# ryogrid/anime-illust-image-searcher

Hardware: AMD Instinct MI355X
Metric: images/sec tagged (ViT fwd) (higher is better)
Workload: dtype f16; 1 GPU; wd-tagger ViT-B/16 448px 16-bit-operand forward + sigmoid + MCut tag selection, batch 64 per GPU, u8 NHWC images resident in HBM (BASELINE.json configs[1]); batch_per_gpu=64, image=448x448x3 u8, classes=10861, parallelism=single GPU

## Files before the change

anime-illust-image-searcher_amd/csrc/gemm.hip:

```cpp
#include <atomic>
#include <cstdlib>
#include <type_traits>

#include "gemm_plan.h"
#include "vit_internal.h"

namespace hipts {
namespace {

#ifndef HIPTS_DW_SNAKE
#define HIPTS_DW_SNAKE 1
#endif
#if HIPTS_DW_SNAKE
#define HIPTS_SNAKE_J(i, j) (((i) & 1) ? 3 - (j) : (j))
#else
#define HIPTS_SNAKE_J(i, j) (j)
#endif
#ifndef HIPTS_MFMA_ORDER
#define HIPTS_MFMA_ORDER 1
#endif
#include "gemm_epi.h"
#include "gemm_loop.h"


template <int EPI>
__global__ __launch_bounds__(512) void gemm_kernel(const GemmArgs a, int tiles_m, int tiles_n) {
    extern __shared__ __attribute__((aligned(16))) char smem[];
    const int tid = threadIdx.x, lane = tid & 63, wave = tid >> 6;
    const int wave_m = wave >> 2, wave_n = wave & 3;

    const int nwg = tiles_m * tiles_n;
    const int bid = xcd_work_id(blockIdx.x, nwg);
    const int tm = bid / tiles_n, tn = bid % tiles_n;
    const int m0 = tm * BM, n0 = tn * BN;
    const int K = a.K, nt = K / BK;
    const int w_rows = tiles_n * BN;

    f32x4 acc[8][4];
#pragma unroll
    for (int i = 0; i < 8; ++i)
#pragma unroll
        for (int j = 0; j < 4; ++j) acc[i][j] = f32x4{0.f, 0.f, 0.f, 0.f};

    stage_tile(a.A, a.M, K, m0, 0, smem, wave, lane);
    stage_tile(a.W, w_rows, K, n0, 0, smem + TILE_BYTES, wave, lane);
    asm volatile("s_waitcnt vmcnt(0)" ::: "memory");
    __syncthreads();

    for (int t = 0; t < nt; ++t) {
        char* cur = smem + (t & 1) * STAGE_BYTES;
        if (t + 1 < nt) {
            char* nxt = smem + ((t + 1) & 1) * STAGE_BYTES;
            stage_tile(a.A, a.M, K, m0, t + 1, nxt, wave, lane);
            stage_tile(a.W, w_rows, K, n0, t + 1, nxt + TILE_BYTES, wave, lane);
        }
#pragma unroll
        for (int kk = 0; kk < 2; ++kk) {
            bf16x8 af[8], wf[4];
#pragma unroll
            for (int j = 0; j < 4; ++j) wf[j] = read_frag(cur + TILE_BYTES, wave_n * 4 + j, kk, lane);
#pragma unroll
            for (int i = 0; i < 8; ++i) af[i] = read_frag(cur, wave_m * 8 + i, kk, lane);
#pragma unroll
            for (int i = 0; i < 8; ++i)
#pragma unroll
                for (int j = 0; j < 4; ++j) {
                    if constexpr (EPI == EPI_VT)
                        acc[i][j] = __builtin_amdgcn_mfma_f32_16x16x32_bf16(af[i], wf[j], acc[i][j], 0, 0, 0);
                    else
                        acc[i][j] = __builtin_amdgcn_mfma_f32_16x16x32_bf16(wf[j], af[i], acc[i][j], 0, 0, 0);
                }
        }
        asm volatile("s_waitcnt vmcnt(0)" ::: "memory");
        __syncthreads();
    }

    gemm_epilogue<EPI>(a, acc, m0, n0, wave_m, wave_n, lane);
}

__device__ __forceinline__ void wait_vmcnt(int n) {
    switch (n) {
        case 0: asm volatile("s_waitcnt vmcnt(0)" ::: "memory"); break;
        case 1: asm volatile("s_waitcnt vmcnt(1)" ::: "memory"); break;
        case 2: asm volatile("s_waitcnt vmcnt(2)" ::: "memory"); break;
        case 3: asm volatile("s_waitcnt vmcnt(3)" ::: "memory"); break;
        case 4: asm volatile("s_waitcnt vmcnt(4)" ::: "memory"); break;
        case 5: asm volatile("s_waitcnt vmcnt(5)" ::: "memory"); break;
        case 6: asm volatile("s_waitcnt vmcnt(6)" ::: "memory"); break;
        case 7: asm volatile("s_waitcnt vmcnt(7)" ::: "memory"); break;
        default: asm volatile("s_waitcnt vmcnt(8)" ::: "memory"); break;
    }
}

template <int EPI, int MR = 8, bool F16 = false, bool OP8 = false, bool SK = false, bool INT = false>
__global__ __launch_bounds__(512) __attribute__((amdgpu_num_vgpr(240))) void gemm_pp_kernel(const GemmArgs a, int tiles_m, int tiles_n) {
    static_assert(!INT || (EPI == EPI_RESID_XG && MR == 8 && !OP8 && !SK), "INT: the residual epilogue's interior form");
    static_assert(!OP8 || (F16 && MR == 8), "e4m3 operands: half 16-bit outputs, full tiles");
    static_assert(!SK || (!OP8 && MR == 8), "split-K: 16-bit operands, full tiles");
    constexpr int TBM = 2 * MR * 16;
    extern __shared__ __attribute__((aligned(16))) char smem[];
    __shared__ float2 st_table[256];
    __shared__ float2 sw_red[EPI == EPI_SWIGLU ? 1024 : 1];
    __shared__ unsigned sk_ticket[SK ? 4 : 1];
    __shared__ f32x4 colvec[INT ? (EPI == EPI_RESID_XGI ? 768 : 512) : 1];
    const int tid = threadIdx.x, lane = tid & 63;
    const int wave = __builtin_amdgcn_readfirstlane(tid >> 6);
    const int wave_m = wave >> 2, wave_n = wave & 3;

    const int nwg = tiles_m * tiles_n;
    const int K = OP8 ? a.K / 2 : a.K, nt_all = K / BK;
    const int w_rows = tiles_n * BN;
    const int S = SK ? a.sk_slices : 1;
    const int n_items = SK ? a.sk_first + (nwg - a.sk_first) * S : nwg;
    auto decode = [&](int item, WorkItem& w) {
        if (!SK || item < a.sk_first) {
            w.tile = item; w.slice = -1; w.kt0 = 0; w.nt = nt_all;
        } else {
            const int j = item - a.sk_first;
            w.tile = a.sk_first + j / S;
            w.slice = j - (j / S) * S;
            w.kt0 = w.slice * nt_all / S;
            w.nt = (w.slice + 1) * nt_all / S - w.kt0;
        }
    };
    const int scale_w = (127 - a.w_exp) * 0x01010101, scale_1 = 127 * 0x01010101;

    int stamp_tile = 0;
#define PPSTAMP(idx)                                                                                     \
    do {                                                                                                 \
        if (a.stamps && blockIdx.x == 8 && stamp_tile < 8) {                                             \
            __builtin_amdgcn_sched_barrier(0);                                                           \
            const unsigned long long ts_ = __builtin_readcyclecounter();                                 \
            if (lane == 0) a.stamps[wave * 64 + stamp_tile * 8 + (idx)] = ts_;                           \
            __builtin_amdgcn_sched_barrier(0);                                                           \
        }                                                                                                \
    } while (0)
    int item = blockIdx.x, m0, n0;
    WorkItem wi;
    decode(item, wi);
    tile_origin<TBM>(a, wi.tile, tiles_m, tiles_n, m0, n0);
    int par = 0;

    if (wave * 4 < 4 * MR) stage_tile(a.A, a.M, K, m0, wi.kt0, smem, wave, lane);
    stage_tile(a.W, w_rows, K, n0, wi.kt0, smem + TILE_BYTES, wave, lane);
    if constexpr (INT) {
        for (int i = tid; i < (a.N >> 2); i += 512) {
            colvec[i] = reinterpret_cast<const f32x4*>(a.ln_gamma)[i];
            colvec[256 + i] = reinterpret_cast<const f32x4*>(a.bias)[i];
            if constexpr (EPI == EPI_RESID_XGI) colvec[512 + i] = reinterpret_cast<const f32x4*>(a.col_u)[i];
        }
        asm volatile("s_waitcnt lgkmcnt(0)" ::: "memory");
    }

    for (;;) {
        f32x4 acc[MR][4];
        const bf16_t* src[8];
        int dst[8];
        {
            const int row_in = lane >> 3;
            const int chunk = (lane & 7) ^ row_in;
            auto slot = [&](int idx, bool isW, int rb8) {
                int grow = (isW ? n0 : m0) + rb8 * 8 + row_in;
                const int lim = isW ? w_rows : a.M;
                grow = grow < lim ? grow : lim - 1;
                src[idx] = (isW ? a.W : a.A) + (size_t)grow * K + (size_t)(wi.kt0 + 1) * BK + chunk * 8;
                dst[idx] = (isW ? TILE_BYTES : 0) + rb8 * 1024;
            };
            for (int u = 0; u < 2; ++u) {
                const int e = 2 * wave + u;
                slot(0 + u, true, e);
                slot(2 + u, true, 16 + e);
                slot(4 + u, false, e < 8 ? e : 2 * MR + (e - 8));
            }
            if constexpr (MR == 8) {
                for (int u = 0; u < 2; ++u) {
                    const int e = 2 * wave + u;
                    slot(6 + u, false, e < 8 ? 8 + e : 2 * MR + 8 + (e - 8));
                }
            } else if constexpr (MR == 6) {
                slot(6, false, wave < 4 ? 8 + wave : 2 * MR + 8 + (wave - 4));
                src[7] = src[6];
                dst[7] = dst[6];
            } else {
                static_assert(MR == 7, "tile heights: 256, 224 or 192 rows");
                auto hi = [](int f) { return f < 6 ? 8 + f : 2 * MR + 8 + (f - 6); };
                if (wave < 4) {
                    slot(6, false, hi(2 * wave));
                    slot(7, false, hi(2 * wave + 1));
                } else {
                    slot(6, false, hi(8 + (wave - 4)));
                    src[7] = src[6];
                    dst[7] = dst[6];
                }
            }
        }
        const int n_hi = (MR == 8 || (MR == 7 && wave < 4)) ? 2 : 1;
        PPSTAMP(0);
        asm volatile("s_waitcnt vmcnt(0)" ::: "memory");
        PPSTAMP(1);
        __builtin_amdgcn_s_barrier();
        if (wave_m == 1) __builtin_amdgcn_s_barrier();
        PPSTAMP(2);
        if (a.stamps && blockIdx.x == 8 && stamp_tile < 8 && lane == 0) a.stamps[wave * 64 + stamp_tile * 8 + 6] = wall_clock64();
        if (HIPTS_STAGE_AHEAD && !HIPTS_STAGE_ORDER_OLD && wi.nt > 1) {
            char* st1 = smem + ((par + 1) & 1) * STAGE_BYTES;
            for (int k : {4, 5, 0, 1}) {
                glds16(src[k], st1 + dst[k]);
                src[k] += BK;
            }
        }

        bf16x8 wf[2][4];
        i32x8 wf8[4], af8[4];
        unsigned xpf = 0;
        auto ktile = [&](int t, auto first_tag) __attribute__((always_inline)) {
            constexpr bool FIRST = decltype(first_tag)::value;
            const char* cur = smem + ((par + t) & 1) * STAGE_BYTES;
            char* nxt = smem + ((par + t + 1) & 1) * STAGE_BYTES;
            const bool more = t + 1 < wi.nt;
#pragma unroll
            for (int p = 0; p < 4; ++p) {
                const int mh = p >> 1, kk = p & 1;
                bf16x8 af[4];
                if constexpr (OP8) {
                    if (p < 2) {
#pragma unroll
                        for (int jj = 0; jj < 2; ++jj) wf8[2 * kk + jj] = read_frag8(cur + TILE_BYTES, wave_n * 4 + 2 * kk + jj, lane);
                    }
                    if (kk == 0) {
#pragma unroll
                        for (int i = 0; i < 4; ++i) af8[i] = read_frag8(cur, wave_m * MR + mh * 4 + i, lane);
                    }
                } else {
                if (p < 2) {
#pragma unroll
                    for (int j = 0; j < 4; ++j) wf[kk][j] = read_frag(cur + TILE_BYTES, wave_n * 4 + j, kk, lane);
                }
#pragma unroll
                for (int i = 0; i < 4; ++i)
                    if (mh * 4 + i < MR) af[i] = read_frag(cur, wave_m * MR + mh * 4 + i, kk, lane);
                }
                if (more) {
                    auto issue = [&](int k) {
                        glds16(src[k], nxt + dst[k]);
                        src[k] += BK;
                    };
                    if (HIPTS_STAGE_ORDER_OLD) {
                        issue(2 * p);
                        if (p < 3 || n_hi == 2) issue(2 * p + 1);
                        if (p == 3) {
                            if (n_hi == 2) asm volatile("s_waitcnt vmcnt(2)" ::: "memory");
                            else asm volatile("s_waitcnt vmcnt(1)" ::: "memory");
                        } else if (p == 1) {
                            asm volatile("s_waitcnt vmcnt(4)" ::: "memory");
                        }
                    } else if (HIPTS_STAGE_AHEAD) {
                        if (p == 0) {
                            issue(2); issue(3);
                        } else if (p == 1) {
                            issue(6);
                            if (n_hi == 2) issue(7);
                            wait_vmcnt(6 + n_hi);
                        } else if (p == 3) {
                            if (t + 2 < wi.nt) {
                                for (int k : {4, 5, 0, 1}) {
                                    glds16(src[k], const_cast<char*>(cur) + dst[k]);
                                    src[k] += BK;
                                }
                                wait_vmcnt(n_hi + 4);
                            } else {
                                wait_vmcnt(n_hi);
                            }
                        }
                    } else {
                        if (p == 0) {
                            issue(4); issue(5); issue(0); issue(1);
                            if (HIPTS_STAGE_W_EARLY) { issue(2); issue(3); }
                        } else if (p == 1) {
                            if (!HIPTS_STAGE_W_EARLY) { issue(2); issue(3); }
                            asm volatile("s_waitcnt vmcnt(6)" ::: "memory");
                        } else if (p == 2) {
                            issue(6);
                            if (n_hi == 2) issue(7);
                        } else {
                            if (n_hi == 2) asm volatile("s_waitcnt vmcnt(2)" ::: "memory");
                            else asm volatile("s_waitcnt vmcnt(1)" ::: "memory");
                        }
                    }
                } else if (p == 1) {
                    asm volatile("s_waitcnt vmcnt(0)" ::: "memory");
                }
                if constexpr (INT) {
                    if (!more && p == 2 && a.epi_prefetch) {
                        const int ldx = a.ld_out ? a.ld_out : a.N;
                        const char* xb = reinterpret_cast<const char*>(a.out_f32 + (size_t)(m0 + wave_m * 128) * ldx + n0 + wave_n * 64);
                        const unsigned o0 = (unsigned)(((lane >> 1) * ldx + (lane & 1) * 32) * 4), ost = (unsigned)(32 * ldx * 4);
                        asm volatile("global_load_dword %0, %1, %5\n\tglobal_load_dword %0, %2, %5\n\tglobal_load_dword %0, %3, %5\n\tglobal_load_dword %0, %4, %5"
                                     : "=&v"(xpf)
                                     : "v"(o0), "v"(o0 + ost), "v"(o0 + 2 * ost), "v"(o0 + 3 * ost), "s"(xb)
                                     : "memory");
                    }
                }
                __builtin_amdgcn_sched_barrier(0);
                __builtin_amdgcn_s_barrier();
                __builtin_amdgcn_sched_barrier(0);
                asm volatile("s_waitcnt lgkmcnt(0)" ::: "memory");
                __builtin_amdgcn_sched_barrier(0);
                __builtin_amdgcn_s_setprio(1);
                pp_multiply<EPI, MR, F16, OP8, FIRST>(p, acc, wf, af, wf8, af8, scale_w, scale_1);
                __builtin_amdgcn_s_setprio(0);
                __builtin_amdgcn_sched_barrier(0);
                __builtin_amdgcn_s_barrier();
                __builtin_amdgcn_sched_barrier(0);
            }
        };
        ktile(0, std::true_type{});
        for (int t = 1; t < wi.nt; ++t) ktile(t, std::false_type{});
        if (wave_m == 0) __builtin_amdgcn_s_barrier();
        PPSTAMP(3);
        if (a.stamps && blockIdx.x == 8 && stamp_tile < 8 && lane == 0) a.stamps[wave * 64 + stamp_tile * 8 + 7] = wall_clock64();

        int elane = lane;
        asm volatile("" : "+v"(elane));
        f32x4 bias_pre[4];
        if constexpr (INT) {
#pragma unroll
            for (int j = 0; j < 4; ++j) bias_pre[j] = f32x4{0.f, 0.f, 0.f, 0.f};
        } else {
            load_bias<EPI>(a, n0, wave_n, elane, bias_pre);
        }
        constexpr bool FOLDABLE = EPI == EPI_VT || EPI == EPI_GELU || EPI == EPI_STAR || EPI == EPI_QK || EPI == EPI_QK_ROPE || EPI == EPI_SWIGLU ||
                                  EPI == EPI_RESID_ROWSTAT || EPI == EPI_RESID_XGI;
        const bool fold_st = FOLDABLE && a.stat_in != nullptr;
        const bool fold_many = fold_st && a.stat_in_blocks > 4;
        float2 st_pv[4];
        if (fold_st && !fold_many && tid < TBM) row_stat_request(a, m0 + tid, st_pv);
        const int next = item + gridDim.x;
        const bool has_next = next < n_items;
        WorkItem wi_next{0, -1, 0, nt_all};
        int m0n = 0, n0n = 0;
        const int par_next = (par + wi.nt) & 1;
        if (has_next) {
            decode(next, wi_next);
            tile_origin<TBM>(a, wi_next.tile, tiles_m, tiles_n, m0n, n0n);
            char* st = smem + par_next * STAGE_BYTES;
            if (wave * 4 < 4 * MR) stage_tile(a.A, a.M, K, m0n, wi_next.kt0, st, wave, lane);
            stage_tile(a.W, w_rows, K, n0n, wi_next.kt0, st + TILE_BYTES, wave, lane);
        }
        PPSTAMP(4);
        bool run_epilogue = true;
        if constexpr (SK) {
            if (wi.slice >= 0) {
                constexpr size_t SLAB = (size_t)TBM * BN * 4;
                const int tl = wi.tile - a.sk_first;
                unsigned* tickets = reinterpret_cast<unsigned*>(a.sk_ws);
                char* slabs = reinterpret_cast<char*>(a.sk_ws) + 4096 + (size_t)tl * S * SLAB;
                {
                    const auto rs = __builtin_amdgcn_make_buffer_rsrc(slabs + (size_t)wi.slice * SLAB, 0, (int)SLAB, 0x00020000);
                    typedef unsigned int u32x4 __attribute__((ext_vector_type(4)));
#pragma unroll
                    for (int i = 0; i < MR; ++i)
#pragma unroll
                        for (int j = 0; j < 4; ++j)
                            __builtin_amdgcn_raw_buffer_store_b128(__builtin_bit_cast(u32x4, acc[i][j]), rs, (((wave * MR + i) * 4 + j) * 64 + lane) * 16, 0, 16);
                }
                asm volatile("s_waitcnt vmcnt(0)" ::: "memory");
                __builtin_amdgcn_s_barrier();
                if (threadIdx.x == 0)
                    sk_ticket[0] = __hip_atomic_fetch_add(tickets + tl, 1u, __ATOMIC_RELAXED, __HIP_MEMORY_SCOPE_AGENT);
                __builtin_amdgcn_fence(__ATOMIC_RELEASE, "workgroup");
                __builtin_amdgcn_s_barrier();
                __builtin_amdgcn_fence(__ATOMIC_ACQUIRE, "workgroup");
                const unsigned ticket = sk_ticket[0];
                if (ticket != (unsigned)(S - 1)) {
                    run_epilogue = false;
                } else {
                    if (threadIdx.x == 0) {
                        __builtin_amdgcn_fence(__ATOMIC_ACQUIRE, "agent");
                        __hip_atomic_store(tickets + tl, 0u, __ATOMIC_RELAXED, __HIP_MEMORY_SCOPE_AGENT);
                    }
                    asm volatile("s_waitcnt vmcnt(0)" ::: "memory");
                    __builtin_amdgcn_s_barrier();
                    const f32x4* sl = reinterpret_cast<const f32x4*>(slabs) + (size_t)(wave * MR * 4) * 64 + lane;
#pragma unroll
                    for (int i = 0; i < MR; ++i) {
#pragma unroll
                        for (int j = 0; j < 4; ++j) acc[i][j] = sl[(size_t)(i * 4 + j) * 64];
                        for (int sx = 1; sx < S; ++sx) {
                            const f32x4* sp = sl + (size_t)sx * (SLAB / 16);
                            f32x4 v[4];
#pragma unroll
                            for (int j = 0; j < 4; ++j) v[j] = sp[(size_t)(i * 4 + j) * 64];
#pragma unroll
                            for (int j = 0; j < 4; ++j) acc[i][j] = acc[i][j] + v[j];
                        }
                    }
                }
            }
        }
        if (run_epilogue) {
            if (fold_st) fold_publish(a, m0, tid, TBM, fold_many, st_pv, st_table);
            bool staged = false;
            if constexpr (staged_epilogue_built(EPI)) {
                if (staged_epilogue_ok(EPI, a)) {
                    float2* red = (EPI == EPI_SWIGLU && a.stat_part) ? sw_red : nullptr;
                    gemm_epilogue_staged<EPI, MR, F16>(a, acc, m0, n0, wave_m, wave_n, elane, smem + ((par + wi.nt + 1) & 1) * STAGE_BYTES + wave * 8192, bias_pre,
                                                       fold_st ? st_table : nullptr, red);
                    staged = true;
                    if constexpr (EPI == EPI_SWIGLU) {
                        if (red) {
                            lds_table_visible();
                            if (tid < TBM) {
                                const float2 p0 = red[tid * 4], p1 = red[tid * 4 + 1], p2 = red[tid * 4 + 2], p3 = red[tid * 4 + 3];
                                const int m = m0 + tid;
                                if (m < a.M)
                                    *reinterpret_cast<float2*>(a.stat_part + 2 * ((size_t)(n0 >> 8) * a.stat_stride + m)) =
                                        make_float2((p0.x + p1.x) + (p2.x + p3.x), (p0.y + p1.y) + (p2.y + p3.y));
                            }
                        }
                    }
                }
            }
            if (!staged)
                gemm_epilogue<EPI, MR, F16, INT>(a, acc, m0, n0, wave_m, wave_n, elane, bias_pre, smem + ((par + wi.nt + 1) & 1) * STAGE_BYTES,
                                                 fold_st ? st_table : nullptr, INT ? colvec : nullptr);
        }
        if (a.epi_prio) __builtin_amdgcn_s_setprio(0);
        if constexpr (INT) asm volatile("" ::"v"(xpf));
        PPSTAMP(5);
        ++stamp_tile;
        if (!has_next) break;
        item = next;
        wi = wi_next;
        m0 = m0n;
        n0 = n0n;
        par = par_next;
    }
#undef PPSTAMP
}

#define PP2_STAMP(idx)                                                                                   \
    if constexpr (STAMP) {                                                                               \
        if (blockIdx.x == 0 && (t == 10 || t == 11)) {                                                   \
            __builtin_amdgcn_sched_barrier(0);                                                           \
            unsigned long long ts_;                                                                      \
            asm volatile("s_memtime %0\n\ts_waitcnt lgkmcnt(0)" : "=s"(ts_)::"memory");                 \
            if (lane == 0) a.stamps[wave * 64 + (t - 10) * 16 + mh * 8 + (idx)] = ts_;                   \
            __builtin_amdgcn_sched_barrier(0);                                                           \
        }                                                                                                \
    }

template <int EPI, bool STAMP = false>
__global__ __launch_bounds__(512) void gemm_pp2_kernel(const GemmArgs a, int tiles_m, int tiles_n) {
    extern __shared__ __attribute__((aligned(16))) char smem[];
    const int tid = threadIdx.x, lane = tid & 63;
    const int wave = __builtin_amdgcn_readfirstlane(tid >> 6);
    const int wave_m = wave >> 2, wave_n = wave & 3;

    const int nwg = tiles_m * tiles_n;
    const int bid = xcd_work_id(blockIdx.x, nwg);
    const int tm = bid / tiles_n, tn = bid % tiles_n;
    const int m0 = tm * BM, n0 = tn * BN;
    const int K = a.K, nt = K / BK;
    const int w_rows = tiles_n * BN;

    f32x4 acc[8][4];
#pragma unroll
    for (int i = 0; i < 8; ++i)
#pragma unroll
        for (int j = 0; j < 4; ++j) acc[i][j] = f32x4{0.f, 0.f, 0.f, 0.f};

    stage_tile(a.A, a.M, K, m0, 0, smem, wave, lane);
    stage_tile(a.W, w_rows, K, n0, 0, smem + TILE_BYTES, wave, lane);

    const bf16_t* src[8];
    int dst[8];
    {
        const int row_in = lane >> 3;
        const int chunk = (lane & 7) ^ row_in;
        auto slot = [&](int idx, bool isW, int rb8) {
            int grow = (isW ? n0 : m0) + rb8 * 8 + row_in;
            const int lim = isW ? w_rows : a.M;
            grow = grow < lim ? grow : lim - 1;
            src[idx] = (isW ? a.W : a.A) + (size_t)grow * K + BK + chunk * 8;
            dst[idx] = (isW ? TILE_BYTES : 0) + rb8 * 1024;
        };
        for (int u = 0; u < 4; ++u) slot(u, true, 4 * wave + u);
        for (int u = 0; u < 2; ++u) {
            const int e = 2 * wave + u;
            slot(4 + u, false, e < 8 ? e : e + 8);
            slot(6 + u, false, e < 8 ? 8 + e : 16 + e);
        }
    }
    asm volatile("s_waitcnt vmcnt(0)" ::: "memory");
    __builtin_amdgcn_s_barrier();
    if (wave_m == 1) __builtin_amdgcn_s_barrier();

    bf16x8 wf[2][4];
    for (int t = 0; t < nt; ++t) {
        const char* cur = smem + (t & 1) * STAGE_BYTES;
        char* nxt = smem + ((t + 1) & 1) * STAGE_BYTES;
        const bool more = t + 1 < nt;
#pragma unroll
        for (int mh = 0; mh < 2; ++mh) {
            PP2_STAMP(0)
            bf16x8 af[2][4];
            if (mh == 0) {
#pragma unroll
                for (int kk = 0; kk < 2; ++kk)
#pragma unroll
                    for (int j = 0; j < 4; ++j) wf[kk][j] = read_frag(cur + TILE_BYTES, wave_n * 4 + j, kk, lane);
            }
#pragma unroll
            for (int kk = 0; kk < 2; ++kk)
#pragma unroll
                for (int i = 0; i < 4; ++i) af[kk][i] = read_frag(cur, wave_m * 8 + mh * 4 + i, kk, lane);
            if (more) {
                if (mh == 0) {
#pragma unroll
                    for (int u = 0; u < 6; ++u) {
                        glds16(src[u], nxt + dst[u]);
                        src[u] += BK;
                    }
                    PP2_STAMP(1)
                    asm volatile("s_waitcnt vmcnt(6)" ::: "memory");
                } else {
#pragma unroll
                    for (int u = 6; u < 8; ++u) {
                        glds16(src[u], nxt + dst[u]);
                        src[u] += BK;
                    }
                    PP2_STAMP(1)
                    asm volatile("s_waitcnt vmcnt(2)" ::: "memory");
                }
            } else if (mh == 0) {
                asm volatile("s_waitcnt vmcnt(0)" ::: "memory");
            }
            PP2_STAMP(2)
            __builtin_amdgcn_sched_barrier(0);
            __builtin_amdgcn_s_barrier();
            __builtin_amdgcn_sched_barrier(0);
            PP2_STAMP(3)
            asm volatile("s_waitcnt lgkmcnt(0)" ::: "memory");
            __builtin_amdgcn_sched_barrier(0);
            PP2_STAMP(4)
            __builtin_amdgcn_s_setprio(1);
#pragma unroll
            for (int kk = 0; kk < 2; ++kk)
#pragma unroll
                for (int i = 0; i < 4; ++i)
#pragma unroll
                    for (int j = 0; j < 4; ++j) {
                        if constexpr (EPI == EPI_VT)
                            acc[mh * 4 + i][j] = __builtin_amdgcn_mfma_f32_16x16x32_bf16(af[kk][i], wf[kk][j], acc[mh * 4 + i][j], 0, 0, 0);
                        else
                            acc[mh * 4 + i][j] = __builtin_amdgcn_mfma_f32_16x16x32_bf16(wf[kk][j], af[kk][i], acc[mh * 4 + i][j], 0, 0, 0);
                    }
            __builtin_amdgcn_s_setprio(0);
            PP2_STAMP(5)
// ... 126 lines not shown
            dst[4 + i] = DW_A_BYTES + rb * 1024;
        }
    }
    const int frag_off = (lane & 15) * 64 + (((lane >> 4) ^ Image64::swizzle(lane & 15)) * 16);
    auto issue = [&](int i, char* st) {
        glds16(src[i], st + dst[i]);
        src[i] += DW_BK;
    };
    auto frag = [&](const char* base, int rb) { return *reinterpret_cast<const bf16x8*>(base + rb * 1024 + frag_off); };

    f32x4 acc[8][4];

    const bool trace = a.stamps && a.trace && blockIdx.x < 4096;
    if (trace && tid == 0) {
        a.stamps[blockIdx.x * 8 + 0] = __builtin_amdgcn_s_getreg(63492);
        a.stamps[blockIdx.x * 8 + 1] = __builtin_amdgcn_s_getreg(63508);
        a.stamps[blockIdx.x * 8 + 2] = wall_clock64();
    }
    const int npro = nt < 3 ? nt : 3;
    for (int s0 = 0; s0 < npro; ++s0)
#pragma unroll
        for (int i = 0; i < 6; ++i) issue(i, smem + s0 * DW_STAGE);
    if (npro == 3) asm volatile("s_waitcnt vmcnt(12)" ::: "memory");
    else if (npro == 2) asm volatile("s_waitcnt vmcnt(6)" ::: "memory");
    else asm volatile("s_waitcnt vmcnt(0)" ::: "memory");
    __builtin_amdgcn_s_barrier();
    __builtin_amdgcn_sched_barrier(0);

    bf16x8 wfr[2][4], alo[2][4], ahi[4];
#pragma unroll
    for (int j = 0; j < 4; ++j) wfr[0][j] = frag(smem + DW_A_BYTES, wave_n * 4 + j);
#pragma unroll
    for (int i = 0; i < 4; ++i) alo[0][i] = frag(smem, wave_m * 8 + i);

    int slot = 0;
    unsigned long long wait_cyc = 0, bar_cyc = 0;
    const unsigned long long loop_t0 = a.stamps ? __builtin_readcyclecounter() : 0;
    const unsigned long long wall_t0 = a.stamps ? wall_clock64() : 0;
    auto mm = [&](f32x4& c, const bf16x8& av, const bf16x8& wv, bool zero) {
        const f32x4 c0 = zero ? f32x4{0.f, 0.f, 0.f, 0.f} : c;
        if constexpr (EPI == EPI_VT) c = mfma_16x16x32<F16>(av, wv, c0);
        else c = mfma_16x16x32<F16>(wv, av, c0);
    };
    auto step = [&](auto H1, auto H2, auto H3, auto U, auto Z) __attribute__((always_inline)) {
        constexpr bool has1 = decltype(H1)::value, has2 = decltype(H2)::value, has3 = decltype(H3)::value, first = decltype(Z)::value;
        constexpr int u = decltype(U)::value;
        const char* cur = smem + slot * DW_STAGE;
        const int slot1 = slot == 2 ? 0 : slot + 1;
        const char* nx = smem + slot1 * DW_STAGE;
#pragma unroll
        for (int i = 0; i < 4; ++i)
#pragma unroll
            for (int j = 0; j < 4; ++j) {
                mm(acc[i][HIPTS_SNAKE_J(i, j)], alo[u][i], wfr[u][HIPTS_SNAKE_J(i, j)], first);
                if (i == 0) ahi[j] = frag(cur, wave_m * 8 + 4 + j);
                __builtin_amdgcn_sched_barrier(0);
            }
        if constexpr (has1) {
            unsigned long long q0 = 0, q1 = 0;
            if (a.stamps) q0 = __builtin_readcyclecounter();
            if constexpr (has2) asm volatile("s_waitcnt vmcnt(6) lgkmcnt(0)" ::: "memory");
            else asm volatile("s_waitcnt vmcnt(0) lgkmcnt(0)" ::: "memory");
            if (a.stamps) q1 = __builtin_readcyclecounter();
            __builtin_amdgcn_s_barrier();
            if (a.stamps) { const unsigned long long q2 = __builtin_readcyclecounter(); wait_cyc += q1 - q0; bar_cyc += q2 - q1; }
        }
        __builtin_amdgcn_sched_barrier(0);
        char* fill = smem + slot * DW_STAGE;
#pragma unroll
        for (int i = 0; i < 4; ++i)
#pragma unroll
            for (int j = 0; j < 4; ++j) {
                mm(acc[4 + i][HIPTS_SNAKE_J(i, j)], ahi[i], wfr[u][HIPTS_SNAKE_J(i, j)], first);
                const int idx = i * 4 + j;
                if constexpr (has1) {
                    if (idx < 4) wfr[u ^ 1][idx] = frag(nx + DW_A_BYTES, wave_n * 4 + idx);
                    else if (idx < 8) alo[u ^ 1][idx - 4] = frag(nx, wave_m * 8 + (idx - 4));
                }
                if constexpr (has3) {
                    if (idx >= 8 && idx < 14) issue(idx - 8, fill);
                }
                __builtin_amdgcn_sched_barrier(0);
            }
        slot = slot1;
    };
    using T = std::true_type;
    using F = std::false_type;
    using U0 = std::integral_constant<int, 0>;
    using U1 = std::integral_constant<int, 1>;
    if (nt >= 6) {
        step(T{}, T{}, T{}, U0{}, T{});
        step(T{}, T{}, T{}, U1{}, F{});
        for (int s = 2; s + 6 <= nt; s += 2) {
            step(T{}, T{}, T{}, U0{}, F{});
            step(T{}, T{}, T{}, U1{}, F{});
        }
    }
    if (nt >= 4) {
        if (nt == 4) step(T{}, T{}, T{}, U0{}, T{});
        else step(T{}, T{}, T{}, U0{}, F{});
        step(T{}, T{}, F{}, U1{}, F{});
    }
    if (nt == 2) step(T{}, F{}, F{}, U0{}, T{});
    else step(T{}, F{}, F{}, U0{}, F{});
    step(F{}, F{}, F{}, U1{}, F{});
    if (trace && tid == 0) a.stamps[blockIdx.x * 8 + 3] = wall_clock64();
    if (a.stamps && !trace && blockIdx.x == 8 && lane == 0) {
        a.stamps[wave * 64 + 0] = __builtin_readcyclecounter() - loop_t0;
        a.stamps[wave * 64 + 1] = wait_cyc;
        a.stamps[wave * 64 + 2] = bar_cyc;
        a.stamps[wave * 64 + 3] = wall_clock64() - wall_t0;
    }
    __builtin_amdgcn_s_barrier();
    if constexpr (staged_epilogue_built(EPI)) {
        if (staged_epilogue_ok(EPI, a)) {
            const float2* st_tab = nullptr;
            if (a.stat_in) {
                float2* tab = reinterpret_cast<float2*>(smem + 4 * 8192 * 2);
                fold_rows<false>(a, m0 + tid, tab, tid);
                st_tab = tab;
            }
            gemm_epilogue_staged<EPI, 8, F16>(a, acc, m0, n0, wave_m, wave_n, lane, smem + wave * 8192, nullptr, st_tab);
            if (trace && tid == 0) a.stamps[blockIdx.x * 8 + 4] = wall_clock64();
            return;
        }
    }
    gemm_epilogue<EPI, 8, F16>(a, acc, m0, n0, wave_m, wave_n, lane, nullptr, smem);
    if (trace && tid == 0) a.stamps[blockIdx.x * 8 + 4] = wall_clock64();
}

static_assert(GEMM_PLAN_TILE == BM && GEMM_PLAN_TILE == BN && GEMM_PLAN_BK == BK && GEMM_PLAN_HALF_BN == DW_BN && GEMM_PLAN_HALF_BN == S3_BN &&
              GEMM_PLAN_LDS == LDS_BYTES && GEMM_PLAN_LDS3 == DW_LDS && GEMM_PLAN_LDS3 == S3_LDS, "gemm_plan.h plans for other tiles than these kernels'");

std::atomic<long long> g_q4_mask{-1};
unsigned gemm_q4_mask() {
    long long v = g_q4_mask.load(std::memory_order_relaxed);
    if (v < 0) {
        v = getenv("HIPTS_GEMM_Q4") ? (long long)(unsigned)strtoul(getenv("HIPTS_GEMM_Q4"), nullptr, 0) : (long long)GEMM_Q4_DEFAULT_MASK;
        g_q4_mask.store(v, std::memory_order_relaxed);
    }
    return (unsigned)v;
}

int gemm_variant() { return gemm_knobs().variant; }

int gemm_plan_status(const GemmPlan& p, GemmEpilogue epi) {
    if (p.error == 1) return set_error(HIPTS_ERR_INVALID, "half-precision operands are only built for the pp and dw GEMM loops");
    if (p.error == 2) return set_error(HIPTS_ERR_INVALID, "gemm: e4m3 operands are not built for epilogue %d", (int)epi);
    return HIPTS_OK;
}

using GemmKernel = void (*)(const GemmArgs, int, int);
template <int EPI>
GemmKernel pp_kernel(int mr, bool f16, bool op8, bool sk, bool interior) {
    if (op8) {
        if constexpr (EPI == EPI_STAR || EPI == EPI_RESID || EPI == EPI_RESCALE || EPI == EPI_RESID_LN || EPI == EPI_QK || EPI == EPI_VT || EPI == EPI_BIAS)
            if (mr == 8 && f16 && !sk && !interior) return gemm_pp_kernel<EPI, 8, true, true>;
        return nullptr;
    }
    if (sk) {
        if constexpr (EPI == EPI_RESID || EPI == EPI_RESID_XG || EPI == EPI_RESID_XGI || EPI == EPI_RESID_ROWSTAT || EPI == EPI_HEAD)
            if (mr == 8 && !interior) return f16 ? gemm_pp_kernel<EPI, 8, true, false, true> : gemm_pp_kernel<EPI, 8, false, false, true>;
        return nullptr;
    }
    if (interior) {
        if constexpr (EPI == EPI_RESID_XG)
            if (mr == 8) return f16 ? gemm_pp_kernel<EPI, 8, true, false, false, true> : gemm_pp_kernel<EPI, 8, false, false, false, true>;
        return nullptr;
    }
    if (f16) return mr == 6 ? gemm_pp_kernel<EPI, 6, true> : mr == 7 ? gemm_pp_kernel<EPI, 7, true> : mr == 8 ? gemm_pp_kernel<EPI, 8, true> : nullptr;
    return mr == 7 ? gemm_pp_kernel<EPI, 7, false> : mr == 8 ? gemm_pp_kernel<EPI, 8, false> : nullptr;
}

template <int EPI>
int kernel_resources_t(int mr, bool f16, bool op8, bool sk, bool interior, int* num_regs, int* scratch_bytes, int* static_lds) {
    const GemmKernel k = pp_kernel<EPI>(mr, f16, op8, sk, interior);
    HIPTS_REQUIRE(k != nullptr, "hiptsdbg_gemm_kernel_resources: no gemm_pp_kernel is built for epilogue %d, mr %d, f16 %d, op8 %d, sk %d, interior %d", EPI, mr,
                  (int)f16, (int)op8, (int)sk, (int)interior);
    hipFuncAttributes at;
    HIPTS_HIP(hipFuncGetAttributes(&at, reinterpret_cast<const void*>(k)));
    *num_regs = at.numRegs;
    *scratch_bytes = (int)at.localSizeBytes;
    *static_lds = (int)at.sharedSizeBytes;
    return HIPTS_OK;
}

template <int EPI>
int launch_t(const GemmArgs& a, hipStream_t s) {
    int dev = 0;
    const int cus = current_device_cus(&dev);
    const GemmPlan p = gemm_plan((GemmEpilogue)EPI, a, cus, gemm_knobs(), gemm_q4_mask());
    HIPTS_TRY(gemm_plan_status(p, (GemmEpilogue)EPI));
    GemmArgs ar = a;
    ar.raster_gm = p.raster_gm; ar.raster_gn = p.raster_gn; ar.epi_prio = p.epi_prio; ar.epi_prefetch = p.epi_prefetch;
    ar.sk_first = p.sk_first; ar.sk_slices = p.sk_slices;
    const bool f16 = a.f16 != 0;
    auto go = [&](void (*kernel)(const GemmArgs, int, int)) { kernel<<<p.grid, p.block, p.lds_bytes, s>>>(ar, p.tiles_m, p.tiles_n); };
    switch (p.loop) {
        case HIPTSDBG_GEMM_Q4: return launch_gemm_q4((GemmEpilogue)EPI, ar, p, dev, s);
        case HIPTSDBG_GEMM_PP_E4M3:
            if constexpr (EPI == EPI_STAR || EPI == EPI_RESID || EPI == EPI_RESCALE || EPI == EPI_RESID_LN || EPI == EPI_QK || EPI == EPI_VT ||
                          EPI == EPI_BIAS) {
                static PerDevice once;
                HIPTS_TRY(allow_dynamic_lds(once, dev, p.lds_bytes, gemm_pp_kernel<EPI, 8, true, true>));
                go(pp_kernel<EPI>(8, true, true, false, false));
            }
            break;
        case HIPTSDBG_GEMM_DW: {
            if constexpr (EPI == EPI_VT || EPI == EPI_GELU || EPI == EPI_STAR || EPI == EPI_QK || EPI == EPI_QK_ROPE || EPI == EPI_SWIGLU)
                HIPTS_REQUIRE(!(a.stat_in && a.stat_in_blocks > 4), "gemm: the two-workgroups-per-CU loop folds at most 4 stat_in pairs per row (%d given)", a.stat_in_blocks);
            static PerDevice once;
            HIPTS_TRY(allow_dynamic_lds(once, dev, p.lds_bytes, gemm_dw_kernel<EPI, false>, gemm_dw_kernel<EPI, true>));
            if (f16) go(gemm_dw_kernel<EPI, true>);
            else go(gemm_dw_kernel<EPI, false>);
            break;
        }
        case HIPTSDBG_GEMM_S3: {
            static PerDevice once;
            HIPTS_TRY(allow_dynamic_lds(once, dev, p.lds_bytes, gemm_s3_kernel<EPI>));
            go(gemm_s3_kernel<EPI>);
            break;
        }
        case HIPTSDBG_GEMM_V1: {
            static PerDevice once;
            HIPTS_TRY(allow_dynamic_lds(once, dev, p.lds_bytes, gemm_kernel<EPI>));
            go(gemm_kernel<EPI>);
            break;
        }
        case HIPTSDBG_GEMM_PP2: {
            static PerDevice once;
            if constexpr (EPI == EPI_GELU) {
                HIPTS_TRY(allow_dynamic_lds(once, dev, p.lds_bytes, gemm_pp2_kernel<EPI, false>, gemm_pp2_kernel<EPI, true>));
                if (p.stamped) {
                    go(gemm_pp2_kernel<EPI, true>);
                    break;
                }
            } else {
                HIPTS_TRY(allow_dynamic_lds(once, dev, p.lds_bytes, gemm_pp2_kernel<EPI, false>));
            }
            go(gemm_pp2_kernel<EPI, false>);
            break;
        }
        default: {
            if constexpr (EPI == EPI_RESID || EPI == EPI_RESID_XG || EPI == EPI_RESID_XGI || EPI == EPI_RESID_ROWSTAT || EPI == EPI_HEAD) {
                if (p.sk_slices >= 2) {
                    static PerDevice once;
                    HIPTS_TRY(allow_dynamic_lds(once, dev, p.lds_bytes, gemm_pp_kernel<EPI, 8, false, false, true>, gemm_pp_kernel<EPI, 8, true, false, true>));
                    go(pp_kernel<EPI>(8, f16, false, true, false));
                    break;
                }
            }
            if constexpr (EPI == EPI_RESID_XG) {
                if (p.interior) {
                    static PerDevice once;
                    HIPTS_TRY(allow_dynamic_lds(once, dev, p.lds_bytes, gemm_pp_kernel<EPI, 8, false, false, false, true>, gemm_pp_kernel<EPI, 8, true, false, false, true>));
                    go(pp_kernel<EPI>(8, f16, false, false, true));
                    break;
                }
            }
            static PerDevice once;
            HIPTS_TRY(allow_dynamic_lds(once, dev, p.lds_bytes, gemm_pp_kernel<EPI, 8, false>, gemm_pp_kernel<EPI, 7, false>, gemm_pp_kernel<EPI, 8, true>,
                                        gemm_pp_kernel<EPI, 7, true>, gemm_pp_kernel<EPI, 6, true>));
            const GemmKernel k = pp_kernel<EPI>(p.mr, f16, false, false, false);
            HIPTS_REQUIRE(k != nullptr, "gemm: no %d-row tiles are built for these operands", 32 * p.mr);
            go(k);
        }
    }
    HIPTS_LAUNCH_CHECK();
    return HIPTS_OK;
}

}

const GemmKnobs& gemm_knobs() {
    static const GemmKnobs knobs = [] {
        auto num = [](const char* name, int dflt) { const char* e = getenv(name); return e ? atoi(e) : dflt; };
        GemmKnobs k;
        const char* e = getenv("HIPTS_GEMM");
        k.variant_set = e != nullptr;
        k.variant = (e && strcmp(e, "v1") == 0) ? HIPTSDBG_GEMM_V1 : (e && strcmp(e, "pp2") == 0) ? HIPTSDBG_GEMM_PP2 : (e && strcmp(e, "s3") == 0) ? HIPTSDBG_GEMM_S3
                    : (e && strcmp(e, "dw") == 0) ? HIPTSDBG_GEMM_DW : HIPTSDBG_GEMM_PP;
        k.auto_dw = num("HIPTS_GEMM_AUTO_DW", 1) != 0;
        k.dw_limit4 = num("HIPTS_GEMM_DW_LIMIT", 2);
        k.dw_mask = getenv("HIPTS_GEMM_DW_MASK") ? (unsigned)strtoul(getenv("HIPTS_GEMM_DW_MASK"), nullptr, 0) : 0u;
        e = getenv("HIPTS_GEMM_BM");
        k.min_mr = !e ? 6 : strcmp(e, "256") == 0 ? 8 : strcmp(e, "224") == 0 ? 7 : 6;
        k.mr_shared = num("HIPTS_GEMM_MR_SHARED", -1);
        e = getenv("HIPTS_GEMM_PERSIST");
        k.persist = !(e && strcmp(e, "0") == 0);
        k.raster = num("HIPTS_GEMM_RASTER", 8);
        k.raster_gn = num("HIPTS_GEMM_RASTER_GN", 6);
        k.epi_prio = num("HIPTS_EPI_PRIO", 0);
        k.epi_prefetch = num("HIPTS_EPI_PREFETCH", 0);
        k.resid_general = num("HIPTS_RESID_GENERAL", 0) != 0;
        k.splitk = num("HIPTS_GEMM_SPLITK", 0);
        k.splitk_head = num("HIPTS_GEMM_SPLITK_HEAD", 0);
        k.splitk_minkt = num("HIPTS_GEMM_SPLITK_MINKT", 5);
        return k;
    }();
    return knobs;
}

int launch_gemm(GemmEpilogue epi, const GemmArgs& a, hipStream_t s) {
    if (a.op8) HIPTS_REQUIRE(a.K % 128 == 0 && a.K >= 128, "gemm: K=%d must be a positive multiple of 128 with e4m3 operands", a.K);
    if (a.out8)
        HIPTS_REQUIRE((epi == EPI_STAR || epi == EPI_RESID_LN) && (a.ld_out ? a.ld_out : a.N) % 16 == 0,
                      "gemm: e4m3 output needs the STAR / RESID_LN epilogue and a row stride that is a multiple of 16");
    HIPTS_REQUIRE(a.K % BK == 0 && a.K >= BK, "gemm: K=%d must be a positive multiple of %d", a.K, BK);
    HIPTS_REQUIRE(a.M >= 1 && a.N >= 1, "gemm: empty problem");
    if (epi != EPI_HEAD) HIPTS_REQUIRE(a.N % 16 == 0, "gemm: N=%d must be a multiple of 16", a.N);
    if (epi == EPI_VT) HIPTS_REQUIRE(a.M % 4 == 0 && a.tokens % 4 == 0, "gemm: V^T epilogue needs tokens %% 4 == 0");
    if (epi == EPI_VT && staged_epilogue_ok(epi, a))
        HIPTS_REQUIRE(a.M % 8 == 0, "gemm: V^T epilogue with tokens %% 8 == 0 needs M %% 8 == 0 (M = %d)", a.M);
    if (epi == EPI_QK || epi == EPI_VT) HIPTS_REQUIRE(a.hd_log2 == 5 || a.hd_log2 == 6, "gemm: head_dim must be 32 or 64");
    if (epi == EPI_QK || epi == EPI_QK_ROPE)
        HIPTS_REQUIRE(a.out_bf16 && a.out2_bf16 && a.dim > 0 && a.N <= 3 * a.dim && (a.N <= 2 * a.dim || a.out3_bf16), "gemm: q / k / v outputs missing for N = %d, dim = %d", a.N, a.dim);
    if (epi == EPI_QK_ROPE)
        HIPTS_REQUIRE(a.hd_log2 == 6 && a.dim % 64 == 0 && a.rope && a.rope_tokens >= 0 && a.tokens >= 1, "gemm: QK_ROPE needs head_dim 64 and the rotary table");
    if (epi == EPI_RESID_XG) HIPTS_REQUIRE(!a.rowstat && !a.stat_in, "gemm: RESID_XG ignores an input fold; use RESID_XGI");
    if (epi == EPI_RESID_XGI) HIPTS_REQUIRE((a.rowstat || a.stat_in) && a.col_u, "gemm: RESID_XGI needs rowstat / stat_in and col_u");
    if (epi == EPI_RESID_XG || epi == EPI_RESID_XGI)
        HIPTS_REQUIRE(a.out_f32 && (!a.out_bf16 || (a.ln_gamma && a.N % 8 == 0 && (!a.stat_part || a.stat_stride >= a.M))),
                      "gemm: RESID_XG needs the fp32 stream, col_u with rowstat, and gamma (N %% 8 == 0) with the 16-bit copy");
    if (a.stat_in) HIPTS_REQUIRE(a.stat_in_blocks <= 64 && a.stat_in_blocks >= 1 && a.stat_in_stride >= a.M && a.ln_dim >= 1, "gemm: stat_in needs its block count (<= 64), stride and ln_dim");
    if ((a.rowstat || a.stat_in) && epi != EPI_RESID_ROWSTAT && epi != EPI_RESID_XGI)
        HIPTS_REQUIRE(a.col_u && (epi == EPI_QK || epi == EPI_QK_ROPE || epi == EPI_VT || epi == EPI_GELU || epi == EPI_SWIGLU || epi == EPI_STAR),
                      "gemm: a folded LayerNorm (rowstat) is built for the QK, QK_ROPE, VT, GELU, STAR and SWIGLU epilogues");
    if ((a.rowstat || a.stat_in) && epi != EPI_RESID_ROWSTAT && epi != EPI_RESID_XGI) {
        HIPTS_REQUIRE(staged_epilogue_ok(epi, a) && (gemm_variant() == 1 || gemm_variant() == 4), "gemm: a folded LayerNorm needs the staged epilogue (pp / dw loops, aligned outputs)");
    }
    if (epi == EPI_RESID_ROWSTAT) HIPTS_REQUIRE((a.rowstat || a.stat_in) && a.col_u && a.out_f32, "gemm: RESID_ROWSTAT needs rowstat / stat_in, col_u and the fp32 stream");
    if (epi == EPI_SWIGLU) HIPTS_REQUIRE(!a.stat_part || a.stat_stride >= a.M, "gemm: SWIGLU stat_stride must cover M rows");
    if (epi == EPI_SWIGLU)
        HIPTS_REQUIRE(a.N % 64 == 0 && (a.ld_out ? a.ld_out : a.N / 2) % 8 == 0 && a.out_bf16, "gemm: SWIGLU needs N %% 64 == 0 and an output stride that is a multiple of 8");
    if (epi == EPI_RESCALE) HIPTS_REQUIRE(a.res_scale != nullptr, "gemm: RESCALE epilogue needs res_scale");
    if (epi == EPI_RESID_LS) HIPTS_REQUIRE(a.res_scale && a.out_f32 && !a.x_blocked, "gemm: RESID_LS needs the layer scale and the row-major fp32 stream");
    if (epi == EPI_RESID_LN)
        HIPTS_REQUIRE(a.N <= BN && a.ln_gamma && a.out_bf16 && a.out_f32, "gemm: RESID_LN needs the whole row in one tile (N <= %d), gamma and both outputs", BN);
    switch (epi) {
        case EPI_PATCH: return launch_t<EPI_PATCH>(a, s);
        case EPI_QK: return launch_t<EPI_QK>(a, s);
        case EPI_VT: return launch_t<EPI_VT>(a, s);
        case EPI_RESID: return launch_t<EPI_RESID>(a, s);
        case EPI_GELU: return launch_t<EPI_GELU>(a, s);
        case EPI_HEAD: return launch_t<EPI_HEAD>(a, s);
        case EPI_STAR: return launch_t<EPI_STAR>(a, s);
        case EPI_RESCALE: return launch_t<EPI_RESCALE>(a, s);
        case EPI_BIAS: return launch_t<EPI_BIAS>(a, s);
        case EPI_RESID_LN: return launch_t<EPI_RESID_LN>(a, s);
        case EPI_QK_ROPE: return launch_t<EPI_QK_ROPE>(a, s);
        case EPI_SWIGLU: return launch_t<EPI_SWIGLU>(a, s);
        case EPI_RESID_ROWSTAT: return launch_t<EPI_RESID_ROWSTAT>(a, s);
        case EPI_RESID_XG: return launch_t<EPI_RESID_XG>(a, s);
        case EPI_RESID_XGI: return launch_t<EPI_RESID_XGI>(a, s);
        case EPI_RESID_LS: return launch_t<EPI_RESID_LS>(a, s);
    }
    return set_error(HIPTS_ERR_INVALID, "gemm: unknown epilogue");
}

void set_gemm_q4_mask(unsigned mask) { g_q4_mask.store((long long)mask, std::memory_order_relaxed); }

namespace {
__global__ void gelu_probe_kernel(const f32x4* __restrict__ x, f32x4* __restrict__ y, int n4, int tanh_form) {
    const int i = blockIdx.x * blockDim.x + threadIdx.x;
    if (i < n4) y[i] = gelu_f4(x[i], tanh_form);
}
}

}

extern "C" int hiptsdbg_gelu(const float* x_host, int n, int tanh_form, float* y_host) {
    using namespace hipts;
    HIPTS_TRY(use_device(0));
    HIPTS_REQUIRE(x_host && y_host && n > 0 && n % 4 == 0, "hiptsdbg_gelu: n must be a positive multiple of 4");
    DevBuf x, y;
    HIPTS_TRY(x.alloc((size_t)n * 4));
    HIPTS_TRY(y.alloc((size_t)n * 4));
    HIPTS_TRY(upload(x.p, x_host, (size_t)n * 4));
    gelu_probe_kernel<<<(n / 4 + 255) / 256, 256>>>(x.as<f32x4>(), y.as<f32x4>(), n / 4, tanh_form);
    HIPTS_LAUNCH_CHECK();
    HIPTS_HIP(hipMemcpy(y_host, y.p, (size_t)n * 4, hipMemcpyDeviceToHost));
    return HIPTS_OK;
}

extern "C" int hiptsdbg_gemm_kernel_resources(int epi, int mr, int f16, int op8, int sk, int interior, int* num_regs, int* scratch_bytes, int* static_lds) {
    using namespace hipts;
    HIPTS_REQUIRE(num_regs && scratch_bytes && static_lds && epi >= EPI_PATCH && epi <= EPI_RESID_LS, "hiptsdbg_gemm_kernel_resources: bad argument");
    HIPTS_TRY(use_device(0));
#define HIPTS_RES_CASE(E) \
    case E: return kernel_resources_t<E>(mr, f16 != 0, op8 != 0, sk != 0, interior != 0, num_regs, scratch_bytes, static_lds)
    switch (epi) {
        HIPTS_RES_CASE(EPI_PATCH); HIPTS_RES_CASE(EPI_QK); HIPTS_RES_CASE(EPI_VT); HIPTS_RES_CASE(EPI_RESID); HIPTS_RES_CASE(EPI_GELU);
        HIPTS_RES_CASE(EPI_HEAD); HIPTS_RES_CASE(EPI_STAR); HIPTS_RES_CASE(EPI_RESCALE); HIPTS_RES_CASE(EPI_BIAS); HIPTS_RES_CASE(EPI_RESID_LN);
        HIPTS_RES_CASE(EPI_QK_ROPE); HIPTS_RES_CASE(EPI_SWIGLU); HIPTS_RES_CASE(EPI_RESID_ROWSTAT); HIPTS_RES_CASE(EPI_RESID_XG);
        HIPTS_RES_CASE(EPI_RESID_XGI); HIPTS_RES_CASE(EPI_RESID_LS);
    }
#undef HIPTS_RES_CASE
    return set_error(HIPTS_ERR_INVALID, "hiptsdbg_gemm_kernel_resources: unknown epilogue");
}

extern "C" int hiptsdbg_gemm_plan(int epi, int M, int N, int K, int f16, int shared_chip, unsigned features, int ld_out, int dim, int cus,
                                  unsigned q4_mask, hiptsdbg_gemm_plan_t* out) {
    using namespace hipts;
    HIPTS_REQUIRE(out && epi >= EPI_PATCH && epi <= EPI_RESID_LS && M >= 1 && N >= 1 && K >= 64 && K % 64 == 0 && cus >= 1, "hiptsdbg_gemm_plan: bad argument");
    static float dummy[2];
    GemmArgs g{};
    g.M = M; g.N = N; g.K = K; g.f16 = f16; g.shared_chip = shared_chip; g.ld_out = ld_out; g.dim = dim;
    if (features & 1) g.stat_part = dummy;
    if (features & 2) { g.sk_ws = dummy; g.sk_ws_bytes = GEMM_SK_WS_BYTES; }
    if (features & 4) g.pos = dummy;
    if (features & 8) g.res_scale = dummy;
    if (features & 16) { g.out_bf16 = reinterpret_cast<bf16_t*>(dummy); g.ln_gamma = dummy; }
    if (features & 32) g.stat_in = dummy;
    if (features & 64) g.op8 = 1;
    if (features & 128) g.stamps = reinterpret_cast<unsigned long long*>(dummy);
    *out = gemm_plan((GemmEpilogue)epi, g, cus, gemm_knobs(), q4_mask);
    return gemm_plan_status(*out, (GemmEpilogue)epi);
}

extern "C" int hiptsdbg_gemm_tile_walk(int tiles_m, int tiles_n, int tile_rows, int raster_gm, int raster_gn, int32_t* m0, int32_t* n0) {
    using namespace hipts;
    HIPTS_REQUIRE(m0 && n0 && tiles_m >= 1 && tiles_n >= 1 && (tile_rows == 256 || tile_rows == 224 || tile_rows == 192) && raster_gm >= 0 && raster_gn >= 0,
                  "hiptsdbg_gemm_tile_walk: bad argument");
    GemmArgs g{};
    g.raster_gm = raster_gm;
    g.raster_gn = raster_gn;
    for (int id = 0; id < tiles_m * tiles_n; ++id) {
        int m, n;
        if (tile_rows == 256) tile_origin<256>(g, id, tiles_m, tiles_n, m, n);
        else if (tile_rows == 224) tile_origin<224>(g, id, tiles_m, tiles_n, m, n);
        else tile_origin<192>(g, id, tiles_m, tiles_n, m, n);
        m0[id] = m;
        n0[id] = n;
    }
    return HIPTS_OK;
}
```

anime-illust-image-searcher_amd/csrc/gemm_dbg.hip:

```cpp
#include <vector>

#include "../../include/hip_tagsearch_debug.h"
#include "vit_internal.h"

namespace hipts {
namespace {

int put_f32(DevBuf& buf, const float* host, size_t n, const float** dev) {
    *dev = nullptr;
    if (!host) return HIPTS_OK;
    HIPTS_TRY(buf.alloc(n * 4));
    HIPTS_TRY(upload(buf.p, host, n * 4));
    *dev = buf.as<float>();
    return HIPTS_OK;
}

int guarded(DevBuf& buf, uint64_t bytes, uint64_t need, int fill, const char* what, bool required) {
    if (bytes == 0) {
        HIPTS_REQUIRE(!required, "hiptsdbg_gemm_epilogue: the %s buffer is required by this epilogue", what);
        return HIPTS_OK;
    }
    HIPTS_REQUIRE(bytes >= need, "hiptsdbg_gemm_epilogue: the %s buffer has %llu bytes, the launch's extent is %llu", what, (unsigned long long)bytes,
                  (unsigned long long)need);
    HIPTS_TRY(buf.alloc(bytes));
    HIPTS_HIP(hipMemset(buf.p, fill & 0xff, bytes));
    return HIPTS_OK;
}

int fetch(void* host, const DevBuf& buf, uint64_t bytes) {
    if (bytes == 0) return HIPTS_OK;
    HIPTS_REQUIRE(host, "hiptsdbg_gemm_epilogue: an output buffer has a size but no host pointer");
    HIPTS_HIP(hipMemcpy(host, buf.p, bytes, hipMemcpyDeviceToHost));
    return HIPTS_OK;
}

}
}

extern "C" int hiptsdbg_gemm_epilogue(const hiptsdbg_gemm_case_t* in, hiptsdbg_gemm_out_t* out) {
    using namespace hipts;
    HIPTS_REQUIRE(in && out && in->a && in->w, "hiptsdbg_gemm_epilogue: null argument");
    const int epi = in->epi, M = in->M, N = in->N, K = in->K;
    HIPTS_REQUIRE(epi >= EPI_PATCH && epi <= EPI_RESID_LS && M >= 1 && N >= 1 && K >= 64 && K % 64 == 0 && (long long)M * K < (1ll << 31) &&
                      (long long)N * K < (1ll << 31),
                  "hiptsdbg_gemm_epilogue: unsupported shape");
    HIPTS_REQUIRE(epi == EPI_HEAD || N % 16 == 0, "hiptsdbg_gemm_epilogue: N must be a multiple of 16");
    HIPTS_TRY(use_device(0));

    const bool is_qk = epi == EPI_QK || epi == EPI_QK_ROPE;
    const uint64_t ld = in->ld_out ? in->ld_out : (epi == EPI_SWIGLU ? N / 2 : N);
    HIPTS_REQUIRE(ld >= (uint64_t)(epi == EPI_SWIGLU ? N / 2 : N) || is_qk || epi == EPI_VT, "hiptsdbg_gemm_epilogue: ld_out is smaller than a row");
    const bool blocked_ok = epi == EPI_RESID || epi == EPI_RESCALE || epi == EPI_RESID_ROWSTAT || epi == EPI_RESID_XG || epi == EPI_RESID_XGI ||
                            epi == EPI_BIAS || epi == EPI_RESID_LN;
    HIPTS_REQUIRE(!in->x_blocked || (blocked_ok && ld % 16 == 0), "hiptsdbg_gemm_epilogue: x_blocked needs a residual / bias epilogue and ld %% 16 == 0");
    const bool writes_x = blocked_ok || epi == EPI_PATCH || epi == EPI_RESID_LS;
    const uint64_t rows_x = in->x_blocked ? (uint64_t)round_up(M, 16) : (uint64_t)M;
    uint64_t need16[3] = {0, 0, 0};
    bool req16[3] = {false, false, false};
    if (is_qk || epi == EPI_VT) {
        HIPTS_REQUIRE(in->tokens >= 1 && in->tokens_pad >= in->tokens && in->dim >= 16 && (in->hd_log2 == 5 || in->hd_log2 == 6) &&
                          (in->heads << in->hd_log2) == in->dim && N <= (is_qk ? 3 : 1) * in->dim,
                      "hiptsdbg_gemm_epilogue: q / k / v layouts need tokens <= tokens_pad, heads * head_dim == dim and N within the layouts");
        const uint64_t images = (uint64_t)(M + in->tokens - 1) / in->tokens;
        const uint64_t layout = images * in->tokens_pad * in->dim * 2;
        need16[0] = layout; req16[0] = true;
        if (is_qk) { need16[1] = layout; req16[1] = true; }
        if (is_qk && N > 2 * in->dim) { need16[2] = layout; req16[2] = true; }
    } else if (epi == EPI_GELU || epi == EPI_STAR || epi == EPI_SWIGLU || epi == EPI_RESID_LN) {
        need16[0] = (uint64_t)M * ld * 2; req16[0] = true;
    } else if (epi == EPI_RESID_XG || epi == EPI_RESID_XGI || epi == EPI_RESID_LS) {
        need16[0] = (uint64_t)M * ld * 2;
    }
    if (epi == EPI_PATCH || in->pos) HIPTS_REQUIRE(in->pos && in->tokens >= 1, "hiptsdbg_gemm_epilogue: pos needs tokens");
    const bool has_stat = epi == EPI_SWIGLU || epi == EPI_RESID_XG || epi == EPI_RESID_XGI;
    HIPTS_REQUIRE(out->stat_part_bytes == 0 || (has_stat && in->stat_stride >= M), "hiptsdbg_gemm_epilogue: stat_part needs SWIGLU / RESID_XG / RESID_XGI and stat_stride >= M");
    HIPTS_REQUIRE(out->rowmajor_bytes == 0 || (in->x_blocked && (epi == EPI_RESID || epi == EPI_RESCALE || epi == EPI_RESID_ROWSTAT)),
                  "hiptsdbg_gemm_epilogue: resid_rowmajor_out needs x_blocked and a plain residual epilogue");
    HIPTS_REQUIRE(out->probs_bytes == 0 || epi == EPI_HEAD, "hiptsdbg_gemm_epilogue: probs is EPI_HEAD's");
    HIPTS_REQUIRE(in->x_init_bytes <= out->x_bytes && (in->x_init_bytes == 0 || in->x_init), "hiptsdbg_gemm_epilogue: x_init does not fit x");
    if (in->stat_in)
        HIPTS_REQUIRE(in->stat_in_blocks >= 1 && in->stat_in_blocks <= 64 && in->stat_in_stride >= M, "hiptsdbg_gemm_epilogue: stat_in needs its block count and stride");

    DevBuf x, rowmajor, probs, o16[3], stat;
    HIPTS_TRY(guarded(x, out->x_bytes, (writes_x || epi == EPI_HEAD) ? rows_x * ld * 4 : 0, in->fill, "x", writes_x));
    HIPTS_TRY(guarded(rowmajor, out->rowmajor_bytes, (uint64_t)M * ld * 4, in->fill, "rowmajor", false));
    HIPTS_TRY(guarded(probs, out->probs_bytes, (uint64_t)M * ld * 4, in->fill, "probs", false));
    for (int i = 0; i < 3; ++i) {
        HIPTS_REQUIRE(out->out16_bytes[i] == 0 || need16[i] > 0, "hiptsdbg_gemm_epilogue: this epilogue has no 16-bit output %d", i);
        HIPTS_TRY(guarded(o16[i], out->out16_bytes[i], need16[i], in->fill, "out16", req16[i]));
    }
    HIPTS_TRY(guarded(stat, out->stat_part_bytes, (uint64_t)((N + 255) / 256) * (uint64_t)in->stat_stride * 8, in->fill, "stat_part", false));
    if (in->x_init_bytes) HIPTS_TRY(upload(x.p, in->x_init, in->x_init_bytes));

    DevBuf A, W, bias, pos, rs, lg, lb, cu, rst, sti, rope, skws;
    const int Np = round_up(N, 256);
    HIPTS_TRY(A.alloc((size_t)M * K * 2));
    HIPTS_TRY(W.alloc((size_t)Np * K * 2));
    HIPTS_HIP(hipMemset(W.p, 0, W.bytes));
    HIPTS_TRY(upload(A.p, in->a, (size_t)M * K * 2));
    HIPTS_TRY(upload(W.p, in->w, (size_t)N * K * 2));
    GemmArgs g{};
    g.A = A.as<bf16_t>(); g.W = W.as<bf16_t>(); g.M = M; g.N = N; g.K = K; g.f16 = in->f16 ? 1 : 0; g.shared_chip = in->shared_chip ? 1 : 0;
    if (in->bias) {
        HIPTS_TRY(put_f32(bias, in->bias, (size_t)N, &g.bias));
    } else {
        HIPTS_TRY(bias.alloc((size_t)Np * 4));
        HIPTS_HIP(hipMemset(bias.p, 0, bias.bytes));
        g.bias = bias.as<float>();
    }
    HIPTS_TRY(put_f32(pos, in->pos, in->pos ? (size_t)in->tokens * N : 0, &g.pos));
    HIPTS_TRY(put_f32(rs, in->res_scale, (size_t)N, &g.res_scale));
    HIPTS_TRY(put_f32(lg, in->ln_gamma, (size_t)(epi == EPI_SWIGLU ? N / 2 : N), &g.ln_gamma));
    HIPTS_TRY(put_f32(lb, in->ln_beta, (size_t)N, &g.ln_beta));
    HIPTS_TRY(put_f32(cu, in->col_u, (size_t)N, &g.col_u));
    HIPTS_TRY(put_f32(rst, in->rowstat, (size_t)2 * M, &g.rowstat));
    HIPTS_TRY(put_f32(sti, in->stat_in, in->stat_in ? (size_t)2 * in->stat_in_blocks * in->stat_in_stride : 0, &g.stat_in));
    if (epi == EPI_QK_ROPE) {
        HIPTS_REQUIRE(in->rope && in->rope_tokens >= 1, "hiptsdbg_gemm_epilogue: QK_ROPE needs the rotary table");
        HIPTS_TRY(put_f32(rope, in->rope, (size_t)in->rope_tokens * 64, &g.rope));
    }
    if (in->sk_ws) {
        HIPTS_TRY(skws.alloc(GEMM_SK_WS_BYTES));
        HIPTS_HIP(hipMemset(skws.p, 0, skws.bytes));
        g.sk_ws = skws.p; g.sk_ws_bytes = GEMM_SK_WS_BYTES;
    }
    g.out_f32 = out->x_bytes ? x.as<float>() : nullptr;
    g.resid_rowmajor_out = out->rowmajor_bytes ? rowmajor.as<float>() : nullptr;
    g.out2_f32 = out->probs_bytes ? probs.as<float>() : nullptr;
    g.out_bf16 = out->out16_bytes[0] ? o16[0].as<bf16_t>() : nullptr;
    g.out2_bf16 = out->out16_bytes[1] ? o16[1].as<bf16_t>() : nullptr;
    g.out3_bf16 = out->out16_bytes[2] ? o16[2].as<bf16_t>() : nullptr;
    g.stat_part = out->stat_part_bytes ? stat.as<float>() : nullptr;
    g.stat_stride = in->stat_stride;
    g.tokens = in->tokens; g.tokens_pad = in->tokens_pad; g.heads = in->heads; g.dim = in->dim; g.hd_log2 = in->hd_log2;
    g.stat_in_blocks = in->stat_in_blocks; g.stat_in_stride = in->stat_in_stride; g.ln_dim = in->ln_dim; g.rope_tokens = in->rope_tokens;
    g.gelu_tanh = in->gelu_tanh; g.star_kind = in->star_kind; g.ld_out = in->ld_out; g.x_blocked = in->x_blocked ? 1 : 0;
    g.qscale = in->qscale; g.ln_eps = in->ln_eps; g.star_scale = in->star_scale; g.star_bias = in->star_bias;

    HIPTS_TRY(launch_gemm((GemmEpilogue)epi, g, nullptr));
    HIPTS_HIP(hipDeviceSynchronize());

    HIPTS_TRY(fetch(out->x, x, out->x_bytes));
    HIPTS_TRY(fetch(out->rowmajor, rowmajor, out->rowmajor_bytes));
    HIPTS_TRY(fetch(out->probs, probs, out->probs_bytes));
    for (int i = 0; i < 3; ++i) HIPTS_TRY(fetch(out->out16[i], o16[i], out->out16_bytes[i]));
    HIPTS_TRY(fetch(out->stat_part, stat, out->stat_part_bytes));
    return HIPTS_OK;
}
```

anime-illust-image-searcher_amd/csrc/gemm_epi.h:

```cpp

constexpr int BM = 256, BN = 256, BK = 64;
#ifndef HIPTS_STAGE_AHEAD
#define HIPTS_STAGE_AHEAD 1
#endif
#ifndef HIPTS_STAGE_W_EARLY
#define HIPTS_STAGE_W_EARLY 0
#endif
#ifndef HIPTS_STAGE_ORDER_OLD
#define HIPTS_STAGE_ORDER_OLD 0
#endif
constexpr int TILE_BYTES = BM * BK * 2;
constexpr int STAGE_BYTES = 2 * TILE_BYTES;
constexpr int LDS_BYTES = 2 * STAGE_BYTES;

__device__ __forceinline__ void glds16(const void* g, void* lds) {
    __builtin_amdgcn_global_load_lds((const __attribute__((address_space(1))) void*)g,
                                     (__attribute__((address_space(3))) void*)lds, 16, 0, 0);
}

__device__ __forceinline__ void stage_tile(const bf16_t* __restrict__ X, int rows_total, int K, int row0, int kt,
                                           char* lds_tile, int wave, int lane) {
    const int row_in = lane >> 3;
    const int chunk = (lane & 7) ^ row_in;
#pragma unroll
    for (int i = 0; i < 4; ++i) {
        const int rb8 = wave * 4 + i;
        int grow = row0 + rb8 * 8 + row_in;
        grow = grow < rows_total ? grow : rows_total - 1;
        const bf16_t* g = X + (size_t)grow * K + (size_t)kt * BK + chunk * 8;
        glds16(g, lds_tile + rb8 * 1024);
    }
}

__device__ __forceinline__ bf16x8 read_frag(const char* lds_tile, int rowblk, int kk, int lane) {
    const int r = lane & 15;
    const int c = (kk * 4 + (lane >> 4)) ^ (r & 7);
    return *reinterpret_cast<const bf16x8*>(lds_tile + (rowblk * 2 + (r >> 3)) * 1024 + (r & 7) * 128 + c * 16);
}

__device__ __forceinline__ i32x8 read_frag8(const char* lds_tile, int rowblk, int lane) {
    const int r = lane & 15, q = lane >> 4;
    const char* row = lds_tile + (rowblk * 2 + (r >> 3)) * 1024 + (r & 7) * 128;
    const int4 lo = *reinterpret_cast<const int4*>(row + (((2 * q) ^ (r & 7)) * 16));
    const int4 hi = *reinterpret_cast<const int4*>(row + (((2 * q + 1) ^ (r & 7)) * 16));
    return i32x8{lo.x, lo.y, lo.z, lo.w, hi.x, hi.y, hi.z, hi.w};
}

template <bool TANH>
__device__ __forceinline__ f32x4 gelu_f4(f32x4 x) {
    if constexpr (TANH) {
        const float c1 = -2.885390081777927f * 0.7978845608028654f, c2 = c1 * 0.044715f;
        const f32x4 t = x * x;
        const f32x4 g = x * __builtin_elementwise_fma(f32x4{c2, c2, c2, c2}, t, f32x4{c1, c1, c1, c1});
        f32x4 e{__builtin_amdgcn_exp2f(g[0]), __builtin_amdgcn_exp2f(g[1]), __builtin_amdgcn_exp2f(g[2]), __builtin_amdgcn_exp2f(g[3])};
        e = e + f32x4{1.f, 1.f, 1.f, 1.f};
        return x * f32x4{__builtin_amdgcn_rcpf(e[0]), __builtin_amdgcn_rcpf(e[1]), __builtin_amdgcn_rcpf(e[2]), __builtin_amdgcn_rcpf(e[3])};
    }
    const f32x4 xc{__builtin_amdgcn_fmed3f(x[0], -5.5f, 5.5f), __builtin_amdgcn_fmed3f(x[1], -5.5f, 5.5f), __builtin_amdgcn_fmed3f(x[2], -5.5f, 5.5f),
                   __builtin_amdgcn_fmed3f(x[3], -5.5f, 5.5f)};
    const f32x4 t = xc * xc;
    auto k4 = [](float c) { return f32x4{c, c, c, c}; };
    f32x4 p = __builtin_elementwise_fma(k4(2.2240455115528255e-08f), t, k4(6.478198381570408e-06f));
    p = __builtin_elementwise_fma(p, t, k4(0.00017989516452868775f));
    p = __builtin_elementwise_fma(p, t, k4(0.00474442647621276f));
    p = __builtin_elementwise_fma(p, t, k4(0.03488362160853281f));
    p = __builtin_elementwise_fma(p, t, k4(0.39894214428114516f));
    f32x4 q = __builtin_elementwise_fma(k4(1.1920686967418627e-06f), t, k4(7.74708620425572e-05f));
    q = __builtin_elementwise_fma(q, t, k4(0.0019464965294343475f));
    q = __builtin_elementwise_fma(q, t, k4(0.02924650260921815f));
    q = __builtin_elementwise_fma(q, t, k4(0.25410501090673415f));
    q = __builtin_elementwise_fma(q, t, k4(1.0f));
    const f32x4 rq{__builtin_amdgcn_rcpf(q[0]), __builtin_amdgcn_rcpf(q[1]), __builtin_amdgcn_rcpf(q[2]), __builtin_amdgcn_rcpf(q[3])};
    const f32x4 r = (xc * p) * rq;
    return x * (r + k4(0.5f));
}
__device__ __forceinline__ f32x4 gelu_f4(f32x4 x, int tanh_form) { return tanh_form ? gelu_f4<true>(x) : gelu_f4<false>(x); }

__device__ __forceinline__ float2 ln_stat_pair(const GemmArgs& a, float s1, float s2) {
    const float inv = 1.0f / (float)a.ln_dim;
    const float mean = s1 * inv;
    const float var = fmaxf(s2 * inv - mean * mean, 0.f);
    const float rstd = 1.0f / sqrtf(var + a.ln_eps);
    return make_float2(rstd, rstd * mean);
}

__device__ __forceinline__ float2 row_stat(const GemmArgs& a, int m) {
    m = m < a.M ? m : a.M - 1;
    if (a.stat_in) {
        float s1 = 0.f, s2 = 0.f;
        int b = 0;
        for (; b + 8 <= a.stat_in_blocks; b += 8) {
            float2 v[8];
#pragma unroll
            for (int u = 0; u < 8; ++u) v[u] = *reinterpret_cast<const float2*>(a.stat_in + 2 * ((size_t)(b + u) * a.stat_in_stride + m));
#pragma unroll
            for (int u = 0; u < 8; ++u) {
                s1 += v[u].x;
                s2 += v[u].y;
            }
        }
        for (; b < a.stat_in_blocks; ++b) {
            const float2 v = *reinterpret_cast<const float2*>(a.stat_in + 2 * ((size_t)b * a.stat_in_stride + m));
            s1 += v.x;
            s2 += v.y;
        }
        return ln_stat_pair(a, s1, s2);
    }
    return *reinterpret_cast<const float2*>(a.rowstat + 2 * (size_t)m);
}

__device__ __forceinline__ void row_stat_request(const GemmArgs& a, int m, float2 (&pv)[4]) {
    m = m < a.M ? m : a.M - 1;
#pragma unroll
    for (int b = 0; b < 4; ++b)
        pv[b] = b < a.stat_in_blocks ? *reinterpret_cast<const float2*>(a.stat_in + 2 * ((size_t)b * a.stat_in_stride + m)) : make_float2(0.f, 0.f);
}
__device__ __forceinline__ float2 row_stat_finish(const GemmArgs& a, const float2 (&pv)[4]) {
    return ln_stat_pair(a, ((pv[0].x + pv[1].x) + pv[2].x) + pv[3].x, ((pv[0].y + pv[1].y) + pv[2].y) + pv[3].y);
}

__device__ __forceinline__ void epi_turn(const GemmArgs& a, int wave_m, int step) {
    if (a.epi_prio) {
        if ((step ^ wave_m) & 1) __builtin_amdgcn_s_setprio(1);
        else __builtin_amdgcn_s_setprio(0);
    }
}

__device__ __forceinline__ size_t x_off(const GemmArgs& a, int m, int nc, int ld) {
    if (a.x_blocked) return (((size_t)(m >> 4) * (size_t)(ld >> 4) + (size_t)(nc >> 4)) << 8) + (size_t)((m & 15) * 16 + (nc & 15));
    return (size_t)m * ld + nc;
}

template <int EPI>
__device__ __forceinline__ void load_cols(const float* __restrict__ vec, const GemmArgs& a, int n0, int wave_n, int lane, f32x4 (&bv)[4]);
template <int EPI>
__device__ __forceinline__ void load_bias(const GemmArgs& a, int n0, int wave_n, int lane, f32x4 (&bv)[4]) {
    load_cols<EPI>(a.bias, a, n0, wave_n, lane, bv);
}
template <int EPI>
__device__ __forceinline__ void load_cols(const float* __restrict__ vec, const GemmArgs& a, int n0, int wave_n, int lane, f32x4 (&bv)[4]) {
    const int lr = lane & 15, lq = lane >> 4;
#pragma unroll
    for (int j = 0; j < 4; ++j) {
        if constexpr (EPI == EPI_VT) {
            const int n = n0 + wave_n * 64 + j * 16 + lr;
            bv[j] = f32x4{n < a.N ? vec[n] : 0.f, 0.f, 0.f, 0.f};
        } else if constexpr (EPI == EPI_HEAD) {
            bv[j] = f32x4{0.f, 0.f, 0.f, 0.f};
        } else {
            const int nc = n0 + wave_n * 64 + j * 16 + 4 * lq;
            bv[j] = nc < a.N ? *reinterpret_cast<const f32x4*>(vec + nc) : f32x4{0.f, 0.f, 0.f, 0.f};
        }
    }
}

__device__ __forceinline__ f32x4 star_relu4(f32x4 x, float s, float b, int kind = 0) {
    if (kind == 1) {
        const f32x4 g = x * -1.4426950408889634f;
        const f32x4 e{__builtin_amdgcn_exp2f(g[0]), __builtin_amdgcn_exp2f(g[1]), __builtin_amdgcn_exp2f(g[2]), __builtin_amdgcn_exp2f(g[3])};
        const f32x4 d = e + 1.0f;
        return x * f32x4{__builtin_amdgcn_rcpf(d[0]), __builtin_amdgcn_rcpf(d[1]), __builtin_amdgcn_rcpf(d[2]), __builtin_amdgcn_rcpf(d[3])};
    }
    if (kind == 2) return x;
    const f32x4 r = __builtin_elementwise_max(x, f32x4{0.f, 0.f, 0.f, 0.f});
    return r * r * s + b;
}

template <int EPI>
__device__ __forceinline__ void epi_bias(const GemmArgs& a, int n0, int wave_n, int lane, const f32x4* bias_pre, f32x4 (&bias_v)[4]) {
    if (bias_pre) {
#pragma unroll
        for (int j = 0; j < 4; ++j) bias_v[j] = bias_pre[j];
    } else {
        load_bias<EPI>(a, n0, wave_n, lane, bias_v);
    }
}

template <int CHUNKS>
struct RowImage {
    static_assert(CHUNKS == 8 || CHUNKS == 4, "128 B or 64 B rows");
    static __device__ __forceinline__ int swizzle(int row) { return CHUNKS == 8 ? (row >> 1) & 7 : (row >> 2) & 3; }
    static __device__ __forceinline__ char* at(char* image, int row, int chunk) { return image + row * (CHUNKS * 16) + (chunk ^ swizzle(row)) * 16; }
    static __device__ __forceinline__ void put4(char* image, int row, int j, int lq, bf16x4 v) {
// ... 424 lines not shown
                __builtin_amdgcn_fence(__ATOMIC_ACQUIRE, "workgroup");
                const int t = wave_n * 64 + lane;
                if (t < MR * 16) {
                    const int r = wave_m * (MR * 16) + t;
                    const float2 p0 = red[r * 4], p1 = red[r * 4 + 1], p2 = red[r * 4 + 2], p3 = red[r * 4 + 3];
                    const int m = m0 + r;
                    if (m < a.M)
                        *reinterpret_cast<float2*>(a.stat_part + 2 * ((size_t)(n0 >> 8) * a.stat_stride + m)) =
                            make_float2((p0.x + p1.x) + (p2.x + p3.x), (p0.y + p1.y) + (p2.y + p3.y));
                }
            }
            return;
        }
        if constexpr (EPI == EPI_RESID || EPI == EPI_RESCALE || EPI == EPI_RESID_ROWSTAT || EPI == EPI_RESID_LS) {
            f32x4 rs[4];
            if constexpr (EPI == EPI_RESCALE) {
#pragma unroll
                for (int j = 0; j < 4; ++j) rs[j] = nv[j] ? *reinterpret_cast<const f32x4*>(a.res_scale + nc[j]) : f32x4{0.f, 0.f, 0.f, 0.f};
            }
            if constexpr (EPI == EPI_RESID_ROWSTAT) {
#pragma unroll
                for (int j = 0; j < 4; ++j) rs[j] = nv[j] ? *reinterpret_cast<const f32x4*>(a.col_u + nc[j]) : f32x4{0.f, 0.f, 0.f, 0.f};
            }
            constexpr int RB = 4;
            auto rmw = [&](auto interior_tag) {
                constexpr bool INTERIOR = decltype(interior_tag)::value;
#pragma unroll
                for (int i2 = 0; i2 < MR; i2 += RB) {
                    epi_turn(a, wave_m, i2 / RB);
                    f32x4 xv[RB][4];
#pragma unroll
                    for (int u = 0; u < RB; ++u) {
                        if (i2 + u >= MR) continue;
                        const int m = m0 + wave_m * (MR * 16) + (i2 + u) * 16 + lr;
                        const int mr = (INTERIOR || m < a.M) ? m : a.M - 1;
#pragma unroll
                        for (int j = 0; j < 4; ++j)
                            xv[u][j] = (INTERIOR || nv[j]) ? *reinterpret_cast<const f32x4*>(a.out_f32 + x_off(a, mr, nc[j], ld)) : f32x4{0.f, 0.f, 0.f, 0.f};
                    }
#pragma unroll
                    for (int u = 0; u < RB; ++u) {
                        if (i2 + u >= MR) continue;
                        const int m = m0 + wave_m * (MR * 16) + (i2 + u) * 16 + lr;
                        const int mc = (INTERIOR || m < a.M) ? m : a.M - 1;
                        float* row = (a.x_blocked && a.resid_rowmajor_out) ? a.resid_rowmajor_out + (size_t)mc * ld : nullptr;
                        float2 st = make_float2(1.f, 0.f);
                        if constexpr (EPI == EPI_RESID_ROWSTAT) st = st_lds ? st_lds[mc - m0] : row_stat(a, mc);
#pragma unroll
                        for (int j = 0; j < 4; ++j) {
                            f32x4 v;
                            if constexpr (EPI == EPI_RESCALE)
                                v = xv[u][j] * rs[j] + (acc[i2 + u][j] + bv[j]);
                            else if constexpr (EPI == EPI_RESID_ROWSTAT)
                                v = xv[u][j] + ((acc[i2 + u][j] * st.x - rs[j] * st.y) + bv[j]);
                            else if constexpr (EPI == EPI_RESID_LS)
                                v = xv[u][j] + ((INTERIOR || nv[j]) ? *reinterpret_cast<const f32x4*>(a.res_scale + nc[j]) : f32x4{0.f, 0.f, 0.f, 0.f}) *
                                                   (acc[i2 + u][j] + bv[j]);
                            else
                                v = xv[u][j] + (acc[i2 + u][j] + bv[j]);
                            if (INTERIOR || (nv[j] && m < a.M)) *reinterpret_cast<f32x4*>(row ? row + nc[j] : a.out_f32 + x_off(a, mc, nc[j], ld)) = v;
                            if constexpr (EPI == EPI_RESID_LS) {
                                if (a.out_bf16 && (INTERIOR || (nv[j] && m < a.M)))
                                    *reinterpret_cast<bf16x4*>(a.out_bf16 + (size_t)mc * ld + nc[j]) = pack4<F16>(v[0], v[1], v[2], v[3]);
                            }
                        }
                    }
                }
            };
            if (m0 + 2 * MR * 16 <= a.M && n0 + BN <= a.N) rmw(std::true_type{});
            else rmw(std::false_type{});
            return;
        }
        if constexpr (EPI == EPI_PATCH || EPI == EPI_BIAS) {
            if (m0 + 2 * MR * 16 <= a.M && n0 + BN <= a.N) {
#pragma unroll
                for (int i = 0; i < MR; ++i) {
                    const int m = m0 + wave_m * (MR * 16) + i * 16 + lr;
                    f32x4 pv[4];
                    if constexpr (EPI == EPI_PATCH) {
                        const int t = m % a.tokens;
#pragma unroll
                        for (int j = 0; j < 4; ++j) pv[j] = *reinterpret_cast<const f32x4*>(a.pos + (size_t)t * a.N + nc[j]);
                    }
#pragma unroll
                    for (int j = 0; j < 4; ++j) {
                        if constexpr (EPI == EPI_PATCH) *reinterpret_cast<f32x4*>(a.out_f32 + (size_t)m * ld + nc[j]) = acc[i][j] * a.qscale + bv[j] + pv[j];
                        else *reinterpret_cast<f32x4*>(a.out_f32 + x_off(a, m, nc[j], ld)) = acc[i][j] + bv[j];
                    }
                }
                return;
            }
        }
        if constexpr (EPI == EPI_GELU) {
            auto rows = [&](auto form) __attribute__((always_inline)) {
#pragma unroll
                for (int i = 0; i < MR; ++i) {
                    const int m = m0 + wave_m * (MR * 16) + i * 16 + lr;
                    if (m >= a.M) continue;
#pragma unroll
                    for (int j = 0; j < 4; ++j) {
                        if (!nv[j]) continue;
                        const f32x4 gv = gelu_f4<decltype(form)::value>(acc[i][j] + bv[j]);
                        *reinterpret_cast<bf16x4*>(a.out_bf16 + (size_t)m * ld + nc[j]) = pack4<F16>(gv[0], gv[1], gv[2], gv[3]);
                    }
                }
            };
            if (a.gelu_tanh) rows(std::true_type{});
            else rows(std::false_type{});
            return;
        }
#pragma unroll
        for (int i = 0; i < MR; ++i) {
            const int m = m0 + wave_m * (MR * 16) + i * 16 + lr;
            if (m >= a.M) continue;
            if constexpr (EPI == EPI_PATCH) {
                const int t = m % a.tokens;
                f32x4 pv[4];
#pragma unroll
                for (int j = 0; j < 4; ++j)
                    pv[j] = nv[j] ? *reinterpret_cast<const f32x4*>(a.pos + (size_t)t * a.N + nc[j]) : f32x4{0.f, 0.f, 0.f, 0.f};
#pragma unroll
                for (int j = 0; j < 4; ++j)
                    if (nv[j]) *reinterpret_cast<f32x4*>(a.out_f32 + (size_t)m * ld + nc[j]) = acc[i][j] * a.qscale + bv[j] + pv[j];
            } else if constexpr (EPI == EPI_BIAS) {
#pragma unroll
                for (int j = 0; j < 4; ++j)
                    if (nv[j]) *reinterpret_cast<f32x4*>(a.out_f32 + x_off(a, m, nc[j], ld)) = acc[i][j] + bv[j];
            } else if constexpr (EPI == EPI_STAR) {
#pragma unroll
                for (int j = 0; j < 4; ++j) {
                    if (!nv[j]) continue;
                    const f32x4 v = star_relu4(acc[i][j] + bv[j], a.star_scale, a.star_bias, a.star_kind);
                    *reinterpret_cast<bf16x4*>(a.out_bf16 + (size_t)m * ld + nc[j]) = pack4<F16>(v[0], v[1], v[2], v[3]);
                }
            } else if constexpr (EPI == EPI_QK) {
                const int b = m / a.tokens, t = m - b * a.tokens;
#pragma unroll
                for (int j = 0; j < 4; ++j) {
                    if (!nv[j]) continue;
                    const int which = nc[j] >= 2 * a.dim ? 2 : (nc[j] >= a.dim ? 1 : 0);
                    const int nn = nc[j] - which * a.dim;
                    const int head = nn >> a.hd_log2, d = nn & ((1 << a.hd_log2) - 1);
                    const float sc = which ? 1.0f : a.qscale;
                    const f32x4 v = acc[i][j] + bv[j];
                    const bf16x4 o = pack4<F16>(v[0] * sc, v[1] * sc, v[2] * sc, v[3] * sc);
                    bf16_t* base = which == 2 ? a.out3_bf16 : (which ? a.out2_bf16 : a.out_bf16);
                    *reinterpret_cast<bf16x4*>(base + ((((size_t)(b * a.heads + head) * a.tokens_pad + t)) << a.hd_log2) + d) = o;
                }
            }
        }
    }
}

template <int EPI, int MR, bool F16, int FORM = -1>
__device__ __forceinline__ void gemm_epilogue_staged(const GemmArgs& a, f32x4 (&acc)[MR][4], int m0, int n0, int wave_m, int wave_n,
                                                     int lane, char* region, const f32x4* bias_pre = nullptr, const float2* st_lds = nullptr,
                                                     float2* red = nullptr) {
    if constexpr (EPI == EPI_GELU && FORM < 0) {
        if (a.gelu_tanh) gemm_epilogue_staged<EPI, MR, F16, 1>(a, acc, m0, n0, wave_m, wave_n, lane, region, bias_pre, st_lds, red);
        else gemm_epilogue_staged<EPI, MR, F16, 0>(a, acc, m0, n0, wave_m, wave_n, lane, region, bias_pre, st_lds, red);
        return;
    }
    f32x4 bias_v[4];
    epi_bias<EPI>(a, n0, wave_n, lane, bias_pre, bias_v);
    static_assert(EPI == EPI_VT || EPI == EPI_GELU || EPI == EPI_STAR || EPI == EPI_QK || EPI == EPI_QK_ROPE || EPI == EPI_SWIGLU,
                  "staged epilogue: half-precision outputs only");
    constexpr bool IS_QK = EPI == EPI_QK || EPI == EPI_QK_ROPE;
    const bool fold = a.rowstat != nullptr || a.stat_in != nullptr;
    f32x4 cu[4];
    if (fold) load_cols<EPI>(a.col_u, a, n0, wave_n, lane, cu);
    else {
#pragma unroll
        for (int j = 0; j < 4; ++j) cu[j] = f32x4{0.f, 0.f, 0.f, 0.f};
    }
    const int lr = lane & 15, lq = lane >> 4;
    const int ncol0 = n0 + wave_n * 64;
    const int mrow0 = m0 + wave_m * (MR * 16);
    const int lc = lane & 7, lrow = lane >> 3;
    if constexpr (EPI == EPI_VT) {
        float bv[4];
#pragma unroll
        for (int j = 0; j < 4; ++j) bv[j] = bias_v[j][0];
#pragma unroll
        for (int pass = 0; pass < 2; ++pass) {
            if (pass) __builtin_amdgcn_wave_barrier();
#pragma unroll
            for (int ii = 0; ii < 4; ++ii) {
                const int i = pass * 4 + ii;
                if (i >= MR) continue;
                f32x4 sx{1.f, 1.f, 1.f, 1.f}, sy{0.f, 0.f, 0.f, 0.f};
                if (fold) {
                    const int mr = mrow0 + i * 16 + 4 * lq;
#pragma unroll
                    for (int e = 0; e < 4; ++e) {
                        const float2 st = st_lds ? st_lds[mr + e - m0] : row_stat(a, mr + e);
                        sx[e] = st.x;
                        sy[e] = st.y;
                    }
                }
#pragma unroll
                for (int j = 0; j < 4; ++j) {
                    const f32x4 c = acc[i][j] * sx + (bv[j] - sy * cu[j][0]);
                    Image128::put4(region, j * 16 + lr, ii, lq, pack4<F16>(c[0], c[1], c[2], c[3]));
                }
            }
            __builtin_amdgcn_fence(__ATOMIC_RELEASE, "wavefront");
            __builtin_amdgcn_wave_barrier();
            const int m = mrow0 + pass * 64 + lc * 8;
            const int b = m / a.tokens, t = m - b * a.tokens;
            const bool mv = pass * 64 + lc * 8 < MR * 16 && m < a.M;
#pragma unroll
            for (int r8 = 0; r8 < 8; ++r8) {
                const int d = r8 * 8 + lrow;
                const int n = ncol0 + d;
                const uint4 v = *reinterpret_cast<const uint4*>(Image128::at(region, d, lc));
                if (mv && n < a.N)
                    *reinterpret_cast<uint4*>(a.out_bf16 +
                                              ((((size_t)(b * a.heads + (n >> a.hd_log2))) << a.hd_log2) + (n & ((1 << a.hd_log2) - 1))) * a.tokens_pad + t) = v;
            }
            __builtin_amdgcn_fence(__ATOMIC_ACQUIRE, "wavefront");
        }
    } else {
        f32x4 bv[4];
#pragma unroll
        for (int j = 0; j < 4; ++j) bv[j] = bias_v[j];
        if constexpr (EPI == EPI_STAR) {
            if (a.out8) {
                staged_store_rows8<MR>(region, lane, mrow0, a.M, reinterpret_cast<uint8_t*>(a.out_bf16), a.ld_out ? a.ld_out : a.N, ncol0, a.N,
                                       [&](int i, int j) { return star_relu4(acc[i][j] + bv[j], a.star_scale, a.star_bias, a.star_kind); });
                return;
            }
        }
        if constexpr (EPI == EPI_SWIGLU) {
#pragma unroll
            for (int i = 0; i < MR; ++i) {
                float2 st = make_float2(1.f, 0.f);
                if (fold) st = st_lds ? st_lds[mrow0 - m0 + i * 16 + lr] : row_stat(a, mrow0 + i * 16 + lr);
#pragma unroll
                for (int jj = 0; jj < 2; ++jj)
                    acc[i][jj] = star_relu4(acc[i][jj] * st.x + (bv[jj] - cu[jj] * st.y), 0.f, 0.f, 1) *
                                 (acc[i][jj + 2] * st.x + (bv[jj + 2] - cu[jj + 2] * st.y));
                if (a.stat_part) {
                    const float2 s = row_sums<2>(acc[i]);
                    const int m = mrow0 + i * 16 + lr;
                    if (red) {
                        if (lq == 0) red[(mrow0 - m0 + i * 16 + lr) * 4 + wave_n] = ncol0 < a.N ? s : make_float2(0.f, 0.f);
                    } else if (lq == 0 && m < a.M && ncol0 < a.N)
                        *reinterpret_cast<float2*>(a.stat_part + 2 * ((size_t)(ncol0 >> 6) * a.stat_stride + m)) = s;
                }
                if (a.ln_gamma) {
#pragma unroll
                    for (int jj = 0; jj < 2; ++jj) {
                        const int u0 = (ncol0 >> 1) + jj * 16 + 4 * lq;
                        if (u0 < (a.N >> 1)) acc[i][jj] = acc[i][jj] * *reinterpret_cast<const f32x4*>(a.ln_gamma + u0);
                    }
                }
            }
            staged_store_half_rows<MR, F16>(region, lane, mrow0, a.M, a.out_bf16, a.ld_out ? a.ld_out : a.N / 2, ncol0 >> 1, a.N >> 1,
                                            [&](int i, int jj) { return acc[i][jj]; });
            return;
        }
        const int which = !IS_QK ? 0 : (ncol0 >= 2 * a.dim ? 2 : (ncol0 >= a.dim ? 1 : 0));
        const float sc = (IS_QK && !which) ? a.qscale : 1.0f;
        const bool nvl = ncol0 + lc * 8 < a.N;
        const int ld = a.ld_out ? a.ld_out : a.N;
        bf16_t* qk_base = nullptr;
        int head = 0, hd_off = 0;
        if constexpr (IS_QK) {
            qk_base = which == 2 ? a.out3_bf16 : (which ? a.out2_bf16 : a.out_bf16);
            const int col = ncol0 - which * a.dim + lc * 8;
            head = col >> a.hd_log2;
            hd_off = col & ((1 << a.hd_log2) - 1);
        }
        int qb = 0, qt = 0;
        if constexpr (IS_QK) {
            qb = (mrow0 + lrow) / a.tokens;
            qt = (mrow0 + lrow) - qb * a.tokens;
        }
#pragma unroll
        for (int pass = 0; pass < 2; ++pass) {
            if (pass) __builtin_amdgcn_wave_barrier();
#pragma unroll
            for (int ii = 0; ii < 4; ++ii) {
                const int i = pass * 4 + ii;
                if (i >= MR) continue;
                epi_turn(a, wave_m, i);
                float2 st = make_float2(1.f, 0.f);
                if (fold) st = st_lds ? st_lds[mrow0 - m0 + i * 16 + lr] : row_stat(a, mrow0 + i * 16 + lr);
                f32x4 rp[4];
                bool rok = false;
                if constexpr (EPI == EPI_QK_ROPE) {
                    const int m = mrow0 + i * 16 + lr;
                    const int t = m - (m / a.tokens) * a.tokens;
                    rok = t >= 1 && t <= a.rope_tokens && which < 2;
                    const f32x4* rr = reinterpret_cast<const f32x4*>(a.rope) + (size_t)(rok ? t - 1 : 0) * 16 + lq;
#pragma unroll
                    for (int j = 0; j < 4; ++j) rp[j] = rr[j * 4];
                }
#pragma unroll
                for (int j = 0; j < 4; ++j) {
                    f32x4 v = acc[i][j] * st.x + (bv[j] - cu[j] * st.y);
                    if constexpr (EPI == EPI_QK_ROPE) {
                        if (rok)
                            v = f32x4{v[0] * rp[j][1] - v[1] * rp[j][0], v[1] * rp[j][1] + v[0] * rp[j][0],
                                      v[2] * rp[j][3] - v[3] * rp[j][2], v[3] * rp[j][3] + v[2] * rp[j][2]};
                    }
                    bf16x4 o;
                    if constexpr (EPI == EPI_GELU) {
                        const f32x4 gv = gelu_f4<FORM == 1>(v);
                        o = pack4<F16>(gv[0], gv[1], gv[2], gv[3]);
                    } else if constexpr (EPI == EPI_STAR) {
                        const f32x4 gv = star_relu4(v, a.star_scale, a.star_bias, a.star_kind);
                        o = pack4<F16>(gv[0], gv[1], gv[2], gv[3]);
                    } else
                        o = pack4<F16>(v[0] * sc, v[1] * sc, v[2] * sc, v[3] * sc);
                    Image128::put4(region, ii * 16 + lr, j, lq, o);
                }
            }
            __builtin_amdgcn_fence(__ATOMIC_RELEASE, "wavefront");
            __builtin_amdgcn_wave_barrier();
            if constexpr (EPI == EPI_GELU || EPI == EPI_STAR) {
                if (mrow0 + pass * 64 + 64 <= a.M && pass * 64 + 64 <= MR * 16 && ncol0 + 64 <= a.N) {
                    bf16_t* base = a.out_bf16 + (size_t)(mrow0 + pass * 64 + lrow) * ld + ncol0 + lc * 8;
                    uint4 v[8];
#pragma unroll
                    for (int r8 = 0; r8 < 8; ++r8) v[r8] = *reinterpret_cast<const uint4*>(Image128::at(region, r8 * 8 + lrow, lc));
#pragma unroll
                    for (int r8 = 0; r8 < 8; ++r8) *reinterpret_cast<uint4*>(base + (size_t)r8 * 8 * ld) = v[r8];
                    __builtin_amdgcn_fence(__ATOMIC_ACQUIRE, "wavefront");
                    continue;
                }
            }
            if constexpr (IS_QK) {
                if (mrow0 + pass * 64 + 64 <= a.M && pass * 64 + 64 <= MR * 16 && ncol0 + 64 <= a.N) {
                    uint4 v[8];
                    size_t off[8];
#pragma unroll
                    for (int r8 = 0; r8 < 8; ++r8) {
                        v[r8] = *reinterpret_cast<const uint4*>(Image128::at(region, r8 * 8 + lrow, lc));
                        off[r8] = ((((size_t)(qb * a.heads + head) * a.tokens_pad + qt)) << a.hd_log2) + hd_off;
                        qt += 8;
                        while (qt >= a.tokens) {
                            qt -= a.tokens;
                            ++qb;
                        }
                    }
#pragma unroll
                    for (int r8 = 0; r8 < 8; ++r8) *reinterpret_cast<uint4*>(qk_base + off[r8]) = v[r8];
                    __builtin_amdgcn_fence(__ATOMIC_ACQUIRE, "wavefront");
                    continue;
                }
            }
#pragma unroll
            for (int r8 = 0; r8 < 8; ++r8) {
                const int row = r8 * 8 + lrow;
                const int m = mrow0 + pass * 64 + row;
                const uint4 v = *reinterpret_cast<const uint4*>(Image128::at(region, row, lc));
                const int qb_now = qb, qt_now = qt;
                if constexpr (IS_QK) {
                    qt += 8;
                    while (qt >= a.tokens) {
                        qt -= a.tokens;
                        ++qb;
                    }
                }
                if (pass * 64 + row >= MR * 16 || m >= a.M || !nvl) continue;
                if constexpr (EPI == EPI_GELU || EPI == EPI_STAR) {
                    *reinterpret_cast<uint4*>(a.out_bf16 + (size_t)m * ld + ncol0 + lc * 8) = v;
                } else {
                    *reinterpret_cast<uint4*>(qk_base + ((((size_t)(qb_now * a.heads + head) * a.tokens_pad + qt_now)) << a.hd_log2) + hd_off) = v;
                }
            }
            __builtin_amdgcn_fence(__ATOMIC_ACQUIRE, "wavefront");
        }
    }
}
```

anime-illust-image-searcher_amd/csrc/gemm_plan.h:

```cpp
#pragma once
#include <algorithm>

#include "../../include/hip_tagsearch_debug.h"
#include "vit_internal.h"

namespace hipts {

struct GemmKnobs {
    int variant = HIPTSDBG_GEMM_PP;
    bool variant_set = false;
    bool auto_dw = true;
    int dw_limit4 = 2;
    unsigned dw_mask = 0;
    int min_mr = 6;
    int mr_shared = -1;
    bool persist = true;
    int raster = 8;
    int raster_gn = 6;
    int epi_prio = 0;
    int epi_prefetch = 0;
    bool resid_general = false;
    int splitk = 0, splitk_head = 0, splitk_minkt = 5;
};
const GemmKnobs& gemm_knobs();

using GemmPlan = hiptsdbg_gemm_plan_t;
int launch_gemm_q4(GemmEpilogue epi, const GemmArgs& a, const GemmPlan& p, int dev, hipStream_t s);
constexpr int GEMM_PLAN_TILE = 256, GEMM_PLAN_HALF_BN = 128, GEMM_PLAN_BK = 64;
constexpr int GEMM_PLAN_LDS = 128 * 1024, GEMM_PLAN_LDS3 = 72 * 1024;

inline bool gemm_dw_size(long tiles256, int cus, const GemmKnobs& k) { return k.auto_dw && tiles256 * 4 <= (long)cus * k.dw_limit4; }

inline GemmPlan gemm_plan(GemmEpilogue epi, const GemmArgs& a, int cus, const GemmKnobs& k, unsigned q4_mask) {
    constexpr int T = GEMM_PLAN_TILE;
    GemmPlan p{};
    p.mr = 8; p.block = 512; p.lds_bytes = GEMM_PLAN_LDS; p.sk_slices = 1;
    p.tiles_m = (a.M + T - 1) / T;
    p.tiles_n = (a.N + T - 1) / T;
    const int slots = cus >= 8 ? cus / 8 * 8 : cus;
    if (a.op8) {
        if (epi != EPI_STAR && epi != EPI_RESID && epi != EPI_RESCALE && epi != EPI_RESID_LN && epi != EPI_QK && epi != EPI_VT && epi != EPI_BIAS) {
            p.error = 2;
            return p;
        }
        p.loop = HIPTSDBG_GEMM_PP_E4M3;
        p.grid = std::min(p.tiles_m * p.tiles_n, slots);
        return p;
    }
    const bool staged_only = epi == EPI_QK_ROPE || epi == EPI_SWIGLU || epi == EPI_RESID_XG || epi == EPI_RESID_XGI;
    const bool next_ln = epi == EPI_RESID_XG || epi == EPI_RESID_XGI;
    int variant = k.variant;
    if (staged_only) variant = HIPTSDBG_GEMM_PP;
    if (epi == EPI_RESID_LN) variant = HIPTSDBG_GEMM_PP;
    if (variant == HIPTSDBG_GEMM_PP && epi != EPI_HEAD && epi != EPI_RESID_LN && (!k.variant_set || staged_only) &&
        gemm_dw_size((long)p.tiles_m * p.tiles_n, cus, k) && a.M > T && !((next_ln || epi == EPI_SWIGLU) && a.stat_part))
        variant = HIPTSDBG_GEMM_DW;
#ifdef HIPTS_X_DW_STAT
    const bool mask_stat_ok = true;
#else
    const bool mask_stat_ok = !(next_ln && a.stat_part);
#endif
    if (variant == HIPTSDBG_GEMM_PP && ((k.dw_mask >> (int)epi) & 1u) && a.M > T && mask_stat_ok) variant = HIPTSDBG_GEMM_DW;
    if (a.f16 && variant != HIPTSDBG_GEMM_PP && variant != HIPTSDBG_GEMM_DW) {
        p.error = 1;
        return p;
    }
    p.loop = variant;
    if (variant == HIPTSDBG_GEMM_DW || variant == HIPTSDBG_GEMM_S3) {
        p.tiles_n = (a.N + GEMM_PLAN_HALF_BN - 1) / GEMM_PLAN_HALF_BN;
        p.block = 256;
        p.lds_bytes = GEMM_PLAN_LDS3;
    }
    p.grid = p.tiles_m * p.tiles_n;
    if (variant == HIPTSDBG_GEMM_PP2) p.stamped = epi == EPI_GELU && a.stamps;
    if (variant != HIPTSDBG_GEMM_PP) return p;

    const int tiles_n = p.tiles_n;
    auto tiles_of = [&](int mr) { return (a.M + 32 * mr - 1) / (32 * mr); };
    auto cost_of = [&](int mr) { return ((long)tiles_of(mr) * tiles_n + cus - 1) / cus * (32 * mr); };
    int mr = 8;
    if (!a.shared_chip || k.mr_shared == 1 || (k.mr_shared != 0 && (long)tiles_of(8) * tiles_n < cus)) {
        long best = cost_of(8) * 93;
        for (int c = 7; c >= (a.f16 ? k.min_mr : std::max(k.min_mr, 7)); --c)
            if (cost_of(c) * 100 < best) {
                best = cost_of(c) * 100;
                mr = c;
            }
    }
    if (epi == EPI_HEAD && a.sk_ws && k.splitk_head >= 2) mr = 8;
    p.mr = mr;
    p.tiles_m = tiles_of(mr);
    const int ntile = p.tiles_m * tiles_n;
    p.grid = (k.persist && ntile > slots) ? slots : ntile;
    p.epi_prio = k.epi_prio;
    p.epi_prefetch = k.epi_prefetch;
    p.raster_gm = (k.raster > 0 && tiles_n >= 8) ? k.raster : 0;
    p.raster_gn = (k.raster_gn > 0 && tiles_n >= 8 && tiles_n > k.raster_gn) ? k.raster_gn : 0;
    const bool whole = epi == EPI_RESID_XG && mr == 8 && a.M % T == 0 && a.N % T == 0 && a.N <= 1024 && !a.pos && !a.res_scale && a.out_bf16 && a.stat_part;

    if (mr == 8 && ((q4_mask >> (int)epi) & 1u) && (epi == EPI_GELU || epi == EPI_QK || epi == EPI_RESID_XG) && a.sk_slices <= 1 &&
        !(a.stamps && !(a.f16 && (epi == EPI_GELU || epi == EPI_RESID_XG))) && a.M % T == 0 && a.N % T == 0 && a.K % 128 == 0 && a.K >= 128 &&
        !(epi == EPI_GELU && (a.ld_out ? a.ld_out : a.N) % 8) && !(epi == EPI_QK && a.dim % 64) &&
        (size_t)256 * a.K * 2 < ((size_t)1 << 31)) {
        p.loop = HIPTSDBG_GEMM_Q4;
        p.block = 256;
        p.grid = std::min(ntile, slots);
        p.interior = whole && !a.rowstat && !a.stat_in;
        p.stamped = a.stamps && a.f16 && (epi == EPI_GELU || p.interior);
        return p;
    }
    if (epi == EPI_RESID || next_ln || epi == EPI_RESID_ROWSTAT || epi == EPI_HEAD) {
        const int sk_max = epi == EPI_HEAD ? (p.tiles_m == 1 ? k.splitk_head : 0) : k.splitk;
        const int rem = ntile % slots;
        if (a.sk_ws && mr == 8 && sk_max >= 2 && rem > 0 && rem * 2 <= slots && rem <= 1024) {
            int sl = std::min(sk_max, std::min(slots / rem, a.K / GEMM_PLAN_BK / (k.splitk_minkt > 0 ? k.splitk_minkt : 1)));
            while (sl >= 2 && 4096 + (size_t)rem * sl * ((size_t)T * T * 4) > a.sk_ws_bytes) --sl;
            if (sl >= 2) {
                p.sk_first = ntile - rem;
                p.sk_slices = sl;
                const int items = p.sk_first + rem * sl;
                p.grid = (k.persist && items > slots) ? slots : items;
                return p;
            }
        }
    }
    p.interior = whole && !k.resid_general;
    return p;
}

}
```

anime-illust-image-searcher_amd/csrc/vit.hip:

```cpp
#include <algorithm>
#include "../../include/hip_tagsearch_debug.h"
#include <cmath>
#include <cstdlib>
#include <cstdio>
#include <cstring>
#include <string>
#include <vector>

#include "vit_internal.h"
#include "dbg_buf.h"
#include "model_host.h"
#include "prof.h"
#include "row_ln.h"
#include "patch_rows.h"

using namespace hipts;

namespace {

struct Layer {
    DevBuf ln1_g, ln1_b, ln2_g, ln2_b;
    DevBuf qkv_w, qkv_b, proj_w, proj_b, fc1_w, fc1_b, fc2_w, fc2_b;
    DevBuf qkv_u, qkv_c, fc1_u, fc1_c;
};
}

enum ProfCat { PC_PATCHIFY = 0, PC_GEMM_PATCH, PC_LAYERNORM, PC_GEMM_QK, PC_GEMM_VT, PC_ATTENTION, PC_GEMM_RESID,
               PC_GEMM_GELU, PC_POOL, PC_GEMM_HEAD, PC_OTHER, PC_COUNT };
static_assert(PC_COUNT == HIPTS_VIT_PROF_CATEGORIES, "category count");
static const char* const kProfNames[PC_COUNT] = {
    "patchify_kernel", "gemm_kernel<EPI_PATCH>", "layernorm_kernel", "gemm_kernel<EPI_QKV>", "gemm_kernel<EPI_VT>",
    "attn2_kernel", "gemm_kernel<EPI_RESID>", "gemm_kernel<EPI_GELU>", "pool_kernels", "gemm_kernel<EPI_HEAD>", "other"};

struct hipts_vit {
    bool prof = false;
    int prof_every = 0;
    uint32_t prof_mask = 0xffffffffu;
    long prof_calls = 0;
    EventProfile<PC_COUNT> ep;
    int device = 0;
    hipts_vit_config_t cfg{};
    int grid = 0, tokens = 0, tokens_pad = 0, patch_k = 0;
    std::vector<Layer> layers;
    DevBuf patch_w, patch_w2, patch_b, patch_b_u8, pos, norm_g, norm_b, head_w, head_b;
    std::vector<float> h_patch_bias, h_patch_rowsum;
    TensorLedger ledger;
    DevBuf img_in, a0, x, xn, q, k, v, att, hmid, pool_part, pooled2, logits, probs, stat_part;
    DevBuf x_rm;
    DevBuf sk_ws;
    bool fold_ln = false;
    bool fold_dirty = true;
    bool split_att = false;
    int pool_splits = 1;
    static constexpr int kMaxSub = 4;
    int want_sub = 0;
    bool deferred_join = false;
    int last_ns = 0;
    int pend_ns = 0, pend_batch = 0;
    SubStreams<kMaxSub> streams;
    hipEvent_t ev_stagger = nullptr;
};

namespace {

template <bool F16>
__global__ __launch_bounds__(256) void patchify_u8_p16_kernel(const uint8_t* __restrict__ img, bf16_t* __restrict__ a0, int size, int grid,
                                                              int xgroups) {
    __shared__ __attribute__((aligned(16))) char image[16 * 1536];
    const int tid = threadIdx.x;
    const int xg = blockIdx.x % xgroups, py = (blockIdx.x / xgroups) % grid, b = blockIdx.x / (xgroups * grid);
    const int px0 = xg * 16, ntok = min(16, grid - px0);
    const int chunks_per_row = ntok * 3;
    const int total = 16 * chunks_per_row;
    const uint8_t* src0 = img + (((int64_t)b * size + (int64_t)py * 16) * size + px0 * 16) * 3;
#pragma unroll
    for (int j = 0; j < 3; ++j) {
        const int L = j * 256 + tid;
        if (L < total) {
            const int ky = L / chunks_per_row, c16 = L - ky * chunks_per_row;
            const uint4 in = *reinterpret_cast<const uint4*>(src0 + (int64_t)ky * size * 3 + c16 * 16);
            const uint32_t w[4] = {in.x, in.y, in.z, in.w};
            bf16x8 lo, hi;
#pragma unroll
            for (int e = 0; e < 8; ++e) {
                lo[e] = to_op<F16>((float)((w[e >> 2] >> (8 * (e & 3))) & 0xffu));
                hi[e] = to_op<F16>((float)((w[2 + (e >> 2)] >> (8 * (e & 3))) & 0xffu));
            }
            const int tok = c16 / 3, part = c16 - tok * 3;
            char* d = image + tok * 1536 + ky * 96 + part * 32;
            *reinterpret_cast<bf16x8*>(d) = lo;
            *reinterpret_cast<bf16x8*>(d + 16) = hi;
        }
    }
    __syncthreads();
    const int out_chunks = ntok * 96;
    uint4* dst = reinterpret_cast<uint4*>(a0 + (((int64_t)b * grid + py) * grid + px0) * 768);
    for (int L = tid; L < out_chunks; L += 256) dst[L] = *reinterpret_cast<const uint4*>(image + L * 16);
}

__global__ __launch_bounds__(256) void pool_partial_kernel(const float* __restrict__ x, float* __restrict__ part, int tokens,
                                                           int D, float eps, int normalize, int splits) {
    __shared__ float red[4][1024];
    const int lane = threadIdx.x & 63, wave = threadIdx.x >> 6;
    const int split = blockIdx.x, b = blockIdx.y;
    const int per = (tokens + splits - 1) / splits;
    const int t0 = split * per, t1 = min(tokens, t0 + per);
    const int nvec = D >> 2;
    float4 acc[4];
#pragma unroll
    for (int i = 0; i < 4; ++i) acc[i] = make_float4(0.f, 0.f, 0.f, 0.f);
    auto load_row = [&](int t, float4 (&v)[4]) {
        const float4* xr = reinterpret_cast<const float4*>(x + ((int64_t)b * tokens + (t < t1 ? t : t1 - 1)) * D);
#pragma unroll
        for (int i = 0; i < 4; ++i) {
            const int c = lane + 64 * i;
            v[i] = c < nvec ? xr[c] : make_float4(0.f, 0.f, 0.f, 0.f);
        }
    };
    float4 vn[4];
    if (t0 + wave < t1) load_row(t0 + wave, vn);
    for (int t = t0 + wave; t < t1; t += 4) {
        float4 v[4];
#pragma unroll
        for (int i = 0; i < 4; ++i) v[i] = vn[i];
        if (t + 4 < t1) load_row(t + 4, vn);
        float mean = 0.f, rstd = 1.f;
        if (normalize) row_mean_rstd(v, lane, D, eps, mean, rstd);
#pragma unroll
        for (int i = 0; i < 4; ++i) {
            acc[i].x += (v[i].x - mean) * rstd;
            acc[i].y += (v[i].y - mean) * rstd;
            acc[i].z += (v[i].z - mean) * rstd;
            acc[i].w += (v[i].w - mean) * rstd;
        }
    }
#pragma unroll
    for (int i = 0; i < 4; ++i) {
        const int c = lane + 64 * i;
        if (c < nvec) {
            red[wave][4 * c + 0] = acc[i].x;
            red[wave][4 * c + 1] = acc[i].y;
            red[wave][4 * c + 2] = acc[i].z;
            red[wave][4 * c + 3] = acc[i].w;
        }
    }
    __syncthreads();
    for (int d = threadIdx.x; d < D; d += 256)
        part[((int64_t)b * splits + split) * D + d] = (red[0][d] + red[1][d]) + (red[2][d] + red[3][d]);
}

template <bool F16>
__global__ __launch_bounds__(256) void pool_finalize_kernel(const float* __restrict__ part, const float* __restrict__ g,
                                                            const float* __restrict__ bta, bf16_t* __restrict__ out, int tokens,
                                                            int D, float eps, int normalize_after, int splits) {
    __shared__ float feat[1024];
    __shared__ float red[8];
    const int b = blockIdx.x;
    float s = 0.f;
    for (int d = threadIdx.x; d < D; d += 256) {
        float a = 0.f;
        for (int sp = 0; sp < splits; ++sp) a += part[((int64_t)b * splits + sp) * D + d];
        a = a / (float)tokens;
        feat[d] = a;
        s += a;
    }
    float mean = 0.f, rstd = 1.f;
    if (normalize_after) {
        s = wave_sum(s);
        if ((threadIdx.x & 63) == 0) red[threadIdx.x >> 6] = s;
        __syncthreads();
        mean = ((red[0] + red[1]) + (red[2] + red[3])) / (float)D;
        float ss = 0.f;
        for (int d = threadIdx.x; d < D; d += 256) {
            const float c = feat[d] - mean;
            ss += c * c;
        }
        ss = wave_sum(ss);
        if ((threadIdx.x & 63) == 0) red[4 + (threadIdx.x >> 6)] = ss;
        __syncthreads();
        rstd = 1.0f / sqrtf(((red[4] + red[5]) + (red[6] + red[7])) / (float)D + eps);
    }
    for (int d = threadIdx.x; d < D; d += 256) {
        const float f = (feat[d] - mean) * rstd * g[d] + bta[d];
        split_hilo<F16>(f, out[(int64_t)b * 2 * D + d], out[(int64_t)b * 2 * D + D + d]);
    }
}

int launch_vit_pool(const float* x, float* part, const float* g, const float* b, bf16_t* out, int nb, int tokens, int D, float eps, bool pool_then_norm,
                    int splits, bool f16, hipStream_t s) {
    pool_partial_kernel<<<dim3(splits, nb), 256, 0, s>>>(x, part, tokens, D, eps, pool_then_norm ? 0 : 1, splits);
    HIPTS_LAUNCH_CHECK();
    HIPTS_LAUNCH_F16(f16, pool_finalize_kernel, nb, 256, 0, s, part, g, b, out, tokens, D, eps, pool_then_norm ? 1 : 0, splits);
    return HIPTS_OK;
}

}

extern "C" {

int hipts_vit_create(const hipts_vit_config_t* cfg, int device, hipts_vit_t** out) {
    HIPTS_REQUIRE(cfg && out, "hipts_vit_create: null argument");
    HIPTS_REQUIRE(cfg->patch >= 4 && cfg->image_size % cfg->patch == 0, "image_size must be a multiple of patch");
    HIPTS_REQUIRE(cfg->heads >= 1 && cfg->dim == cfg->heads * 64, "head dim must be 64 (dim = heads * 64)");
    HIPTS_REQUIRE(cfg->dim % 64 == 0 && cfg->dim <= 1024, "dim must be a multiple of 64, <= 1024");
    HIPTS_REQUIRE(cfg->mlp_dim % 64 == 0, "mlp_dim must be a multiple of 64");
    HIPTS_REQUIRE((cfg->patch * cfg->patch * 3) % 64 == 0, "patch*patch*3 must be a multiple of 64");
    HIPTS_REQUIRE(cfg->depth >= 1 && cfg->num_classes >= 1 && cfg->max_batch >= 1, "bad depth / classes / max_batch");
    const int grid = cfg->image_size / cfg->patch;
    HIPTS_REQUIRE((grid * grid) % 4 == 0, "token count must be a multiple of 4");
    HIPTS_TRY(use_device(device));
    auto* h = new hipts_vit();
    h->device = device;
    h->cfg = *cfg;
    h->grid = grid;
    h->tokens = grid * grid;
    h->tokens_pad = round_up(h->tokens, 64);
    h->patch_k = cfg->patch * cfg->patch * 3;
    h->split_att = (cfg->operand_f16 & HIPTS_OPERAND_SPLIT_ATT) != 0;
    h->layers.resize(cfg->depth);
    for (const char* s : {"patch_embed.proj.weight", "patch_embed.proj.bias", "pos_embed", "norm.weight", "norm.bias", "head.weight", "head.bias"})
        h->ledger.need(s);
    for (int i = 0; i < cfg->depth; ++i) {
        const std::string p = "blocks." + std::to_string(i) + ".";
        for (const char* s : {"norm1.weight", "norm1.bias", "attn.qkv.weight", "attn.qkv.bias", "attn.proj.weight",
                              "attn.proj.bias", "norm2.weight", "norm2.bias", "mlp.fc1.weight", "mlp.fc1.bias",
                              "mlp.fc2.weight", "mlp.fc2.bias"})
            h->ledger.need(p + s);
    }
    const size_t B = cfg->max_batch, M = B * h->tokens, D = cfg->dim;
    const size_t qkv_elems = B * cfg->heads * (size_t)h->tokens_pad * 64;
    h->pool_splits = h->tokens >= 64 ? std::min(32, std::max(8, h->tokens / 28)) : 1;
    if (getenv("HIPTS_POOL_SPLITS") && h->tokens >= 64) h->pool_splits = std::max(1, std::min(32, atoi(getenv("HIPTS_POOL_SPLITS"))));
    int st = HIPTS_OK;
    if ((st = h->a0.alloc(M * h->patch_k * 2 * 2)) || (st = h->x.alloc(M * D * 4)) || (st = h->x_rm.alloc(M * D * 4)) || (st = h->xn.alloc(M * D * 2)) ||
        (st = h->q.alloc(qkv_elems * 2)) || (st = h->k.alloc(qkv_elems * 2)) || (st = h->v.alloc(qkv_elems * 2)) ||
        (st = h->att.alloc(M * D * 2 * (h->split_att ? 2 : 1))) || (st = h->hmid.alloc(M * (size_t)cfg->mlp_dim * 2)) ||
        (st = h->pool_part.alloc(B * h->pool_splits * D * 4)) || (st = h->pooled2.alloc(B * 2 * D * 2)) ||
        (st = h->logits.alloc(B * (size_t)cfg->num_classes * 4)) || (st = h->probs.alloc(B * (size_t)cfg->num_classes * 4))) {
        delete h;
        return st;
    }
    h->fold_ln = D % 64 == 0 && h->tokens % 8 == 0 && cfg->mlp_dim % 8 == 0 && !getenv("HIPTS_GEMM") &&
                 !(getenv("HIPTS_LN_FOLD") && atoi(getenv("HIPTS_LN_FOLD")) == 0);
    if (h->fold_ln) {
        if ((st = h->stat_part.alloc(((D + 255) / 256) * M * 8))) {
            delete h;
            return st;
        }
        for (auto& L : h->layers)
            if ((st = L.qkv_u.alloc(3 * D * 4)) || (st = L.qkv_c.alloc(3 * D * 4)) || (st = L.fc1_u.alloc((size_t)cfg->mlp_dim * 4)) ||
                (st = L.fc1_c.alloc((size_t)cfg->mlp_dim * 4))) {
                delete h;
                return st;
            }
    }
    {
        hipError_t e2;
        if ((st = h->sk_ws.alloc(hipts_vit::kMaxSub * GEMM_SK_WS_BYTES)) || (e2 = hipMemset(h->sk_ws.p, 0, h->sk_ws.bytes)) != hipSuccess) {
            delete h;
            return st ? st : set_error(HIPTS_ERR_HIP, "hipMemset failed");
        }
    }
    hipError_t e;
    if ((e = hipMemset(h->q.p, 0, h->q.bytes)) != hipSuccess || (e = hipMemset(h->k.p, 0, h->k.bytes)) != hipSuccess ||
        (e = hipMemset(h->v.p, 0, h->v.bytes)) != hipSuccess) {
        delete h;
        return set_error(HIPTS_ERR_HIP, "hipMemset failed: %s", hipGetErrorString(e));
    }
    *out = h;
    return HIPTS_OK;
}

int hipts_vit_destroy(hipts_vit_t* h) {
    if (h) {
        (void)hipSetDevice(h->device);
        (void)hipDeviceSynchronize();
        if (h->ev_stagger) (void)hipEventDestroy(h->ev_stagger);
        delete h;
    }
    return HIPTS_OK;
}

int hipts_vit_set_tensor(hipts_vit_t* h, const char* key_c, const float* data, int64_t numel) {
    HIPTS_REQUIRE(h && key_c && data, "hipts_vit_set_tensor: null argument");
    HIPTS_TRY(use_device(h->device));
    const bool f16 = (h->cfg.operand_f16 & 1) != 0;
    const std::string key(key_c);
    const auto& c = h->cfg;
    const int D = c.dim, P = c.patch, Mlp = c.mlp_dim, C = c.num_classes;
#define EXPECT(n)                                                                                                      \
    HIPTS_REQUIRE(numel == (int64_t)(n), "tensor %s: expected %lld elements, got %lld", key_c, (long long)(n),         \
                  (long long)numel)
    int st = HIPTS_ERR_INVALID, li = 0;
    std::string sub;
    if (key == "patch_embed.proj.weight") {
        EXPECT((int64_t)D * 3 * P * P);
        std::vector<float> perm((size_t)D * h->patch_k);
        for (int n = 0; n < D; ++n)
            for (int ky = 0; ky < P; ++ky)
                for (int kx = 0; kx < P; ++kx)
                    for (int cr = 0; cr < 3; ++cr)
                        perm[(size_t)n * h->patch_k + (ky * P + kx) * 3 + cr] = data[(((size_t)n * 3 + (2 - cr)) * P + ky) * P + kx];
        st = upload_matrix16(h->patch_w, perm.data(), D, h->patch_k, round_up(D, 256), f16);
        if (st == HIPTS_OK) {
            h->h_patch_rowsum.assign(D, 0.f);
            for (int n = 0; n < D; ++n) {
                double rs = 0.0;
                for (int kk = 0; kk < h->patch_k; ++kk) {
                    float wv;
                    if (f16) {
                        wv = f16_bits_to_f32(f32_to_f16_rne(perm[(size_t)n * h->patch_k + kk]));
                    } else {
                        const uint32_t bits = (uint32_t)f32_to_bf16_rne(perm[(size_t)n * h->patch_k + kk]) << 16;
                        memcpy(&wv, &bits, 4);
                    }
                    rs += (double)wv;
                }
                h->h_patch_rowsum[n] = (float)rs;
            }
            st = upload_matrix16_dup(h->patch_w2, perm.data(), D, h->patch_k, round_up(D, 256), f16);
        }
    } else if (key == "patch_embed.proj.bias") {
        EXPECT(D);
        h->h_patch_bias.assign(data, data + D);
        st = upload_f32(h->patch_b, data, D);
    } else if (key == "pos_embed") {
        EXPECT((int64_t)h->tokens * D);
        st = upload_f32(h->pos, data, (size_t)h->tokens * D);
    } else if (key == "norm.weight") {
        EXPECT(D);
        st = upload_f32(h->norm_g, data, D);
    } else if (key == "norm.bias") {
        EXPECT(D);
        st = upload_f32(h->norm_b, data, D);
    } else if (key == "head.weight") {
        EXPECT((int64_t)C * D);
        st = upload_matrix16_dup(h->head_w, data, C, D, round_up(C, 256), f16);
    } else if (key == "head.bias") {
        EXPECT(C);
        st = upload_f32(h->head_b, data, C);
    } else if (parse_indexed(key, "blocks.", &li, &sub)) {
        HIPTS_REQUIRE(li >= 0 && li < c.depth, "tensor %s: block index out of range", key_c);
        Layer& L = h->layers[li];
        if (sub == "norm1.weight") { EXPECT(D); st = upload_f32(L.ln1_g, data, D); }
        else if (sub == "norm1.bias") { EXPECT(D); st = upload_f32(L.ln1_b, data, D); }
        else if (sub == "norm2.weight") { EXPECT(D); st = upload_f32(L.ln2_g, data, D); }
        else if (sub == "norm2.bias") { EXPECT(D); st = upload_f32(L.ln2_b, data, D); }
        else if (sub == "attn.qkv.weight") { EXPECT((int64_t)3 * D * D); st = upload_matrix16(L.qkv_w, data, 3 * D, D, round_up(2 * D, 256) + round_up(D, 256) + 256, f16); }
        else if (sub == "attn.qkv.bias") { EXPECT(3 * D); st = upload_f32(L.qkv_b, data, 3 * D); }
        else if (sub == "attn.proj.weight") {
            EXPECT((int64_t)D * D);
            if (h->split_att) {
                st = upload_matrix16_dup(L.proj_w, data, D, D, round_up(D, 256), f16, split_lo_scale(f16));
            } else {
                st = upload_matrix16(L.proj_w, data, D, D, round_up(D, 256), f16);
            }
        }
        else if (sub == "attn.proj.bias") { EXPECT(D); st = upload_f32(L.proj_b, data, D); }
        else if (sub == "mlp.fc1.weight") { EXPECT((int64_t)Mlp * D); st = upload_matrix16(L.fc1_w, data, Mlp, D, round_up(Mlp, 256), f16); }
        else if (sub == "mlp.fc1.bias") { EXPECT(Mlp); st = upload_f32(L.fc1_b, data, Mlp); }
        else if (sub == "mlp.fc2.weight") { EXPECT((int64_t)D * Mlp); st = upload_matrix16(L.fc2_w, data, D, Mlp, round_up(D, 256), f16); }
        else if (sub == "mlp.fc2.bias") { EXPECT(D); st = upload_f32(L.fc2_b, data, D); }
        else return set_error(HIPTS_ERR_INVALID, "unknown tensor key %s", key_c);
    } else {
        return set_error(HIPTS_ERR_INVALID, "unknown tensor key %s", key_c);
    }
#undef EXPECT
    if (st == HIPTS_OK) h->ledger.mark_set(key);
    if (st == HIPTS_OK) h->fold_dirty = true;
    if (st == HIPTS_OK && (key == "patch_embed.proj.weight" || key == "patch_embed.proj.bias") &&
        !h->h_patch_bias.empty() && !h->h_patch_rowsum.empty()) {
        std::vector<float> eff(D);
        for (int n = 0; n < D; ++n) eff[n] = (float)((double)h->h_patch_bias[n] - (double)h->h_patch_rowsum[n]);
        st = upload_f32(h->patch_b_u8, eff.data(), D);
    }
    return st;
}

int hipts_vit_profile_name(int category, char* buf, size_t n) {
    HIPTS_REQUIRE(buf && n > 0 && category >= 0 && category < PC_COUNT, "bad category");
    snprintf(buf, n, "%s", kProfNames[category]);
    return HIPTS_OK;
}

int hipts_vit_flops_per_image(const hipts_vit_t* h, double* flops) {
    HIPTS_REQUIRE(h && flops, "null argument");
    const double N = h->tokens, D = h->cfg.dim, Ml = h->cfg.mlp_dim, C = h->cfg.num_classes, Kp = h->patch_k;
    const double per_layer = 2 * N * D * 3 * D + 2 * 2 * N * N * D + 2 * N * D * D + 2 * 2 * N * D * Ml;
    *flops = 2 * N * Kp * D + h->cfg.depth * per_layer + 2 * D * C;
    return HIPTS_OK;
}

}

namespace {

struct ProfScope : EventProfile<PC_COUNT>::Scope {
    ProfScope(hipts_vit* h, hipStream_t s, int cat, double fl, double by) : Scope(h->prof && ((h->prof_mask >> cat) & 1u) ? &h->ep : nullptr, s, cat, fl, by) {}
};

int vit_run_images(hipts_vit* h, const void* in_dev, bool is_u8, int i0, int nb, float* lg, float* pr, hipStream_t s, bool shared_chip,
                   int stagger_at = 0, int sub = 0) {
    const auto& c = h->cfg;
    const int D = c.dim, P = c.patch, S = c.image_size, T = h->tokens, Tp = h->tokens_pad, H = c.heads;
    const int M = nb * T;
    const bool f16 = (c.operand_f16 & 1) != 0;
    const size_t r0 = (size_t)i0 * T;
    const int a0_ld = is_u8 ? h->patch_k : 2 * h->patch_k;
    bf16_t* a0 = h->a0.as<bf16_t>() + r0 * a0_ld;
    float* x = h->x.as<float>() + r0 * D;
    float* x_rm = h->x_rm.as<float>() + r0 * D;
    bf16_t* xn = h->xn.as<bf16_t>() + r0 * D;
    const int att_k = h->split_att ? 2 * D : D;
    bf16_t* att = h->att.as<bf16_t>() + r0 * att_k;
    bf16_t* hmid = h->hmid.as<bf16_t>() + r0 * c.mlp_dim;
    const size_t qoff = (size_t)i0 * H * Tp * 64;
    bf16_t* q = h->q.as<bf16_t>() + qoff;
    bf16_t* k = h->k.as<bf16_t>() + qoff;
    bf16_t* v = h->v.as<bf16_t>() + qoff;
    float* pool_part = h->pool_part.as<float>() + (size_t)i0 * h->pool_splits * D;
    bf16_t* pooled2 = h->pooled2.as<bf16_t>() + (size_t)i0 * 2 * D;
    const size_t img_bytes = (size_t)S * S * 3 * (is_u8 ? 1 : 4);
    const char* in_p = (const char*)in_dev + (size_t)i0 * img_bytes;

    const double dM = (double)M, dD = (double)D, dMlp = (double)c.mlp_dim, dT = (double)T;
    {
        ProfScope ps(h, s, PC_PATCHIFY, 0.0, dM * h->patch_k * (is_u8 ? 3.0 : 6.0));
        const int64_t total = (int64_t)M * P;
        const int blocks = ceil_div(total, 256);
        if (is_u8 && P == 16 && (S * 3) % 16 == 0) {
            const int xgroups = (h->grid + 15) / 16;
            const int pblocks = nb * h->grid * xgroups;
            HIPTS_LAUNCH_F16(f16, patchify_u8_p16_kernel, pblocks, 256, 0, s, (const uint8_t*)in_p, a0, S, h->grid, xgroups);
        } else if (is_u8) {
            HIPTS_LAUNCH_F16(f16, patchify_u8_kernel, blocks, 256, 0, s, (const uint8_t*)in_p, a0, nb, S, P, h->grid);
        } else {
            HIPTS_LAUNCH_F16(f16, patch_gather_kernel, blocks, 256, 0, s, PixelF32Planes<true>{(const float*)in_p}, WindowPatch{P, h->patch_k}, a0,
                             total, S, h->grid);
        }
    }
    GemmArgs g;
    g = gemm_args(f16, shared_chip);
    g.A = a0; g.M = M; g.N = D; g.out_f32 = x; g.pos = h->pos.as<float>(); g.tokens = T;
    if (is_u8) {
        g.W = h->patch_w.as<bf16_t>(); g.K = h->patch_k; g.bias = h->patch_b_u8.as<float>(); g.qscale = 2.0f / 255.0f;
    } else {
        g.W = h->patch_w2.as<bf16_t>(); g.K = 2 * h->patch_k; g.bias = h->patch_b.as<float>(); g.qscale = 1.0f;
    }
    const bool fold = h->fold_ln;
    static const bool xb_env = !(getenv("HIPTS_X_BLOCKED") && atoi(getenv("HIPTS_X_BLOCKED")) == 0);
    const bool xb = xb_env && fold && D % 16 == 0 && T % 16 == 0 && c.depth >= 1;
    const int sblocks = (D + 255) / 256;
    float* stat_p = fold ? h->stat_part.as<float>() + 2 * (size_t)sblocks * r0 : nullptr;
    {
        ProfScope ps(h, s, PC_GEMM_PATCH, 2.0 * dM * dD * h->patch_k, dM * h->patch_k * 2 + dM * dD * 4 + (fold ? dM * dD * 2 : 0.0));
        if (fold) {
            g.out_bf16 = xn; g.ln_gamma = h->layers[0].ln1_g.as<float>(); g.stat_part = stat_p; g.stat_stride = M;
            g.x_blocked = xb ? 1 : 0;
            HIPTS_TRY(launch_gemm(EPI_RESID_XG, g, s));
        } else {
            HIPTS_TRY(launch_gemm(EPI_PATCH, g, s));
        }
    }

    const int ln_blocks = ceil_div(M, 4);
    auto folded = [&](GemmArgs& ga, const float* u, const float* cvec) {
        ga.stat_in = stat_p; ga.stat_in_blocks = sblocks; ga.stat_in_stride = M; ga.ln_dim = D; ga.ln_eps = c.ln_eps;
        ga.col_u = u; ga.bias = cvec;
    };
    auto layernorm = [&](const float* gamma, const float* beta) -> int {
        ProfScope ps(h, s, PC_LAYERNORM, 0.0, dM * dD * 6);
        const LnGammaOptBeta norm{gamma, beta};
        HIPTS_LAUNCH_F16(f16, row_ln_kernel, ln_blocks, 256, 0, s, FromF32{x}, norm, To16{xn}, (int64_t)M, D, c.ln_eps);
        return HIPTS_OK;
    };
    auto residual = [&](const bf16_t* A, const bf16_t* W, const float* bias, int K, const float* next_gamma, double flops, double bytes) -> int {
        GemmArgs r = gemm_args(f16, shared_chip);
        r.A = A; r.W = W; r.M = M; r.N = D; r.K = K; r.bias = bias; r.out_f32 = x;
        r.sk_ws = h->sk_ws.as<char>() + (size_t)sub * GEMM_SK_WS_BYTES; r.sk_ws_bytes = GEMM_SK_WS_BYTES;
        r.x_blocked = xb ? 1 : 0;
        if (next_gamma) {
            r.out_bf16 = xn; r.ln_gamma = next_gamma; r.stat_part = stat_p; r.stat_stride = M;
        } else if (xb) {
            r.resid_rowmajor_out = x_rm;
        }
        {
            ProfScope ps(h, s, PC_GEMM_RESID, flops, bytes + (next_gamma ? dM * dD * 2 : 0.0));
            HIPTS_TRY(launch_gemm(next_gamma ? EPI_RESID_XG : EPI_RESID, r, s));
        }
        return HIPTS_OK;
    };
    for (int li = 0; li < c.depth; ++li) {
        Layer& L = h->layers[li];
        const bool ln1_folded = fold;
        if (!ln1_folded) HIPTS_TRY(layernorm(L.ln1_g.as<float>(), L.ln1_b.as<float>()));
        g = gemm_args(f16, shared_chip);
        g.A = xn; g.W = L.qkv_w.as<bf16_t>(); g.M = M; g.N = 3 * D; g.K = D;
        g.bias = L.qkv_b.as<float>(); g.out_bf16 = q; g.out2_bf16 = k; g.out3_bf16 = v;
        if (ln1_folded) folded(g, L.qkv_u.as<float>(), L.qkv_c.as<float>());
        g.tokens = T; g.tokens_pad = Tp; g.heads = H; g.dim = D;
        g.qscale = 0.125f * 1.4426950408889634f;
        {
            ProfScope ps(h, s, PC_GEMM_QK, 2.0 * dM * 3 * dD * dD, dM * dD * 2 + dM * 3 * dD * 2);
            HIPTS_TRY(launch_gemm(EPI_QK, g, s));
        }
        auto stagger = [&](int pos) {
            if (li == 0 && stagger_at == pos && h->ev_stagger) (void)hipEventRecord(h->ev_stagger, s);
        };
        stagger(1);
        {
            ProfScope ps(h, s, PC_ATTENTION, 4.0 * nb * H * dT * dT * 64, dM * dD * 2 * 4);
            HIPTS_TRY(launch_attention2(q, k, v, att, nb, H, T, Tp, f16, s, 0, 0, h->split_att ? 1 : 0, split_lo_scale(f16)));
        }
        stagger(2);
        HIPTS_TRY(residual(att, L.proj_w.as<bf16_t>(), L.proj_b.as<float>(), att_k, fold ? L.ln2_g.as<float>() : nullptr, 2.0 * dM * dD * att_k,
                           dM * att_k * 2 + dM * dD * 8));
        stagger(3);
        if (!fold) HIPTS_TRY(layernorm(L.ln2_g.as<float>(), L.ln2_b.as<float>()));
        g = gemm_args(f16, shared_chip);
        g.A = xn; g.W = L.fc1_w.as<bf16_t>(); g.M = M; g.N = c.mlp_dim; g.K = D;
        g.bias = L.fc1_b.as<float>(); g.out_bf16 = hmid; g.gelu_tanh = c.gelu_tanh;
        if (fold) folded(g, L.fc1_u.as<float>(), L.fc1_c.as<float>());
        {
            ProfScope ps(h, s, PC_GEMM_GELU, 2.0 * dM * dD * dMlp, dM * dD * 2 + dM * dMlp * 2);
            HIPTS_TRY(launch_gemm(EPI_GELU, g, s));
        }
        stagger(4);
        HIPTS_TRY(residual(hmid, L.fc2_w.as<bf16_t>(), L.fc2_b.as<float>(), c.mlp_dim,
                           (fold && li + 1 < c.depth) ? h->layers[li + 1].ln1_g.as<float>() : nullptr, 2.0 * dM * dD * dMlp,
                           dM * dMlp * 2 + dM * dD * 8));
        stagger(5);
    }
    {
        ProfScope ps(h, s, PC_POOL, 0.0, dM * dD * 4);
        HIPTS_TRY(launch_vit_pool(xb ? x_rm : x, pool_part, h->norm_g.as<float>(), h->norm_b.as<float>(), pooled2, nb, T, D, c.ln_eps, c.pool_then_norm != 0,
                                  h->pool_splits, f16, s));
    }
    g = gemm_args(f16, shared_chip);
    g.A = pooled2; g.W = h->head_w.as<bf16_t>(); g.M = nb; g.N = c.num_classes; g.K = 2 * D;
    g.sk_ws = h->sk_ws.as<char>() + (size_t)sub * GEMM_SK_WS_BYTES; g.sk_ws_bytes = GEMM_SK_WS_BYTES;
    g.bias = h->head_b.as<float>(); g.out_f32 = lg ? lg + (size_t)i0 * c.num_classes : nullptr;
    g.out2_f32 = pr ? pr + (size_t)i0 * c.num_classes : nullptr;
    {
        ProfScope ps(h, s, PC_GEMM_HEAD, 2.0 * nb * dD * c.num_classes, (double)c.num_classes * 2 * dD * 2);
        HIPTS_TRY(launch_gemm(EPI_HEAD, g, s));
    }
    return HIPTS_OK;
}

int vit_forward_impl(hipts_vit* h, const void* input, int in_memspace, bool is_u8, int batch, float* logits_out,
                     float* probs_out, int out_memspace, hipStream_t s) {
    HIPTS_REQUIRE(h && input && batch >= 1, "hipts_vit_forward: bad arguments");
    HIPTS_REQUIRE(batch <= h->cfg.max_batch, "batch %d exceeds max_batch %d", batch, h->cfg.max_batch);
    HIPTS_TRY(h->ledger.require_complete("hipts_vit_forward"));
    HIPTS_TRY(use_device(h->device));
    h->prof = h->prof_every > 0 && (h->prof_calls++ % h->prof_every) == 0;
    const auto& c = h->cfg;
    const int S = c.image_size;

    static const int want_streams = getenv("HIPTS_VIT_STREAMS") ? atoi(getenv("HIPTS_VIT_STREAMS")) : 2;
    const int ns = std::min({h->want_sub > 0 ? h->want_sub : want_streams, (int)hipts_vit::kMaxSub, batch / 8});
    if (h->pend_ns > 0 && (h->pend_ns != ns || h->pend_batch != batch || in_memspace != HIPTS_DEVICE))
        for (int i = 0; i < h->pend_ns; ++i) HIPTS_HIP(hipStreamWaitEvent(s, h->streams.ev_join[i], 0));
    h->pend_ns = 0;

    const void* in_dev = nullptr;
    HIPTS_TRY(stage_input(h->img_in, input, in_memspace, (size_t)batch * S * S * 3 * (is_u8 ? 1 : 4), s, &in_dev));
    const bool dev_out = out_memspace == HIPTS_DEVICE;
    float* lg = (dev_out && logits_out) ? logits_out : h->logits.as<float>();
    float* pr = (probs_out || !dev_out) ? ((dev_out && probs_out) ? probs_out : h->probs.as<float>()) : nullptr;
    if (h->fold_ln && h->fold_dirty) {
        const bool f16w = (c.operand_f16 & 1) != 0;
        for (auto& L : h->layers) {
            HIPTS_TRY(launch_fold_ln(L.qkv_w.as<bf16_t>(), f16w, L.ln1_g.as<float>(), L.ln1_b.as<float>(), L.qkv_b.as<float>(), L.qkv_u.as<float>(),
                                     L.qkv_c.as<float>(), 3 * c.dim, c.dim, s));
            HIPTS_TRY(launch_fold_ln(L.fc1_w.as<bf16_t>(), f16w, L.ln2_g.as<float>(), L.ln2_b.as<float>(), L.fc1_b.as<float>(), L.fc1_u.as<float>(),
                                     L.fc1_c.as<float>(), c.mlp_dim, c.dim, s));
        }
        h->fold_dirty = false;
    }

    if (ns >= 2) {
        if (!h->streams.ev_fork) HIPTS_HIP(hipEventCreateWithFlags(&h->streams.ev_fork, hipEventDisableTiming));
        for (int i = 0; i < ns; ++i)
            if (!h->streams.sub[i]) {
                HIPTS_HIP(hipStreamCreateWithFlags(&h->streams.sub[i], hipStreamNonBlocking));
                if (!h->streams.ev_join[i]) HIPTS_HIP(hipEventCreateWithFlags(&h->streams.ev_join[i], hipEventDisableTiming));
            }
        HIPTS_HIP(hipEventRecord(h->streams.ev_fork, s));
        static const int stagger_at = getenv("HIPTS_VIT_STAGGER") ? atoi(getenv("HIPTS_VIT_STAGGER")) : 0;
        if (stagger_at > 0 && !h->ev_stagger) HIPTS_HIP(hipEventCreateWithFlags(&h->ev_stagger, hipEventDisableTiming));
        for (int i = 0; i < ns; ++i) {
            const int i0 = (int)((int64_t)batch * i / ns), i1 = (int)((int64_t)batch * (i + 1) / ns);
            HIPTS_HIP(hipStreamWaitEvent(h->streams.sub[i], h->streams.ev_fork, 0));
            if (i > 0 && stagger_at > 0) HIPTS_HIP(hipStreamWaitEvent(h->streams.sub[i], h->ev_stagger, 0));
            HIPTS_TRY(vit_run_images(h, in_dev, is_u8, i0, i1 - i0, lg, pr, h->streams.sub[i], true, i == 0 ? stagger_at : 0, i));
            HIPTS_HIP(hipEventRecord(h->streams.ev_join[i], h->streams.sub[i]));
            if (!h->deferred_join || !dev_out) HIPTS_HIP(hipStreamWaitEvent(s, h->streams.ev_join[i], 0));
        }
        h->last_ns = (h->deferred_join && dev_out) ? ns : 0;
        h->pend_ns = h->last_ns;
        h->pend_batch = batch;
    } else {
        HIPTS_TRY(vit_run_images(h, in_dev, is_u8, 0, batch, lg, pr, s, false));
        h->last_ns = 0;
        if (h->deferred_join && dev_out) {
            if (!h->streams.ev_join[0]) HIPTS_HIP(hipEventCreateWithFlags(&h->streams.ev_join[0], hipEventDisableTiming));
            HIPTS_HIP(hipEventRecord(h->streams.ev_join[0], s));
            h->last_ns = 1;
        }
    }
    if (!dev_out) HIPTS_TRY(read_back(s, (size_t)batch * c.num_classes * 4, logits_out, lg, probs_out, pr));
    return HIPTS_OK;
}

}

namespace hipts {
namespace {
__global__ __launch_bounds__(256) void rowstat_kernel(const float2* __restrict__ part, float2* __restrict__ rowstat, int M, int stride, int blocks,
                                                      int D, float eps) {
    const int q = threadIdx.x >> 6;
    const int m = blockIdx.x * 64 + (threadIdx.x & 63);
    __shared__ float2 red[4][64];
    float s1 = 0.f, s2 = 0.f;
    if (m < M) {
#pragma unroll 4
        for (int b = q; b < blocks; b += 4) {
            const float2 v = part[(size_t)b * stride + m];
            s1 += v.x;
            s2 += v.y;
        }
    }
    red[q][threadIdx.x & 63] = make_float2(s1, s2);
    __syncthreads();
    if (q != 0 || m >= M) return;
    const float2 a = red[0][threadIdx.x], b2 = red[1][threadIdx.x], c = red[2][threadIdx.x], d = red[3][threadIdx.x];
    s1 = (a.x + b2.x) + (c.x + d.x);
    s2 = (a.y + b2.y) + (c.y + d.y);
    const float mean = s1 / (float)D;
    const float var = fmaxf(s2 / (float)D - mean * mean, 0.f);
    const float rstd = 1.0f / sqrtf(var + eps);
    rowstat[m] = make_float2(rstd, rstd * mean);
}

template <bool F16>
__global__ __launch_bounds__(256) void fold_ln_kernel(const bf16_t* __restrict__ W, const float* __restrict__ gamma, const float* __restrict__ beta,
                                                      const float* __restrict__ bias, float* __restrict__ u, float* __restrict__ c, int N, int K) {
    const int lane = threadIdx.x & 63;
    const int n = blockIdx.x * 4 + (threadIdx.x >> 6);
    if (n >= N) return;
    double su = 0.0, sc = 0.0;
    for (int k = lane; k < K; k += 64) {
        const double w = (double)from_op<F16>(W[(size_t)n * K + k]);
        su += w * (double)gamma[k];
        if (beta) sc += w * (double)beta[k];
    }
#pragma unroll
    for (int o = 32; o >= 1; o >>= 1) {
        su += __shfl_xor(su, o);
        sc += __shfl_xor(sc, o);
    }
    if (lane == 0) {
        u[n] = (float)su;
        c[n] = (float)(sc + (bias ? (double)bias[n] : 0.0));
    }
}
}

int launch_rowstat(const float* part, float* rowstat, int M, int stride, int blocks, int D, float eps, hipStream_t s) {
    rowstat_kernel<<<(M + 63) / 64, 256, 0, s>>>(reinterpret_cast<const float2*>(part), reinterpret_cast<float2*>(rowstat), M, stride, blocks, D, eps);
    HIPTS_LAUNCH_CHECK();
    return HIPTS_OK;
}
// ... 380 lines not shown
    HIPTS_TRY(upload(dv.p, vT, nqk * 2));
    HIPTS_HIP(hipMemset(dout.p, 0, nout * 2));
    HIPTS_TRY(launch_attention(dq.as<bf16_t>(), dk.as<bf16_t>(), dv.as<bf16_t>(), dout.as<bf16_t>(), batch, heads, tokens, tokens_pad, f16 != 0, nullptr,
                               head_dim, 0));
    HIPTS_HIP(hipDeviceSynchronize());
    HIPTS_HIP(hipMemcpy(out_host, dout.p, nout * 2, hipMemcpyDeviceToHost));
    return HIPTS_OK;
}

extern "C" int hiptsdbg_attention_time(const uint16_t* q, const uint16_t* k, const uint16_t* vT, int batch, int heads, int tokens, int tokens_pad,
                                       int head_dim, int f16, int iters, double* avg_us) {
    HIPTS_REQUIRE(q && k && vT && avg_us && batch >= 1 && heads >= 1 && tokens >= 1 && iters >= 1, "hiptsdbg_attention_time: bad arguments");
    HIPTS_TRY(use_device(0));
    const size_t nqk = (size_t)batch * heads * tokens_pad * head_dim, nout = (size_t)batch * tokens * heads * head_dim;
    DevBuf dq, dk, dv, dout;
    HIPTS_TRY(dq.alloc(nqk * 2));
    HIPTS_TRY(dk.alloc(nqk * 2));
    HIPTS_TRY(dv.alloc(nqk * 2));
    HIPTS_TRY(dout.alloc(nout * 2));
    HIPTS_TRY(upload(dq.p, q, nqk * 2));
    HIPTS_TRY(upload(dk.p, k, nqk * 2));
    HIPTS_TRY(upload(dv.p, vT, nqk * 2));
    hipEvent_t e0, e1;
    HIPTS_HIP(hipEventCreate(&e0));
    HIPTS_HIP(hipEventCreate(&e1));
    int rc = HIPTS_OK;
    for (int i = 0; i < 3 && rc == HIPTS_OK; ++i)
        rc = launch_attention(dq.as<bf16_t>(), dk.as<bf16_t>(), dv.as<bf16_t>(), dout.as<bf16_t>(), batch, heads, tokens, tokens_pad, f16 != 0, nullptr, head_dim, 0);
    HIPTS_HIP(hipEventRecord(e0, nullptr));
    for (int i = 0; i < iters && rc == HIPTS_OK; ++i)
        rc = launch_attention(dq.as<bf16_t>(), dk.as<bf16_t>(), dv.as<bf16_t>(), dout.as<bf16_t>(), batch, heads, tokens, tokens_pad, f16 != 0, nullptr, head_dim, 0);
    HIPTS_HIP(hipEventRecord(e1, nullptr));
    HIPTS_HIP(hipEventSynchronize(e1));
    float ms = 0.f;
    HIPTS_HIP(hipEventElapsedTime(&ms, e0, e1));
    (void)hipEventDestroy(e0);
    (void)hipEventDestroy(e1);
    *avg_us = 1e3 * ms / iters;
    return rc;
}

extern "C" int hiptsdbg_attention2(const uint16_t* q, const uint16_t* k, const uint16_t* v, uint16_t* out_host, int batch, int heads, int tokens,
                                   int tokens_pad, int f16, int variant, int iters, double* avg_us) {
    HIPTS_REQUIRE(q && k && v && batch >= 1 && heads >= 1 && tokens >= 1 && (iters > 0 ? avg_us != nullptr : out_host != nullptr), "hiptsdbg_attention2: bad arguments");
    HIPTS_TRY(use_device(0));
    const size_t nqk = (size_t)batch * heads * tokens_pad * 64, nout = (size_t)batch * tokens * heads * 64;
    DevBuf dq, dk, dv, dout;
    HIPTS_TRY(dq.alloc(nqk * 2));
    HIPTS_TRY(dk.alloc(nqk * 2));
    HIPTS_TRY(dv.alloc(nqk * 2));
    HIPTS_TRY(dout.alloc(nout * 2));
    HIPTS_TRY(upload(dq.p, q, nqk * 2));
    HIPTS_TRY(upload(dk.p, k, nqk * 2));
    HIPTS_TRY(upload(dv.p, v, nqk * 2));
    HIPTS_HIP(hipMemset(dout.p, 0, nout * 2));
    auto run = [&]() { return launch_attention2(dq.as<bf16_t>(), dk.as<bf16_t>(), dv.as<bf16_t>(), dout.as<bf16_t>(), batch, heads, tokens, tokens_pad, f16 != 0, nullptr, 0, variant); };
    if (iters <= 0) {
        HIPTS_TRY(run());
        HIPTS_HIP(hipDeviceSynchronize());
        HIPTS_HIP(hipMemcpy(out_host, dout.p, nout * 2, hipMemcpyDeviceToHost));
        return HIPTS_OK;
    }
    hipEvent_t e0, e1;
    HIPTS_HIP(hipEventCreate(&e0));
    HIPTS_HIP(hipEventCreate(&e1));
    int rc = HIPTS_OK;
    for (int i = 0; i < 3 && rc == HIPTS_OK; ++i) rc = run();
    HIPTS_HIP(hipEventRecord(e0, nullptr));
    for (int i = 0; i < iters && rc == HIPTS_OK; ++i) rc = run();
    HIPTS_HIP(hipEventRecord(e1, nullptr));
    HIPTS_HIP(hipEventSynchronize(e1));
    float ms = 0.f;
    HIPTS_HIP(hipEventElapsedTime(&ms, e0, e1));
    (void)hipEventDestroy(e0);
    (void)hipEventDestroy(e1);
    *avg_us = 1e3 * ms / iters;
    return rc;
}

extern "C" int hiptsdbg_attention2_launch(const uint16_t* q, const uint16_t* k, const uint16_t* v, uint16_t* out_host, long long out_rows, int batch,
                                          int heads, int tokens, int tokens_pad, int f16, int out_tokens_stride, int variant, int split_lo) {
    HIPTS_REQUIRE(q && k && v && out_host && batch >= 1 && heads >= 1 && tokens >= 1 && tokens_pad >= tokens, "hiptsdbg_attention2_launch: bad arguments");
    HIPTS_REQUIRE(out_tokens_stride == 0 || out_tokens_stride >= tokens, "hiptsdbg_attention2_launch: out_tokens_stride %d below tokens %d",
                  out_tokens_stride, tokens);
    const long long stride = out_tokens_stride > 0 ? out_tokens_stride : tokens;
    HIPTS_REQUIRE(out_rows >= (long long)batch * stride, "hiptsdbg_attention2_launch: %lld output rows, the launch covers %lld", out_rows,
                  (long long)batch * stride);
    HIPTS_TRY(use_device(0));
    const size_t nqk = (size_t)batch * heads * tokens_pad * 64, nout = (size_t)out_rows * (split_lo ? 2 : 1) * heads * 64;
    DevBuf dq, dk, dv, dout;
    HIPTS_TRY(dq.alloc(nqk * 2));
    HIPTS_TRY(dk.alloc(nqk * 2));
    HIPTS_TRY(dv.alloc(nqk * 2));
    HIPTS_TRY(dout.alloc(nout * 2));
    HIPTS_TRY(upload(dq.p, q, nqk * 2));
    HIPTS_TRY(upload(dk.p, k, nqk * 2));
    HIPTS_TRY(upload(dv.p, v, nqk * 2));
    HIPTS_HIP(hipMemset(dout.p, 0xFF, nout * 2));
    HIPTS_TRY(launch_attention2(dq.as<bf16_t>(), dk.as<bf16_t>(), dv.as<bf16_t>(), dout.as<bf16_t>(), batch, heads, tokens, tokens_pad, f16 != 0, nullptr,
                                out_tokens_stride, variant, split_lo ? 1 : 0, split_lo_scale(f16 != 0)));
    HIPTS_HIP(hipDeviceSynchronize());
    HIPTS_HIP(hipMemcpy(out_host, dout.p, nout * 2, hipMemcpyDeviceToHost));
    return HIPTS_OK;
}

extern "C" int hiptsdbg_attention2_kernel_resources(int tokens_pad, int f16, int variant, int* num_regs, int* scratch_bytes, int* static_lds) {
    HIPTS_REQUIRE(num_regs && scratch_bytes && static_lds && tokens_pad >= 64 && tokens_pad % 64 == 0, "hiptsdbg_attention2_kernel_resources: bad arguments");
    HIPTS_TRY(use_device(0));
    return attention2_kernel_resources(tokens_pad, f16 != 0, variant, num_regs, scratch_bytes, static_lds);
}

extern "C" int hiptsdbg_attention2_stamps(unsigned long long* host, int n) { return attention2_read_stamps(host, n); }

extern "C" int hiptsdbg_vit_patchify_u8_p16(const uint8_t* images, int batch, int grid, int f16, int fill, uint16_t* a0, uint64_t a0_bytes) {
    HIPTS_REQUIRE(images && a0 && batch >= 1 && batch <= 64 && grid >= 1 && grid <= 64, "hiptsdbg_vit_patchify_u8_p16: bad argument");
    const int S = 16 * grid, xgroups = (grid + 15) / 16;
    const uint64_t need = (uint64_t)batch * grid * grid * 768 * 2;
    HIPTS_REQUIRE(a0_bytes >= need, "hiptsdbg_vit_patchify_u8_p16: a0 has %llu bytes, the launch's extent is %llu", (unsigned long long)a0_bytes,
                  (unsigned long long)need);
    HIPTS_TRY(use_device(0));
    DevBuf img, ad;
    HIPTS_TRY(img.alloc((size_t)batch * S * S * 3));
    HIPTS_TRY(upload(img.p, images, (size_t)batch * S * S * 3));
    HIPTS_TRY(ad.alloc(a0_bytes));
    HIPTS_HIP(hipMemset(ad.p, fill & 0xff, a0_bytes));
    HIPTS_LAUNCH_F16(f16 != 0, patchify_u8_p16_kernel, batch * grid * xgroups, 256, 0, nullptr, img.as<uint8_t>(), ad.as<bf16_t>(), S, grid, xgroups);
    HIPTS_HIP(hipDeviceSynchronize());
    HIPTS_HIP(hipMemcpy(a0, ad.p, a0_bytes, hipMemcpyDeviceToHost));
    return HIPTS_OK;
}

extern "C" int hiptsdbg_vit_pool(const float* x, uint64_t x_bytes, const float* g, const float* b, int batch, int tokens, int D, float eps, int pool_then_norm,
                                 int splits, int f16, int fill, float* part_out, uint64_t part_bytes, uint16_t* out16, uint64_t out16_bytes) {
    const char* who = "hiptsdbg_vit_pool";
    HIPTS_REQUIRE(x && g && b && part_out && out16, "%s: null argument", who);
    HIPTS_REQUIRE(batch >= 1 && batch <= 4096 && tokens >= 1 && tokens <= (1 << 16), "%s: unsupported shape", who);
    HIPTS_REQUIRE(D >= 4 && D % 4 == 0 && D <= 1024, "%s: D=%d must be a multiple of 4, at most 1024", who, D);
    HIPTS_REQUIRE(splits >= 1 && splits <= 32, "%s: splits=%d outside 1..32", who, splits);
    HIPTS_REQUIRE(x_bytes >= (uint64_t)batch * tokens * D * 4, "%s: x does not cover the launch", who);
    HIPTS_TRY(use_device(0));
    DevBuf xd, gd, bd, pd, od;
    HIPTS_TRY(dbg_guarded(pd, part_bytes, (uint64_t)batch * splits * D * 4, fill, who, "partial"));
    HIPTS_TRY(dbg_guarded(od, out16_bytes, (uint64_t)batch * 2 * D * 2, fill, who, "hi | lo"));
    HIPTS_TRY(dbg_put(xd, x, x_bytes));
    HIPTS_TRY(dbg_put(gd, g, (size_t)D * 4));
    HIPTS_TRY(dbg_put(bd, b, (size_t)D * 4));
    HIPTS_TRY(launch_vit_pool(xd.as<float>(), pd.as<float>(), gd.as<float>(), bd.as<float>(), od.as<bf16_t>(), batch, tokens, D, eps, pool_then_norm != 0, splits,
                              f16 != 0, nullptr));
    HIPTS_HIP(hipDeviceSynchronize());
    HIPTS_TRY(dbg_fetch(part_out, pd, part_bytes, who));
    return dbg_fetch(out16, od, out16_bytes, who);
}

extern "C" int hiptsdbg_vit_dump(hipts_vit_t* h, const char* name, void* out_host, size_t max_bytes, size_t* bytes) {
    HIPTS_REQUIRE(h && name && out_host && bytes, "null argument");
    HIPTS_TRY(use_device(h->device));
    const std::string n(name);
    const DevBuf* b = n == "a0" ? &h->a0 : n == "x" ? &h->x : n == "xn" ? &h->xn : n == "q" ? &h->q : n == "k" ? &h->k
                      : n == "v" ? &h->v : n == "att" ? &h->att : n == "hmid" ? &h->hmid : n == "pool_part" ? &h->pool_part
                      : n == "pooled2" ? &h->pooled2 : nullptr;
    HIPTS_REQUIRE(b, "unknown buffer %s", name);
    *bytes = b->bytes < max_bytes ? b->bytes : max_bytes;
    HIPTS_HIP(hipDeviceSynchronize());
    HIPTS_HIP(hipMemcpy(out_host, b->p, *bytes, hipMemcpyDeviceToHost));
    return HIPTS_OK;
}
```

anime-illust-image-searcher_amd/csrc/vit_internal.h:

```cpp
#pragma once
#include <cmath>
#include <cstring>
#include <vector>

#include "common.h"

namespace hipts {

typedef __bf16 bf16_t;
typedef __bf16 bf16x8 __attribute__((ext_vector_type(8)));
typedef __bf16 bf16x4 __attribute__((ext_vector_type(4)));
typedef _Float16 f16x8 __attribute__((ext_vector_type(8)));
typedef _Float16 f16x4 __attribute__((ext_vector_type(4)));
typedef float f32x4 __attribute__((ext_vector_type(4)));
typedef float f32x16 __attribute__((ext_vector_type(16)));
typedef int i32x8 __attribute__((ext_vector_type(8)));

template <bool F16>
__device__ __forceinline__ bf16x4 pack4(float a, float b, float c, float d) {
    if constexpr (F16) {
        f16x4 h;
        h[0] = (_Float16)a; h[1] = (_Float16)b; h[2] = (_Float16)c; h[3] = (_Float16)d;
        return __builtin_bit_cast(bf16x4, h);
    } else {
// ... 19 lines not shown
}
template <bool F16>
__device__ __forceinline__ f32x16 mfma_32x32x16(bf16x8 a, bf16x8 b, f32x16 c) {
    if constexpr (F16) return __builtin_amdgcn_mfma_f32_32x32x16_f16(__builtin_bit_cast(f16x8, a), __builtin_bit_cast(f16x8, b), c, 0, 0, 0);
    else return __builtin_amdgcn_mfma_f32_32x32x16_bf16(a, b, c, 0, 0, 0);
}

__host__ __device__ __forceinline__ int xcd_work_id(int id, int n) {
    const int q = n >> 3, r = n & 7, xcd = id & 7, loc = id >> 3;
    return (xcd < r ? xcd * (q + 1) : r * (q + 1) + (xcd - r) * q) + loc;
}

__device__ __forceinline__ uint32_t pack4_e4m3(float a, float b, float c, float d) {
    a = __builtin_amdgcn_fmed3f(a, -448.0f, 448.0f);
    b = __builtin_amdgcn_fmed3f(b, -448.0f, 448.0f);
    c = __builtin_amdgcn_fmed3f(c, -448.0f, 448.0f);
    d = __builtin_amdgcn_fmed3f(d, -448.0f, 448.0f);
    int p = __builtin_amdgcn_cvt_pk_fp8_f32(a, b, 0, false);
    p = __builtin_amdgcn_cvt_pk_fp8_f32(c, d, p, true);
    return (uint32_t)p;
}
__device__ __forceinline__ f32x4 mfma_16x16x128_e4m3(i32x8 a, i32x8 b, f32x4 c, int scale_a, int scale_b) {
    return __builtin_amdgcn_mfma_scale_f32_16x16x128_f8f6f4(a, b, c, 0, 0, 0, scale_a, 0, scale_b);
}

inline uint8_t f32_to_e4m3_rne(float f) {
    uint32_t u;
    memcpy(&u, &f, 4);
    const uint8_t sign = (uint8_t)((u >> 24) & 0x80u);
    u &= 0x7fffffffu;
    if (u > 0x7f800000u) return (uint8_t)(sign | 0x7f);
    float a;
    memcpy(&a, &u, 4);
    if (a >= 448.0f) return (uint8_t)(sign | 0x7e);
    if (a < 0.0009765625f) return sign;
    int e;
    (void)frexpf(a, &e);
    int ex = e - 1;
    if (ex < -6) ex = -6;
    const float q = ldexpf(1.0f, ex - 3);
    const float n = nearbyintf(a / q);
    float v = n * q;
    if (v >= 448.0f) return (uint8_t)(sign | 0x7e);
    if (v < 0.015625f) return (uint8_t)(sign | (uint8_t)n);
    int e2;
    const float m2 = frexpf(v, &e2);
    const int bexp = e2 - 1 + 7;
    const int mant = (int)((m2 * 2.0f - 1.0f) * 8.0f);
    return (uint8_t)(sign | (bexp << 3) | mant);
}
inline float e4m3_bits_to_f32(uint8_t v) {
    const int s = v >> 7, e = (v >> 3) & 15, m = v & 7;
    float f;
    if (e == 15 && m == 7) {
        const uint32_t qnan = 0x7fc00000u;
        memcpy(&f, &qnan, 4);
    } else if (e == 0) f = ldexpf((float)m, -9);
    else f = ldexpf(1.0f + (float)m / 8.0f, e - 7);
    return s ? -f : f;
}
inline uint16_t f32_to_bf16_rne(float f) {
    uint32_t u;
    memcpy(&u, &f, 4);
    if ((u & 0x7fffffffu) > 0x7f800000u) return (uint16_t)((u >> 16) | 0x40);
    u += 0x7fffu + ((u >> 16) & 1u);
    return (uint16_t)(u >> 16);
}

inline uint16_t f32_to_f16_rne(float f) {
    uint32_t x;
    memcpy(&x, &f, 4);
    const uint32_t sign = (x >> 16) & 0x8000u;
    x &= 0x7fffffffu;
    if (x >= 0x7f800000u) return (uint16_t)(sign | 0x7c00u | (x > 0x7f800000u ? 0x200u : 0));
    if (x >= 0x477ff000u) return (uint16_t)(sign | 0x7c00u);
    if (x < 0x38800000u) {
        if (x < 0x33000000u) return (uint16_t)sign;
        const int shift = 126 - (int)(x >> 23);
        uint32_t mant = (x & 0x7fffffu) | 0x800000u;
        const uint32_t round = (1u << (shift - 1)) - 1 + ((mant >> shift) & 1u);
        mant += round;
        return (uint16_t)(sign | (mant >> shift));
    }
    const uint32_t round = 0xfffu + ((x >> 13) & 1u);
    x += round;
    return (uint16_t)(sign | ((x - 0x38000000u) >> 13));
}
inline float f16_bits_to_f32(uint16_t h) {
    const uint32_t sign = (uint32_t)(h & 0x8000u) << 16;
    uint32_t e = (h >> 10) & 0x1f, m = h & 0x3ffu, out;
    if (e == 0) {
        if (m == 0) out = sign;
        else {
            int sh = 0;
            while (!(m & 0x400u)) { m <<= 1; ++sh; }
            out = sign | ((uint32_t)(113 - sh) << 23) | ((m & 0x3ffu) << 13);
        }
    } else if (e == 31) out = sign | 0x7f800000u | (m << 13);
    else out = sign | ((e + 112) << 23) | (m << 13);
    float f;
    memcpy(&f, &out, 4);
    return f;
}

inline int round_up(int x, int m) { return (x + m - 1) / m * m; }

inline int upload_matrix16(DevBuf& buf, const float* data, int rows, int cols, int rows_pad, bool f16) {
    std::vector<uint16_t> h((size_t)rows_pad * cols, 0);
    if (f16) for (size_t i = 0; i < (size_t)rows * cols; ++i) h[i] = f32_to_f16_rne(data[i]);
    else for (size_t i = 0; i < (size_t)rows * cols; ++i) h[i] = f32_to_bf16_rne(data[i]);
    HIPTS_TRY(buf.alloc(h.size() * 2));
    return upload(buf.p, h.data(), h.size() * 2);
}

inline int upload_matrix8(DevBuf& buf, const float* data, int rows, int cols, int rows_pad, int* w_exp) {
    float mx = 0.f;
    for (size_t i = 0; i < (size_t)rows * cols; ++i) mx = fmaxf(mx, fabsf(data[i]));
    int e = 0;
    if (mx > 0.f && std::isfinite(mx)) {
        e = (int)floorf(log2f(448.0f / mx));
        if (ldexpf(mx, e) > 448.0f) --e;
        e = e > 100 ? 100 : (e < -100 ? -100 : e);
    }
    std::vector<uint8_t> h((size_t)rows_pad * cols, 0);
    for (size_t i = 0; i < (size_t)rows * cols; ++i) h[i] = f32_to_e4m3_rne(ldexpf(data[i], e));
    *w_exp = e;
    HIPTS_TRY(buf.alloc(h.size()));
    return upload(buf.p, h.data(), h.size());
}

enum GemmEpilogue {
    EPI_PATCH = 0,
    EPI_QK = 1,
    EPI_VT = 2,
    EPI_RESID = 3,
    EPI_GELU = 4,
    EPI_HEAD = 5,
    EPI_STAR = 6,
    EPI_RESCALE = 7,
    EPI_BIAS = 8,
    EPI_QK_ROPE = 10,
    EPI_SWIGLU = 11,
    EPI_RESID_ROWSTAT = 12,
    EPI_RESID_XG = 13,
    EPI_RESID_XGI = 14,
    EPI_RESID_LS = 15,
    EPI_RESID_LN = 9
};

struct GemmArgs {
    const bf16_t* A;
    const bf16_t* W;
    int M, N, K;
    const float* bias;
    float* out_f32 = nullptr;
    float* out2_f32 = nullptr;
    bf16_t* out_bf16 = nullptr;
    bf16_t* out2_bf16 = nullptr;
    bf16_t* out3_bf16 = nullptr;
    const float* pos = nullptr;
    int tokens = 0;
    int tokens_pad = 0;
    int heads = 0, dim = 0;
    int hd_log2 = 6;
    const float* res_scale = nullptr;
    const float* ln_gamma = nullptr;
    const float* ln_beta = nullptr;
    float ln_eps = 1e-6f;
    float star_scale = 1.0f, star_bias = 0.0f;
    int star_kind = 0;
    float qscale = 1.0f;
    float* stat_part = nullptr;
    int stat_stride = 0;
    const float* stat_in = nullptr;
    int stat_in_blocks = 0;
    int stat_in_stride = 0;
    int ln_dim = 0;
    const float* rowstat = nullptr;
    const float* col_u = nullptr;
    const float* rope = nullptr;
    int rope_tokens = 0;
    int gelu_tanh = 1;
    int ld_out = 0;
    int f16 = 0;
    int op8 = 0;
    int w_exp = 0;
    int out8 = 0;
    void* sk_ws = nullptr;
    size_t sk_ws_bytes = 0;
    int sk_first = 0, sk_slices = 1;
    int raster_gn = 0;
    int raster_gm = 0;
    int x_blocked = 0;
    float* resid_rowmajor_out = nullptr;
    int epi_prefetch = 0;
    int epi_prio = 0;
    int shared_chip = 0;
    int trace = 0;
    unsigned long long* stamps = nullptr;
};

int launch_gemm(GemmEpilogue epi, const GemmArgs& a, hipStream_t s);
constexpr unsigned GEMM_Q4_DEFAULT_MASK = 0u;
void set_gemm_q4_mask(unsigned mask);
long long gemm_q4_launch_count();
constexpr size_t GEMM_SK_WS_BYTES = 4096 + 256 * (size_t)(256 * 256 * 4);

int launch_attention(const bf16_t* q, const bf16_t* k, const bf16_t* vT, bf16_t* out, int batch, int heads, int tokens,
                     int tokens_pad, bool f16, hipStream_t s, int head_dim = 64, int out_tokens_stride = 0);

int launch_attention2(const bf16_t* q, const bf16_t* k, const bf16_t* v, bf16_t* out, int batch, int heads, int tokens, int tokens_pad, bool f16,
                      hipStream_t s, int out_tokens_stride = 0, int variant = 0, int split_lo = 0, float lo_scale = 1.0f);
inline float split_lo_scale(bool f16) {
    static const float env = getenv("HIPTS_SPLIT_LO_SCALE") ? (float)atof(getenv("HIPTS_SPLIT_LO_SCALE")) : 0.0f;
    if (env > 0.0f) return env;
    return f16 ? 64.0f : 1.0f;
}

int attention2_kernel_resources(int tokens_pad, bool f16, int variant, int* num_regs, int* scratch_bytes, int* static_lds);

int attention2_read_stamps(unsigned long long* host, int n);

int launch_swin_attention(const float* qkv, const float* logit_scale, const float* cpb, bf16_t* out, int batch, int side, int window,
                          int shift, int heads, bool f16, hipStream_t s);

int launch_layernorm(const float* x, const float* g, const float* b, bf16_t* out, int64_t rows, int D, float eps, bool f16,
                     hipStream_t s);
int launch_rowstat(const float* part, float* rowstat, int M, int stride, int blocks, int D, float eps, hipStream_t s);
int launch_fold_ln(const bf16_t* W, bool f16, const float* gamma, const float* beta, const float* bias, float* u, float* c, int N, int K,
                   hipStream_t s);
std::vector<uint16_t> mlp_weight_image(const float* w1, const float* w2, int C);
bool mlp_fused_supports(int C);
int launch_mlp_fused(const bf16_t* xn, const void* wimg, float* x, const float* res_scale, const float* gamma, bf16_t* xn_out, int M, int C,
                     float star_s, float star_b, float eps, hipStream_t s, int waves = 0,
                     int xblk = 0);
int launch_layernorm8(const float* x, const float* g, const float* b, uint8_t* out, int64_t rows, int D, float eps, hipStream_t s);

}
```

include/hip_tagsearch_debug.h:

```cpp
#ifndef HIP_TAGSEARCH_DEBUG_H
#define HIP_TAGSEARCH_DEBUG_H

#include <stddef.h>
#include <stdint.h>

#include "hip_tagsearch.h"

#ifdef __cplusplus
extern "C" {
#endif

int hiptsdbg_gemm_time(int M, int N, int K, int epi, int iters, float* ms_out);
int hiptsdbg_gemm_clock(int M, int N, int K, int epi, int iters, float* ms_out, float* loop_ghz);
int hiptsdbg_gemm_q4_compare(int M, int N, int K, int epi, int f16, int iters, long long* mismatch_out, float* ms_out);
int hiptsdbg_gelu(const float* x_host, int n, int tanh_form, float* y_host);
int hiptsdbg_dwconv7(const uint16_t* in_f16, const float* w, uint16_t* out_f16, int batch, int H, int C, int mode, int iters, float* ms_out);
int hiptsdbg_dwconv7_stamps(unsigned long long* host, int n);
int hiptsdbg_convnext_stream(hipts_convnext_t* h, const float* x_host, int batch, int stage, float* out_host);
int hiptsdbg_swinv2_stream(hipts_swinv2_t* h, const float* x_host, int batch, int stage, float* out_host);
int hiptsdbg_swinv2_window_attention(const float* q, const float* k, const float* v, const float* logit_scale, const float* cpb, int batch,
                                     int heads, int side, int window, int shift, int operand_f16, float* out);
int hiptsdbg_mlp_fused(const uint16_t* xn, const float* w1, const float* w2, float* x, const float* res_scale, const float* gamma, uint16_t* xn_out,
                       int M, int C, float star_s, float star_b, float eps, int iters, float* ms_out, int waves);
int hiptsdbg_mlp_stamps(unsigned long long* host, int n);
int hiptsdbg_mlp_weight_image(const float* w1, const float* w2, int C, uint16_t* out, long long out_halves);
int hiptsdbg_dw_toeplitz(const float* w, int channels, uint32_t* out);
enum { HIPTSDBG_GEMM_V1 = 0, HIPTSDBG_GEMM_PP = 1, HIPTSDBG_GEMM_S3 = 2, HIPTSDBG_GEMM_PP2 = 3, HIPTSDBG_GEMM_DW = 4,
       HIPTSDBG_GEMM_Q4 = 5, HIPTSDBG_GEMM_PP_E4M3 = 6 };
typedef struct hiptsdbg_gemm_plan_t {
    int32_t loop, mr, interior, stamped;
    int32_t tiles_m, tiles_n, grid, block, lds_bytes;
    int32_t sk_first, sk_slices;
    int32_t raster_gm, raster_gn, epi_prio, epi_prefetch;
    int32_t error;
} hiptsdbg_gemm_plan_t;
int hiptsdbg_gemm_plan(int epi, int M, int N, int K, int f16, int shared_chip, unsigned features, int ld_out, int dim, int cus,
                       unsigned q4_mask, hiptsdbg_gemm_plan_t* out);
int hiptsdbg_gemm_tile_walk(int tiles_m, int tiles_n, int tile_rows, int raster_gm, int raster_gn, int32_t* m0, int32_t* n0);
int hiptsdbg_gemm_kernel_resources(int epi, int mr, int f16, int op8, int sk, int interior, int* num_regs, int* scratch_bytes, int* static_lds);
typedef struct hiptsdbg_gemm_case_t {
    int32_t epi, M, N, K, f16, shared_chip;
    const uint16_t* a;
    const uint16_t* w;
    const float* bias;
    const float* pos;
    const float* res_scale;
    const float* ln_gamma;
    const float* ln_beta;
    const float* col_u;
    const float* rowstat;
    const float* stat_in;
    const float* rope;
    const float* x_init;
    uint64_t x_init_bytes;
    int32_t tokens, tokens_pad, heads, dim, hd_log2;
    int32_t stat_in_blocks, stat_in_stride, ln_dim, rope_tokens, stat_stride;
    int32_t gelu_tanh, star_kind, ld_out, x_blocked, sk_ws, fill;
    float qscale, ln_eps, star_scale, star_bias;
} hiptsdbg_gemm_case_t;
typedef struct hiptsdbg_gemm_out_t {
    void* x;
    void* rowmajor;
    void* probs;
    void* out16[3];
    void* stat_part;
    uint64_t x_bytes, rowmajor_bytes, probs_bytes, out16_bytes[3], stat_part_bytes;
} hiptsdbg_gemm_out_t;
int hiptsdbg_gemm_epilogue(const hiptsdbg_gemm_case_t* in, hiptsdbg_gemm_out_t* out);
enum { HIPTSDBG_SRC_F32 = 0, HIPTSDBG_SRC_F32_BLOCKED = 1, HIPTSDBG_SRC_F32_INPLACE = 2, HIPTSDBG_SRC_16_BIAS = 3 };
enum { HIPTSDBG_AFF_GAMMA_BETA = 0, HIPTSDBG_AFF_GAMMA_OPT_BETA = 1, HIPTSDBG_AFF_GAMMA_ADD_ZERO = 2, HIPTSDBG_AFF_GAMMA_PLAIN = 3 };
enum { HIPTSDBG_SINK_16 = 0, HIPTSDBG_SINK_E4M3 = 1, HIPTSDBG_SINK_F32 = 2, HIPTSDBG_SINK_F32_AND_16 = 3, HIPTSDBG_SINK_PATCH2X2 = 4,
       HIPTSDBG_SINK_ADD_HILO = 5, HIPTSDBG_SINK_BACK = 6 };
typedef struct hiptsdbg_row_ln_case_t {
    int32_t src, affine, sink, f16, blk, H, D, fill;
    int64_t rows;
    float eps;
    const void* in;
    uint64_t in_bytes;
    const float* bias;
    const float* g;
    const float* b;
    const float* x_init;
    uint64_t x_init_bytes;
} hiptsdbg_row_ln_case_t;
typedef struct hiptsdbg_rows_out_t {
    void* f32;
    void* o16;
    uint64_t f32_bytes, o16_bytes;
} hiptsdbg_rows_out_t;
int hiptsdbg_row_ln(const hiptsdbg_row_ln_case_t* in, hiptsdbg_rows_out_t* out);
int hiptsdbg_pool_ln(const float* x, uint64_t x_bytes, const float* g, const float* b, int batch, int T, int C, int count, int blk, float eps,
                     int hilo, int f16, int fill, void* out, uint64_t out_bytes);
int hiptsdbg_rowstat(const float* part, uint64_t part_bytes, int M, int stride, int blocks, int D, float eps, int fill, float* out, uint64_t out_bytes);
int hiptsdbg_fold_ln(const uint16_t* w16, int f16, const float* gamma, const float* beta, const float* bias, int N, int K, int fill, float* u, float* c,
                     uint64_t out_bytes);
enum { HIPTSDBG_PIX_U8_AFFINE = 0, HIPTSDBG_PIX_U8_TABLE = 1, HIPTSDBG_PIX_F32_FLIP = 2, HIPTSDBG_PIX_F32 = 3, HIPTSDBG_PIX_U8_RAW = 4 };
enum { HIPTSDBG_WIN_PATCH = 0, HIPTSDBG_WIN_4X4 = 1, HIPTSDBG_WIN_7X7 = 2 };
int hiptsdbg_patch_gather(int pixel, int window, int f16, const void* images, uint64_t image_bytes, const float* lut, int batch, int S, int P,
                          int KH, int fill, uint16_t* a0, uint64_t a0_bytes);
int hiptsdbg_ccip_stem_u8(const uint8_t* images, const float* lut, int batch, int S, int f16, int fill, uint16_t* a0, uint64_t a0_bytes);
int hiptsdbg_vit_patchify_u8_p16(const uint8_t* images, int batch, int grid, int f16, int fill, uint16_t* a0, uint64_t a0_bytes);
int hiptsdbg_vit_pool(const float* x, uint64_t x_bytes, const float* g, const float* b, int batch, int tokens, int D, float eps, int pool_then_norm,
                      int splits, int f16, int fill, float* part_out, uint64_t part_bytes, uint16_t* out16, uint64_t out16_bytes);
int hiptsdbg_eva_assemble(const float* tmp, uint64_t tmp_bytes, const float* cls, const float* pos, int batch, int np, int TS, int D, int blocked, int fill,
                          float* x, uint64_t x_bytes, float* xblk, uint64_t xblk_bytes);
int hiptsdbg_eva_colsum(const float* x, uint64_t x_bytes, int batch, int np, int TS, int D, int fill, float* part, uint64_t part_bytes);
int hiptsdbg_swinv2_merge(const float* x, uint64_t x_bytes, int batch, int H, int C, int f16, int fill, uint16_t* col, uint64_t col_bytes);
int hiptsdbg_swinv2_split_x(const float* x, uint64_t x_bytes, int64_t rows, int D, int f16, int fill, uint16_t* xh2, uint64_t xh2_bytes);
int hiptsdbg_swinv2_mean(const float* y, uint64_t y_bytes, int batch, int T, int C, int f16, int fill, uint16_t* out, uint64_t out_bytes);
int hiptsdbg_ccip_ds_im2col(const uint16_t* xn, uint64_t xn_bytes, int batch, int H, int C, int fill, uint16_t* col, uint64_t col_bytes);
int hiptsdbg_convnext_cast(const float* x, uint64_t x_bytes, int64_t n4, int f16, int fill, uint16_t* xh, uint64_t xh_bytes);
int hiptsdbg_gemm_run(int M, int N, int K, const uint16_t* a_bf16, const uint16_t* w_bf16, float* out_host);
int hiptsdbg_gemm8_run(int M, int N, int K, const float* a_f32, const float* w_f32, int kind, void* out_host, int* w_exp);
int hiptsdbg_vit_dump(hipts_vit_t* h, const char* name, void* out_host, size_t max_bytes, size_t* bytes);

int hiptsdbg_attention_run(const uint16_t* q, const uint16_t* k, const uint16_t* vT, uint16_t* out_host, int batch, int heads, int tokens,
                           int tokens_pad, int head_dim, int f16);
int hiptsdbg_attention_time(const uint16_t* q, const uint16_t* k, const uint16_t* vT, int batch, int heads, int tokens, int tokens_pad,
                            int head_dim, int f16, int iters, double* avg_us);

int hiptsdbg_attention2(const uint16_t* q, const uint16_t* k, const uint16_t* v, uint16_t* out_host, int batch, int heads, int tokens, int tokens_pad,
                        int f16, int variant, int iters, double* avg_us);

int hiptsdbg_attention2_launch(const uint16_t* q, const uint16_t* k, const uint16_t* v, uint16_t* out_host, long long out_rows, int batch, int heads,
                               int tokens, int tokens_pad, int f16, int out_tokens_stride, int variant, int split_lo);

int hiptsdbg_attention2_kernel_resources(int tokens_pad, int f16, int variant, int* num_regs, int* scratch_bytes, int* static_lds);

int hiptsdbg_attention2_stamps(unsigned long long* host, int n);

int hiptsdbg_search1_last(hipts_bm25_t* h, uint32_t* candidates, uint32_t* took_candidate_path);
enum { HIPTSDBG_QUERY_FINISH = 1, HIPTSDBG_QUERY_WIDE = 2, HIPTSDBG_QUERY_TILED = 4, HIPTSDBG_QUERY_PARTS = 8, HIPTSDBG_QUERY_DEFAULT = 15 };
typedef struct hiptsdbg_search1_plan_t {
    int64_t waves;
    int32_t kk, gw, gl, groups, bcap, finish;
    int32_t grid_score, blocks2, blocks3, reserved;
    uint64_t off_wmax, off_bcnt, off_bflag, off_bkey, off_bid, off_wit, ws_bytes;
    uint64_t out_bytes, off_flag;
} hiptsdbg_search1_plan_t;
int hiptsdbg_search1_plan(int64_t D, int k, unsigned knob_bits, hiptsdbg_search1_plan_t* out);
typedef struct hiptsdbg_sim_plan_t {
    int32_t wide_passes, wide_grid, last_n, last_nqb, last_grid;
    int32_t tail_q0, tail_passes, tail_grid, tail_tiled;
    int32_t parts_grid, index_passes, reserved;
    uint64_t parts_bytes;
} hiptsdbg_sim_plan_t;
int hiptsdbg_sim_plan(int have_tiled, int64_t D, int K, int nq, int want_parts, unsigned knob_bits, hiptsdbg_sim_plan_t* out);
int hiptsdbg_topk_stamps(unsigned long long* host16);
int hiptsdbg_related_last(const hipts_bm25_t* h, double* count_ms, int64_t* lds_items, int64_t* direct_items);
int hiptsdbg_radius_passes(const hipts_radius_t* h, double* pass1_ms, double* pass2_ms, double* sort_ms);

#ifdef __cplusplus
}
#endif
#endif
```

Before: 5465 images/sec.

## Store MLP hidden activation in 16x16 blocked layout between FC1 and FC2 GEMMs

The FC1 GELU epilogue can now write the MLP hidden activation in a 16x16-blocked layout, and the FC2 residual GEMM reads its A operand from that layout through new blocked staging and chunk-offset addressing. The goal is for each 16-byte global-to-LDS load and each epilogue store to touch contiguous 512-byte blocks rather than rows strided by the full K, which should improve memory coalescing. When blocked mode is on, these GEMMs lose the DW variant, the q4 path and split-K, which could cost speed on some shapes. The mode is on by default when LN folding is active and the shapes are multiples of 16.

```diff
diff --git a/anime-illust-image-searcher_amd/csrc/act_blocked.h b/anime-illust-image-searcher_amd/csrc/act_blocked.h
--- /dev/null
+++ b/anime-illust-image-searcher_amd/csrc/act_blocked.h
@@ -0,0 +1,19 @@
+#pragma once
+#include <cstddef>
+#include <cstdint>
+
+namespace hipts {
+
+inline size_t act_blocked_index(size_t row, size_t col, size_t ld) {
+    return (((row >> 4) * (ld >> 4) + (col >> 4)) << 8) + ((row & 15) << 4) + (col & 15);
+}
+inline void act_block(const uint16_t* rowmajor, uint16_t* blocked, size_t rows, size_t ld) {
+    for (size_t r = 0; r < rows; ++r)
+        for (size_t c = 0; c < ld; ++c) blocked[act_blocked_index(r, c, ld)] = rowmajor[r * ld + c];
+}
+inline void act_unblock(const uint16_t* blocked, uint16_t* rowmajor, size_t rows, size_t ld) {
+    for (size_t r = 0; r < rows; ++r)
+        for (size_t c = 0; c < ld; ++c) rowmajor[r * ld + c] = blocked[act_blocked_index(r, c, ld)];
+}
+
+}
diff --git a/anime-illust-image-searcher_amd/csrc/gemm.hip b/anime-illust-image-searcher_amd/csrc/gemm.hip
--- a/anime-illust-image-searcher_amd/csrc/gemm.hip
+++ b/anime-illust-image-searcher_amd/csrc/gemm.hip
@@ -92,8 +92,10 @@
     }
 }
 
-template <int EPI, int MR = 8, bool F16 = false, bool OP8 = false, bool SK = false, bool INT = false>
+template <int EPI, int MR = 8, bool F16 = false, bool OP8 = false, bool SK = false, bool INT = false, bool ABLK = false, bool OBLK = false>
 __global__ __launch_bounds__(512) __attribute__((amdgpu_num_vgpr(240))) void gemm_pp_kernel(const GemmArgs a, int tiles_m, int tiles_n) {
+    static_assert(!(ABLK || OBLK) || (!OP8 && !SK), "blocked activations: 16-bit operands, no split-K");
+    static_assert(!OBLK || EPI == EPI_GELU, "blocked 16-bit output: the GELU epilogue");
     static_assert(!INT || (EPI == EPI_RESID_XG && MR == 8 && !OP8 && !SK), "INT: the residual epilogue's interior form");
     static_assert(!OP8 || (F16 && MR == 8), "e4m3 operands: half 16-bit outputs, full tiles");
     static_assert(!SK || (!OP8 && MR == 8), "split-K: 16-bit operands, full tiles");
@@ -110,6 +112,7 @@
     const int nwg = tiles_m * tiles_n;
     const int K = OP8 ? a.K / 2 : a.K, nt_all = K / BK;
     const int w_rows = tiles_n * BN;
+    constexpr int a_kstep = ABLK ? ACT_KTILE_STEP : BK;
     const int S = SK ? a.sk_slices : 1;
     const int n_items = SK ? a.sk_first + (nwg - a.sk_first) * S : nwg;
     auto decode = [&](int item, WorkItem& w) {
@@ -141,6 +144,9 @@
     tile_origin<TBM>(a, wi.tile, tiles_m, tiles_n, m0, n0);
     int par = 0;
 
+    if constexpr (ABLK) {
+        if (wave * 4 < 4 * MR) stage_tile_blocked(a.A, a.M, K, m0, wi.kt0, smem, wave, lane);
+    } else
     if (wave * 4 < 4 * MR) stage_tile(a.A, a.M, K, m0, wi.kt0, smem, wave, lane);
     stage_tile(a.W, w_rows, K, n0, wi.kt0, smem + TILE_BYTES, wave, lane);
     if constexpr (INT) {
@@ -164,6 +170,9 @@
                 const int lim = isW ? w_rows : a.M;
                 grow = grow < lim ? grow : lim - 1;
                 src[idx] = (isW ? a.W : a.A) + (size_t)grow * K + (size_t)(wi.kt0 + 1) * BK + chunk * 8;
+                if constexpr (ABLK) {
+                    if (!isW) src[idx] = a.A + act_chunk_off(grow, K, wi.kt0 + 1, chunk);
+                }
                 dst[idx] = (isW ? TILE_BYTES : 0) + rb8 * 1024;
             };
             for (int u = 0; u < 2; ++u) {
@@ -206,7 +215,7 @@
             char* st1 = smem + ((par + 1) & 1) * STAGE_BYTES;
             for (int k : {4, 5, 0, 1}) {
                 glds16(src[k], st1 + dst[k]);
-                src[k] += BK;
+                src[k] += k >= 4 ? a_kstep : BK;
             }
         }
 
@@ -243,7 +252,7 @@
                 if (more) {
                     auto issue = [&](int k) {
                         glds16(src[k], nxt + dst[k]);
-                        src[k] += BK;
+                        src[k] += k >= 4 ? a_kstep : BK;
                     };
                     if (HIPTS_STAGE_ORDER_OLD) {
                         issue(2 * p);
@@ -265,7 +274,7 @@
                             if (t + 2 < wi.nt) {
                                 for (int k : {4, 5, 0, 1}) {
                                     glds16(src[k], const_cast<char*>(cur) + dst[k]);
-                                    src[k] += BK;
+                                    src[k] += k >= 4 ? a_kstep : BK;
                                 }
                                 wait_vmcnt(n_hi + 4);
                             } else {
@@ -344,6 +353,9 @@
             decode(next, wi_next);
             tile_origin<TBM>(a, wi_next.tile, tiles_m, tiles_n, m0n, n0n);
             char* st = smem + par_next * STAGE_BYTES;
+            if constexpr (ABLK) {
+                if (wave * 4 < 4 * MR) stage_tile_blocked(a.A, a.M, K, m0n, wi_next.kt0, st, wave, lane);
+            } else
             if (wave * 4 < 4 * MR) stage_tile(a.A, a.M, K, m0n, wi_next.kt0, st, wave, lane);
             stage_tile(a.W, w_rows, K, n0n, wi_next.kt0, st + TILE_BYTES, wave, lane);
         }
@@ -404,7 +416,7 @@
             if constexpr (staged_epilogue_built(EPI)) {
                 if (staged_epilogue_ok(EPI, a)) {
                     float2* red = (EPI == EPI_SWIGLU && a.stat_part) ? sw_red : nullptr;
-                    gemm_epilogue_staged<EPI, MR, F16>(a, acc, m0, n0, wave_m, wave_n, elane, smem + ((par + wi.nt + 1) & 1) * STAGE_BYTES + wave * 8192, bias_pre,
+                    gemm_epilogue_staged<EPI, MR, F16, -1, OBLK>(a, acc, m0, n0, wave_m, wave_n, elane, smem + ((par + wi.nt + 1) & 1) * STAGE_BYTES + wave * 8192, bias_pre,
                                                        fold_st ? st_table : nullptr, red);
                     staged = true;
                     if constexpr (EPI == EPI_SWIGLU) {
@@ -837,7 +849,28 @@
 
 using GemmKernel = void (*)(const GemmArgs, int, int);
 template <int EPI>
-GemmKernel pp_kernel(int mr, bool f16, bool op8, bool sk, bool interior) {
+GemmKernel pp_kernel(int mr, bool f16, bool op8, bool sk, bool interior, bool ablk = false, bool oblk = false) {
+    if (ablk || oblk) {
+        if (op8 || sk || (ablk && oblk)) return nullptr;
+        if constexpr (EPI == EPI_GELU) {
+            if (oblk && !interior) {
+                if (f16) return mr == 6 ? gemm_pp_kernel<EPI, 6, true, false, false, false, false, true> : mr == 7 ? gemm_pp_kernel<EPI, 7, true, false, false, false, false, true>
+                                : mr == 8 ? gemm_pp_kernel<EPI, 8, true, false, false, false, false, true> : nullptr;
+                return mr == 7 ? gemm_pp_kernel<EPI, 7, false, false, false, false, false, true> : mr == 8 ? gemm_pp_kernel<EPI, 8, false, false, false, false, false, true> : nullptr;
+            }
+        }
+        if constexpr (EPI == EPI_RESID_XG) {
+            if (ablk && interior && mr == 8) return f16 ? gemm_pp_kernel<EPI, 8, true, false, false, true, true> : gemm_pp_kernel<EPI, 8, false, false, false, true, true>;
+        }
+        if constexpr (EPI == EPI_RESID_XG || EPI == EPI_RESID) {
+            if (ablk && !interior) {
+                if (f16) return mr == 6 ? gemm_pp_kernel<EPI, 6, true, false, false, false, true> : mr == 7 ? gemm_pp_kernel<EPI, 7, true, false, false, false, true>
+                                : mr == 8 ? gemm_pp_kernel<EPI, 8, true, false, false, false, true> : nullptr;
+                return mr == 7 ? gemm_pp_kernel<EPI, 7, false, false, false, false, true> : mr == 8 ? gemm_pp_kernel<EPI, 8, false, false, false, false, true> : nullptr;
+            }
+        }
+        return nullptr;
+    }
     if (op8) {
         if constexpr (EPI == EPI_STAR || EPI == EPI_RESID || EPI == EPI_RESCALE || EPI == EPI_RESID_LN || EPI == EPI_QK || EPI == EPI_VT || EPI == EPI_BIAS)
             if (mr == 8 && f16 && !sk && !interior) return gemm_pp_kernel<EPI, 8, true, true>;
@@ -858,10 +891,10 @@
 }
 
 template <int EPI>
-int kernel_resources_t(int mr, bool f16, bool op8, bool sk, bool interior, int* num_regs, int* scratch_bytes, int* static_lds) {
-    const GemmKernel k = pp_kernel<EPI>(mr, f16, op8, sk, interior);
-    HIPTS_REQUIRE(k != nullptr, "hiptsdbg_gemm_kernel_resources: no gemm_pp_kernel is built for epilogue %d, mr %d, f16 %d, op8 %d, sk %d, interior %d", EPI, mr,
-                  (int)f16, (int)op8, (int)sk, (int)interior);
+int kernel_resources_t(int mr, bool f16, bool op8, bool sk, bool interior, int* num_regs, int* scratch_bytes, int* static_lds, bool ablk = false, bool oblk = false) {
+    const GemmKernel k = pp_kernel<EPI>(mr, f16, op8, sk, interior, ablk, oblk);
+    HIPTS_REQUIRE(k != nullptr, "hiptsdbg_gemm_kernel_resources: no gemm_pp_kernel is built for epilogue %d, mr %d, f16 %d, op8 %d, sk %d, interior %d, blocked A %d / output %d",
+                  EPI, mr, (int)f16, (int)op8, (int)sk, (int)interior, (int)ablk, (int)oblk);
     hipFuncAttributes at;
     HIPTS_HIP(hipFuncGetAttributes(&at, reinterpret_cast<const void*>(k)));
     *num_regs = at.numRegs;
@@ -927,6 +960,15 @@
             break;
         }
         default: {
+            if (a.a_blocked || a.out16_blocked) {
+                const GemmKernel k = pp_kernel<EPI>(p.mr, f16, false, false, p.interior != 0, a.a_blocked != 0, a.out16_blocked != 0);
+                HIPTS_REQUIRE(k != nullptr, "gemm: no kernel for blocked 16-bit activations is built for epilogue %d (A %d, output %d, %d-row tiles)", EPI, a.a_blocked,
+                              a.out16_blocked, 32 * p.mr);
+                static PerDevice once[8];
+                HIPTS_TRY(allow_dynamic_lds(once[(p.mr - 6) * 2 + (f16 ? 1 : 0) + (p.interior ? 2 : 0)], dev, p.lds_bytes, k));
+                go(k);
+                break;
+            }
             if constexpr (EPI == EPI_RESID || EPI == EPI_RESID_XG || EPI == EPI_RESID_XGI || EPI == EPI_RESID_ROWSTAT || EPI == EPI_HEAD) {
                 if (p.sk_slices >= 2) {
                     static PerDevice once;
@@ -1020,6 +1062,10 @@
         HIPTS_REQUIRE(a.N % 64 == 0 && (a.ld_out ? a.ld_out : a.N / 2) % 8 == 0 && a.out_bf16, "gemm: SWIGLU needs N %% 64 == 0 and an output stride that is a multiple of 8");
     if (epi == EPI_RESCALE) HIPTS_REQUIRE(a.res_scale != nullptr, "gemm: RESCALE epilogue needs res_scale");
     if (epi == EPI_RESID_LS) HIPTS_REQUIRE(a.res_scale && a.out_f32 && !a.x_blocked, "gemm: RESID_LS needs the layer scale and the row-major fp32 stream");
+    if (a.a_blocked) HIPTS_REQUIRE(!a.out16_blocked && !a.op8 && a.M % 16 == 0, "gemm: a blocked A operand needs 16-bit elements and M %% 16 == 0 (M = %d)", a.M);
+    if (a.out16_blocked)
+        HIPTS_REQUIRE(epi == EPI_GELU && !a.op8 && a.M % 16 == 0 && (a.ld_out ? a.ld_out : a.N) % 16 == 0 && (a.ld_out ? a.ld_out : a.N) >= a.N,
+                      "gemm: a blocked 16-bit output is built for the GELU epilogue, M %% 16 == 0 and a row stride that is a multiple of 16");
     if (epi == EPI_RESID_LN)
         HIPTS_REQUIRE(a.N <= BN && a.ln_gamma && a.out_bf16 && a.out_f32, "gemm: RESID_LN needs the whole row in one tile (N <= %d), gamma and both outputs", BN);
     switch (epi) {
@@ -1084,6 +1130,18 @@
     return set_error(HIPTS_ERR_INVALID, "hiptsdbg_gemm_kernel_resources: unknown epilogue");
 }
 
+extern "C" int hiptsdbg_gemm_kernel_resources_blocked(int epi, int mr, int f16, int interior, int a_blocked, int out16_blocked, int* num_regs, int* scratch_bytes,
+                                                      int* static_lds) {
+    using namespace hipts;
+    HIPTS_REQUIRE(num_regs && scratch_bytes && static_lds, "hiptsdbg_gemm_kernel_resources_blocked: bad argument");
+    HIPTS_TRY(use_device(0));
+    const bool ab = a_blocked != 0, ob = out16_blocked != 0;
+    if (epi == EPI_GELU) return kernel_resources_t<EPI_GELU>(mr, f16 != 0, false, false, interior != 0, num_regs, scratch_bytes, static_lds, ab, ob);
+    if (epi == EPI_RESID_XG) return kernel_resources_t<EPI_RESID_XG>(mr, f16 != 0, false, false, interior != 0, num_regs, scratch_bytes, static_lds, ab, ob);
+    if (epi == EPI_RESID) return kernel_resources_t<EPI_RESID>(mr, f16 != 0, false, false, interior != 0, num_regs, scratch_bytes, static_lds, ab, ob);
+    return set_error(HIPTS_ERR_INVALID, "hiptsdbg_gemm_kernel_resources_blocked: no blocked kernel is built for epilogue %d", epi);
+}
+
 extern "C" int hiptsdbg_gemm_plan(int epi, int M, int N, int K, int f16, int shared_chip, unsigned features, int ld_out, int dim, int cus,
                                   unsigned q4_mask, hiptsdbg_gemm_plan_t* out) {
     using namespace hipts;
diff --git a/anime-illust-image-searcher_amd/csrc/gemm_dbg.hip b/anime-illust-image-searcher_amd/csrc/gemm_dbg.hip
--- a/anime-illust-image-searcher_amd/csrc/gemm_dbg.hip
+++ b/anime-illust-image-searcher_amd/csrc/gemm_dbg.hip
@@ -1,6 +1,7 @@
 #include <vector>
 
 #include "../../include/hip_tagsearch_debug.h"
+#include "act_blocked.h"
 #include "vit_internal.h"
 
 namespace hipts {
@@ -34,11 +35,26 @@
     return HIPTS_OK;
 }
 
+int gemm_epilogue_case(const hiptsdbg_gemm_case_t* in, hiptsdbg_gemm_out_t* out, bool a_blocked, bool out16_blocked);
+
 }
 }
 
-extern "C" int hiptsdbg_gemm_epilogue(const hiptsdbg_gemm_case_t* in, hiptsdbg_gemm_out_t* out) {
+extern "C" int hiptsdbg_gemm_epilogue(const hiptsdbg_gemm_case_t* in, hiptsdbg_gemm_out_t* out) { return hipts::gemm_epilogue_case(in, out, false, false); }
+extern "C" int hiptsdbg_gemm_epilogue_blocked(const hiptsdbg_gemm_case_t* in, hiptsdbg_gemm_out_t* out, int a_blocked, int out16_blocked) {
+    return hipts::gemm_epilogue_case(in, out, a_blocked != 0, out16_blocked != 0);
+}
+extern "C" int hiptsdbg_act_block(const uint16_t* in, uint16_t* out, int64_t rows, int64_t ld, int unblock) {
     using namespace hipts;
+    HIPTS_REQUIRE(in && out && in != out && rows >= 0 && ld >= 0 && rows % 16 == 0 && ld % 16 == 0, "hiptsdbg_act_block: rows and ld must be multiples of 16, in != out");
+    if (unblock) act_unblock(in, out, (size_t)rows, (size_t)ld);
+    else act_block(in, out, (size_t)rows, (size_t)ld);
+    return HIPTS_OK;
+}
+
+namespace hipts {
+namespace {
+int gemm_epilogue_case(const hiptsdbg_gemm_case_t* in, hiptsdbg_gemm_out_t* out, bool a_blocked, bool out16_blocked) {
     HIPTS_REQUIRE(in && out && in->a && in->w, "hiptsdbg_gemm_epilogue: null argument");
     const int epi = in->epi, M = in->M, N = in->N, K = in->K;
     HIPTS_REQUIRE(epi >= EPI_PATCH && epi <= EPI_RESID_LS && M >= 1 && N >= 1 && K >= 64 && K % 64 == 0 && (long long)M * K < (1ll << 31) &&
@@ -135,6 +151,7 @@
     g.tokens = in->tokens; g.tokens_pad = in->tokens_pad; g.heads = in->heads; g.dim = in->dim; g.hd_log2 = in->hd_log2;
     g.stat_in_blocks = in->stat_in_blocks; g.stat_in_stride = in->stat_in_stride; g.ln_dim = in->ln_dim; g.rope_tokens = in->rope_tokens;
     g.gelu_tanh = in->gelu_tanh; g.star_kind = in->star_kind; g.ld_out = in->ld_out; g.x_blocked = in->x_blocked ? 1 : 0;
+    g.a_blocked = a_blocked ? 1 : 0; g.out16_blocked = out16_blocked ? 1 : 0;
     g.qscale = in->qscale; g.ln_eps = in->ln_eps; g.star_scale = in->star_scale; g.star_bias = in->star_bias;
 
     HIPTS_TRY(launch_gemm((GemmEpilogue)epi, g, nullptr));
@@ -147,3 +164,5 @@
     HIPTS_TRY(fetch(out->stat_part, stat, out->stat_part_bytes));
     return HIPTS_OK;
 }
+}
+}
diff --git a/anime-illust-image-searcher_amd/csrc/gemm_epi.h b/anime-illust-image-searcher_amd/csrc/gemm_epi.h
--- a/anime-illust-image-searcher_amd/csrc/gemm_epi.h
+++ b/anime-illust-image-searcher_amd/csrc/gemm_epi.h
@@ -29,6 +29,22 @@
         grow = grow < rows_total ? grow : rows_total - 1;
         const bf16_t* g = X + (size_t)grow * K + (size_t)kt * BK + chunk * 8;
         glds16(g, lds_tile + rb8 * 1024);
+    }
+}
+
+constexpr int ACT_KTILE_STEP = 4 * 256;
+__device__ __forceinline__ size_t act_chunk_off(int row, int K, int kt, int chunk) {
+    return ((((size_t)(row >> 4) * (size_t)(K >> 4)) + (size_t)kt * 4 + (chunk >> 1)) << 8) + (size_t)((row & 15) * 16 + (chunk & 1) * 8);
+}
+__device__ __forceinline__ void stage_tile_blocked(const bf16_t* __restrict__ X, int rows_total, int K, int row0, int kt, char* lds_tile, int wave, int lane) {
+    const int row_in = lane >> 3;
+    const int chunk = (lane & 7) ^ row_in;
+#pragma unroll
+    for (int i = 0; i < 4; ++i) {
+        const int rb8 = wave * 4 + i;
+        int grow = row0 + rb8 * 8 + row_in;
+        grow = grow < rows_total ? grow : rows_total - 1;
+        glds16(X + act_chunk_off(grow, K, kt, chunk), lds_tile + rb8 * 1024);
     }
 }
 
@@ -759,13 +775,13 @@
     }
 }
 
-template <int EPI, int MR, bool F16, int FORM = -1>
+template <int EPI, int MR, bool F16, int FORM = -1, bool BLK = false>
 __device__ __forceinline__ void gemm_epilogue_staged(const GemmArgs& a, f32x4 (&acc)[MR][4], int m0, int n0, int wave_m, int wave_n,
                                                      int lane, char* region, const f32x4* bias_pre = nullptr, const float2* st_lds = nullptr,
                                                      float2* red = nullptr) {
     if constexpr (EPI == EPI_GELU && FORM < 0) {
-        if (a.gelu_tanh) gemm_epilogue_staged<EPI, MR, F16, 1>(a, acc, m0, n0, wave_m, wave_n, lane, region, bias_pre, st_lds, red);
-        else gemm_epilogue_staged<EPI, MR, F16, 0>(a, acc, m0, n0, wave_m, wave_n, lane, region, bias_pre, st_lds, red);
+        if (a.gelu_tanh) gemm_epilogue_staged<EPI, MR, F16, 1, BLK>(a, acc, m0, n0, wave_m, wave_n, lane, region, bias_pre, st_lds, red);
+        else gemm_epilogue_staged<EPI, MR, F16, 0, BLK>(a, acc, m0, n0, wave_m, wave_n, lane, region, bias_pre, st_lds, red);
         return;
     }
     f32x4 bias_v[4];
@@ -831,6 +847,31 @@
         f32x4 bv[4];
 #pragma unroll
         for (int j = 0; j < 4; ++j) bv[j] = bias_v[j];
+        if constexpr (BLK) {
+            static_assert(EPI == EPI_GELU, "blocked 16-bit output: the GELU arm");
+            const int ldb = (a.ld_out ? a.ld_out : a.N) >> 4;
+            bf16_t* blk = a.out_bf16 + ((((size_t)(mrow0 >> 4) * ldb) + (size_t)(ncol0 >> 4)) << 8) + (lr * 16 + 4 * lq);
+            const size_t rb_step = (size_t)ldb << 8;
+            auto rows = [&](auto interior_tag) __attribute__((always_inline)) {
+                constexpr bool INTERIOR = decltype(interior_tag)::value;
+#pragma unroll
+                for (int i = 0; i < MR; ++i) {
+                    if (!INTERIOR && mrow0 + i * 16 >= a.M) continue;
+                    epi_turn(a, wave_m, i);
+                    float2 st = make_float2(1.f, 0.f);
+                    if (fold) st = st_lds ? st_lds[mrow0 - m0 + i * 16 + lr] : row_stat(a, mrow0 + i * 16 + lr);
+#pragma unroll
+                    for (int j = 0; j < 4; ++j) {
+                        if (!INTERIOR && ncol0 + j * 16 >= a.N) continue;
+                        const f32x4 gv = gelu_f4<FORM == 1>(acc[i][j] * st.x + (bv[j] - cu[j] * st.y));
+                        *reinterpret_cast<bf16x4*>(blk + (size_t)i * rb_step + j * 256) = pack4<F16>(gv[0], gv[1], gv[2], gv[3]);
+                    }
+                }
+            };
+            if (mrow0 + MR * 16 <= a.M && ncol0 + 64 <= a.N) rows(std::true_type{});
+            else rows(std::false_type{});
+            return;
+        }
         if constexpr (EPI == EPI_STAR) {
             if (a.out8) {
                 staged_store_rows8<MR>(region, lane, mrow0, a.M, reinterpret_cast<uint8_t*>(a.out_bf16), a.ld_out ? a.ld_out : a.N, ncol0, a.N,
diff --git a/anime-illust-image-searcher_amd/csrc/gemm_plan.h b/anime-illust-image-searcher_amd/csrc/gemm_plan.h
--- a/anime-illust-image-searcher_amd/csrc/gemm_plan.h
+++ b/anime-illust-image-searcher_amd/csrc/gemm_plan.h
@@ -52,7 +52,9 @@
     int variant = k.variant;
     if (staged_only) variant = HIPTSDBG_GEMM_PP;
     if (epi == EPI_RESID_LN) variant = HIPTSDBG_GEMM_PP;
-    if (variant == HIPTSDBG_GEMM_PP && epi != EPI_HEAD && epi != EPI_RESID_LN && (!k.variant_set || staged_only) &&
+    const bool act_blocked = a.a_blocked || a.out16_blocked;
+    if (act_blocked) variant = HIPTSDBG_GEMM_PP;
+    if (variant == HIPTSDBG_GEMM_PP && !act_blocked && epi != EPI_HEAD && epi != EPI_RESID_LN && (!k.variant_set || staged_only) &&
         gemm_dw_size((long)p.tiles_m * p.tiles_n, cus, k) && a.M > T && !((next_ln || epi == EPI_SWIGLU) && a.stat_part))
         variant = HIPTSDBG_GEMM_DW;
 #ifdef HIPTS_X_DW_STAT
@@ -60,7 +62,7 @@
 #else
     const bool mask_stat_ok = !(next_ln && a.stat_part);
 #endif
-    if (variant == HIPTSDBG_GEMM_PP && ((k.dw_mask >> (int)epi) & 1u) && a.M > T && mask_stat_ok) variant = HIPTSDBG_GEMM_DW;
+    if (variant == HIPTSDBG_GEMM_PP && !act_blocked && ((k.dw_mask >> (int)epi) & 1u) && a.M > T && mask_stat_ok) variant = HIPTSDBG_GEMM_DW;
     if (a.f16 && variant != HIPTSDBG_GEMM_PP && variant != HIPTSDBG_GEMM_DW) {
         p.error = 1;
         return p;
@@ -98,7 +100,7 @@
     p.raster_gn = (k.raster_gn > 0 && tiles_n >= 8 && tiles_n > k.raster_gn) ? k.raster_gn : 0;
     const bool whole = epi == EPI_RESID_XG && mr == 8 && a.M % T == 0 && a.N % T == 0 && a.N <= 1024 && !a.pos && !a.res_scale && a.out_bf16 && a.stat_part;
 
-    if (mr == 8 && ((q4_mask >> (int)epi) & 1u) && (epi == EPI_GELU || epi == EPI_QK || epi == EPI_RESID_XG) && a.sk_slices <= 1 &&
+    if (mr == 8 && !act_blocked && ((q4_mask >> (int)epi) & 1u) && (epi == EPI_GELU || epi == EPI_QK || epi == EPI_RESID_XG) && a.sk_slices <= 1 &&
         !(a.stamps && !(a.f16 && (epi == EPI_GELU || epi == EPI_RESID_XG))) && a.M % T == 0 && a.N % T == 0 && a.K % 128 == 0 && a.K >= 128 &&
         !(epi == EPI_GELU && (a.ld_out ? a.ld_out : a.N) % 8) && !(epi == EPI_QK && a.dim % 64) &&
         (size_t)256 * a.K * 2 < ((size_t)1 << 31)) {
@@ -112,7 +114,7 @@
     if (epi == EPI_RESID || next_ln || epi == EPI_RESID_ROWSTAT || epi == EPI_HEAD) {
         const int sk_max = epi == EPI_HEAD ? (p.tiles_m == 1 ? k.splitk_head : 0) : k.splitk;
         const int rem = ntile % slots;
-        if (a.sk_ws && mr == 8 && sk_max >= 2 && rem > 0 && rem * 2 <= slots && rem <= 1024) {
+        if (a.sk_ws && mr == 8 && !act_blocked && sk_max >= 2 && rem > 0 && rem * 2 <= slots && rem <= 1024) {
             int sl = std::min(sk_max, std::min(slots / rem, a.K / GEMM_PLAN_BK / (k.splitk_minkt > 0 ? k.splitk_minkt : 1)));
             while (sl >= 2 && 4096 + (size_t)rem * sl * ((size_t)T * T * 4) > a.sk_ws_bytes) --sl;
             if (sl >= 2) {
diff --git a/anime-illust-image-searcher_amd/csrc/vit.hip b/anime-illust-image-searcher_amd/csrc/vit.hip
--- a/anime-illust-image-searcher_amd/csrc/vit.hip
+++ b/anime-illust-image-searcher_amd/csrc/vit.hip
@@ -8,6 +8,7 @@
 #include <vector>
 
 #include "vit_internal.h"
+#include "act_blocked.h"
 #include "dbg_buf.h"
 #include "model_host.h"
 #include "prof.h"
@@ -51,6 +52,7 @@
     bool fold_ln = false;
     bool fold_dirty = true;
     bool split_att = false;
+    int act_blocked = 0;
     int pool_splits = 1;
     static constexpr int kMaxSub = 4;
     int want_sub = 0;
@@ -242,6 +244,8 @@
     }
     h->fold_ln = D % 64 == 0 && h->tokens % 8 == 0 && cfg->mlp_dim % 8 == 0 && !getenv("HIPTS_GEMM") &&
                  !(getenv("HIPTS_LN_FOLD") && atoi(getenv("HIPTS_LN_FOLD")) == 0);
+    h->act_blocked = (h->fold_ln && !h->split_att && h->tokens % 16 == 0 && D % 16 == 0 && cfg->mlp_dim % 16 == 0)
+                         ? ((getenv("HIPTS_ACT_BLOCKED") ? atoi(getenv("HIPTS_ACT_BLOCKED")) : 1) & 1) : 0;
     if (h->fold_ln) {
         if ((st = h->stat_part.alloc(((D + 255) / 256) * M * 8))) {
             delete h;
@@ -479,6 +483,7 @@
         r.A = A; r.W = W; r.M = M; r.N = D; r.K = K; r.bias = bias; r.out_f32 = x;
         r.sk_ws = h->sk_ws.as<char>() + (size_t)sub * GEMM_SK_WS_BYTES; r.sk_ws_bytes = GEMM_SK_WS_BYTES;
         r.x_blocked = xb ? 1 : 0;
+        r.a_blocked = (A == hmid && (h->act_blocked & 1)) ? 1 : 0;
         if (next_gamma) {
             r.out_bf16 = xn; r.ln_gamma = next_gamma; r.stat_part = stat_p; r.stat_stride = M;
         } else if (xb) {
@@ -520,6 +525,7 @@
         g = gemm_args(f16, shared_chip);
         g.A = xn; g.W = L.fc1_w.as<bf16_t>(); g.M = M; g.N = c.mlp_dim; g.K = D;
         g.bias = L.fc1_b.as<float>(); g.out_bf16 = hmid; g.gelu_tanh = c.gelu_tanh;
+        g.out16_blocked = h->act_blocked & 1;
         if (fold) folded(g, L.fc1_u.as<float>(), L.fc1_c.as<float>());
         {
             ProfScope ps(h, s, PC_GEMM_GELU, 2.0 * dM * dD * dMlp, dM * dD * 2 + dM * dMlp * 2);
@@ -1206,6 +1212,12 @@
     return dbg_fetch(out16, od, out16_bytes, who);
 }
 
+extern "C" int hiptsdbg_vit_act_blocked(hipts_vit_t* h, int* bits) {
+    HIPTS_REQUIRE(h && bits, "null argument");
+    *bits = h->act_blocked;
+    return HIPTS_OK;
+}
+
 extern "C" int hiptsdbg_vit_dump(hipts_vit_t* h, const char* name, void* out_host, size_t max_bytes, size_t* bytes) {
     HIPTS_REQUIRE(h && name && out_host && bytes, "null argument");
     HIPTS_TRY(use_device(h->device));
@@ -1217,5 +1229,11 @@
     *bytes = b->bytes < max_bytes ? b->bytes : max_bytes;
     HIPTS_HIP(hipDeviceSynchronize());
     HIPTS_HIP(hipMemcpy(out_host, b->p, *bytes, hipMemcpyDeviceToHost));
-    return HIPTS_OK;
-}
+    if (b == &h->hmid && (h->act_blocked & 1)) {
+        const size_t ld = (size_t)h->cfg.mlp_dim, rows = *bytes / (32 * ld) * 16;
+        std::vector<uint16_t> rm(rows * ld);
+        act_unblock(static_cast<const uint16_t*>(out_host), rm.data(), rows, ld);
+        memcpy(out_host, rm.data(), rm.size() * 2);
+    }
+    return HIPTS_OK;
+}
diff --git a/anime-illust-image-searcher_amd/csrc/vit_internal.h b/anime-illust-image-searcher_amd/csrc/vit_internal.h
--- a/anime-illust-image-searcher_amd/csrc/vit_internal.h
+++ b/anime-illust-image-searcher_amd/csrc/vit_internal.h
@@ -195,6 +195,7 @@
     const bf16_t* A;
     const bf16_t* W;
     int M, N, K;
+    int a_blocked = 0;
     const float* bias;
     float* out_f32 = nullptr;
     float* out2_f32 = nullptr;
@@ -206,6 +207,7 @@
     int tokens_pad = 0;
     int heads = 0, dim = 0;
     int hd_log2 = 6;
+    int out16_blocked = 0;
     const float* res_scale = nullptr;
     const float* ln_gamma = nullptr;
     const float* ln_beta = nullptr;
diff --git a/include/hip_tagsearch_debug.h b/include/hip_tagsearch_debug.h
--- a/include/hip_tagsearch_debug.h
+++ b/include/hip_tagsearch_debug.h
@@ -38,6 +38,8 @@
                        unsigned q4_mask, hiptsdbg_gemm_plan_t* out);
 int hiptsdbg_gemm_tile_walk(int tiles_m, int tiles_n, int tile_rows, int raster_gm, int raster_gn, int32_t* m0, int32_t* n0);
 int hiptsdbg_gemm_kernel_resources(int epi, int mr, int f16, int op8, int sk, int interior, int* num_regs, int* scratch_bytes, int* static_lds);
+int hiptsdbg_gemm_kernel_resources_blocked(int epi, int mr, int f16, int interior, int a_blocked, int out16_blocked, int* num_regs, int* scratch_bytes,
+                                           int* static_lds);
 typedef struct hiptsdbg_gemm_case_t {
     int32_t epi, M, N, K, f16, shared_chip;
     const uint16_t* a;
@@ -67,6 +69,8 @@
     uint64_t x_bytes, rowmajor_bytes, probs_bytes, out16_bytes[3], stat_part_bytes;
 } hiptsdbg_gemm_out_t;
 int hiptsdbg_gemm_epilogue(const hiptsdbg_gemm_case_t* in, hiptsdbg_gemm_out_t* out);
+int hiptsdbg_gemm_epilogue_blocked(const hiptsdbg_gemm_case_t* in, hiptsdbg_gemm_out_t* out, int a_blocked, int out16_blocked);
+int hiptsdbg_act_block(const uint16_t* in, uint16_t* out, int64_t rows, int64_t ld, int unblock);
 enum { HIPTSDBG_SRC_F32 = 0, HIPTSDBG_SRC_F32_BLOCKED = 1, HIPTSDBG_SRC_F32_INPLACE = 2, HIPTSDBG_SRC_16_BIAS = 3 };
 enum { HIPTSDBG_AFF_GAMMA_BETA = 0, HIPTSDBG_AFF_GAMMA_OPT_BETA = 1, HIPTSDBG_AFF_GAMMA_ADD_ZERO = 2, HIPTSDBG_AFF_GAMMA_PLAIN = 3 };
 enum { HIPTSDBG_SINK_16 = 0, HIPTSDBG_SINK_E4M3 = 1, HIPTSDBG_SINK_F32 = 2, HIPTSDBG_SINK_F32_AND_16 = 3, HIPTSDBG_SINK_PATCH2X2 = 4,
@@ -113,6 +117,7 @@
 int hiptsdbg_gemm_run(int M, int N, int K, const uint16_t* a_bf16, const uint16_t* w_bf16, float* out_host);
 int hiptsdbg_gemm8_run(int M, int N, int K, const float* a_f32, const float* w_f32, int kind, void* out_host, int* w_exp);
 int hiptsdbg_vit_dump(hipts_vit_t* h, const char* name, void* out_host, size_t max_bytes, size_t* bytes);
+int hiptsdbg_vit_act_blocked(hipts_vit_t* h, int* bits);
 
 int hiptsdbg_attention_run(const uint16_t* q, const uint16_t* k, const uint16_t* vT, uint16_t* out_host, int batch, int heads, int tokens,
                            int tokens_pad, int head_dim, int f16);
```

Result: no change. 5511 images/sec, median of 6 (+0.8%).
